# microsoft/Nova

Hardware: NVIDIA H100
Metric: MSM throughput (2^20 BN254 scalar*G1/s) (higher is better)
Workload: dtype u32 limbs (256-bit prime-field / curve integers)

## Files before the change

nova_b200/csrc/capi.cu:

```cuda
#include <cuda_runtime.h>

#include <atomic>
#include <cstdarg>
#include <cstdio>
#include <cstring>
#include <cstdlib>
#include <map>
#include <memory>
#include <mutex>
#include <vector>

#include "../../include/nova_b200.h"
#include "msm_kernels.cuh"
#include "field_kernels.cuh"
#include "ops.cuh"
#include "poly_kernels.cuh"
#include "transcript.cuh"
#include "transcript_batched.cuh"
#include "sumcheck_tail.cuh"

using namespace nova;

namespace {

thread_local char g_err[512] = "";

int fail(int code, const char* fmt, ...) {
  va_list ap;
  va_start(ap, fmt);
  vsnprintf(g_err, sizeof(g_err), fmt, ap);
  va_end(ap);
  return code;
}

#define CU(call)                                                                        \
  do {                                                                                  \
    cudaError_t e_ = (call);                                                            \
    if (e_ != cudaSuccess)                                                              \
      return fail(e_ == cudaErrorMemoryAllocation ? B200_E_NOMEM : B200_E_CUDA,         \
                  "%s failed: %s (%s:%d)", #call, cudaGetErrorString(e_), __FILE__, __LINE__); \
  } while (0)

struct curve_info {
  int base_fid, scalar_fid;
};
const curve_info CURVES[4] = {
    {B200_FIELD_BN254_FQ, B200_FIELD_BN254_FR},
    {B200_FIELD_BN254_FR, B200_FIELD_BN254_FQ},
    {B200_FIELD_PALLAS_FP, B200_FIELD_PALLAS_FQ},
    {B200_FIELD_PALLAS_FQ, B200_FIELD_PALLAS_FP},
};
const int FIELD_BITS[4] = {254, 254, 255, 255};

struct device_state {
  std::mutex mu;
  bool ready = false;
  int device = 0;
  cudaStream_t stream = nullptr;
  cudaStream_t aux = nullptr;
  bool pool = true;
} g_dev;

int ensure_init() {
  std::lock_guard<std::mutex> lk(g_dev.mu);
  if (g_dev.ready) {
    CU(cudaSetDevice(g_dev.device));
    return B200_OK;
  }
  int cnt = 0;
  cudaError_t e = cudaGetDeviceCount(&cnt);
  if (e != cudaSuccess || cnt == 0)
    return fail(B200_E_CUDA, "no usable CUDA device (%s); nova_b200 has no CPU fallback",
                e == cudaSuccess ? "count = 0" : cudaGetErrorString(e));
  CU(cudaSetDevice(g_dev.device));
  CU(cudaStreamCreateWithFlags(&g_dev.stream, cudaStreamNonBlocking));
  CU(cudaStreamCreateWithFlags(&g_dev.aux, cudaStreamNonBlocking));
  const char* pe = getenv("NOVA_B200_POOL");
  g_dev.pool = !(pe && pe[0] == '0');
  if (g_dev.pool) {
    cudaMemPool_t pool;
    if (cudaDeviceGetDefaultMemPool(&pool, g_dev.device) == cudaSuccess) {
      uint64_t keep = UINT64_MAX;
      cudaMemPoolSetAttribute(pool, cudaMemPoolAttrReleaseThreshold, &keep);
    } else {
      g_dev.pool = false;
      cudaGetLastError();
    }
  }
  g_dev.ready = true;
  return B200_OK;
}

cudaError_t pool_alloc(void** p, size_t bytes) {
  return g_dev.pool ? cudaMallocAsync(p, bytes ? bytes : 1, g_dev.stream) : cudaMalloc(p, bytes ? bytes : 1);
}
cudaError_t pool_free(void* p) { return g_dev.pool ? cudaFreeAsync(p, g_dev.stream) : cudaFree(p); }

struct workspace {
  size_t cap_n = 0;
  void* scalars = nullptr;
  int32_t* digits = nullptr;
  uint32_t *counts = nullptr, *start = nullptr, *cursor = nullptr, *blocksums = nullptr;
  uint64_t* entries = nullptr;
  void *buckets = nullptr, *parts = nullptr, *rparts = nullptr, *sumscratch = nullptr;
  uint32_t* pkeys = nullptr;
  uint32_t* heavy = nullptr;
  uint32_t heavy_cap = 0;
  void* hparts = nullptr;
  void* d_out = nullptr;
  void* h_out = nullptr;
  size_t out_slots = 0;
  uint32_t* idx32 = nullptr;
  size_t idx_cap = 0;
  cudaStream_t last_stream = nullptr;
  cudaEvent_t busy = nullptr;
  void release() {
    if (busy) cudaEventDestroy(busy);
    void* ptrs[] = {scalars, digits, counts, start, cursor, blocksums, entries, buckets,
                    parts, rparts, sumscratch, pkeys, heavy, hparts, d_out, idx32};
    for (void* p : ptrs)
      if (p) cudaFree(p);
    if (h_out) cudaFreeHost(h_out);
    *this = workspace();
  }
};

struct ck_ctx {
  std::mutex mu;
  int curve = 0;
  size_t n = 0;
  size_t stride = 0;
  bool has_h = false;
  int c = 0, W = 0, F = 0, G = 0;
  uint32_t B = 0;
  int m = 4;
  void* tables = nullptr;
  workspace ws;
  struct lane {
    workspace ws;
    cudaStream_t s = nullptr;
    cudaEvent_t done = nullptr;
  };
  static constexpr int NLANES = 4;
  lane lanes[NLANES];
  struct host_slot {
    std::mutex mu;
    workspace ws;
    cudaStream_t s = nullptr, side = nullptr;
  };
  static constexpr int NSLOTS = 4;
  host_slot slots[NSLOTS];
  unsigned next_slot = 0;
  std::shared_ptr<ck_ctx> small;
  ~ck_ctx() {
    if (tables) cudaFree(tables);
    ws.release();
    for (lane& l : lanes) {
      l.ws.release();
      if (l.done) cudaEventDestroy(l.done);
      if (l.s) cudaStreamDestroy(l.s);
    }
    for (host_slot& h : slots) {
      h.ws.release();
      if (h.s) cudaStreamDestroy(h.s);
      if (h.side) cudaStreamDestroy(h.side);
    }
  }
};

enum { ST_DIGITS = 0, ST_SORT, ST_ACCUMULATE, ST_FIXUP, ST_REDUCE, ST_COUNT };
const int STAGE_KERNELS[ST_COUNT] = {1, 4, 1, 3, 2};
struct profile_state {
  std::mutex mu;
  bool enabled = false;
  static constexpr int PROF_RING = 4;
  cudaEvent_t ev[PROF_RING][ST_COUNT + 1] = {};
  bool have_events = false;
  bool pending[PROF_RING] = {};
  int next = 0;
  double ms[ST_COUNT] = {};
  uint64_t msms = 0;
  uint64_t launches = 0;
} g_prof;

void prof_fold_set_locked(int k) {
  if (!g_prof.pending[k]) return;
  if (cudaEventSynchronize(g_prof.ev[k][ST_COUNT]) == cudaSuccess) {
    for (int i = 0; i < ST_COUNT; i++) {
      float t = 0;
      if (cudaEventElapsedTime(&t, g_prof.ev[k][i], g_prof.ev[k][i + 1]) == cudaSuccess) g_prof.ms[i] += t;
    }
    g_prof.msms++;
  }
  g_prof.pending[k] = false;
}
void prof_fold_locked() {
  for (int k = 0; k < profile_state::PROF_RING; k++) prof_fold_set_locked(k);
}

void count_launch(int k) {
  std::lock_guard<std::mutex> lk(g_prof.mu);
  g_prof.launches += k;
}

std::mutex g_handles_mu;
std::map<uint64_t, std::shared_ptr<ck_ctx>> g_handles;
uint64_t g_next_handle = 1;

std::shared_ptr<ck_ctx> get_ck(uint64_t h) {
  std::lock_guard<std::mutex> lk(g_handles_mu);
  auto it = g_handles.find(h);
  return it == g_handles.end() ? nullptr : it->second;
}

constexpr size_t XYZZ_BYTES = 144;
constexpr int SUM_THREADS = NUM_SMS * 128;
constexpr int L_MIN = 32;
constexpr int L_FLOOR_DEFAULT = 16;
constexpr size_t ACC_THREADS = (size_t)NUM_SMS * 16 * 32 * 3;
constexpr uint32_t HEAVY_PARTS = 96;

size_t acc_threads() {
  static const size_t threads = [] {
    const char* e = getenv("NOVA_B200_ACC_WAVES");
    double w = e ? atof(e) : 0.0;
    return w > 0.0 ? (size_t)((double)NUM_SMS * 16 * 32 * w) : ACC_THREADS;
  }();
  return threads;
}
size_t acc_lmin() {
  static const size_t lmin = [] {
    const char* e = getenv("NOVA_B200_ACC_LMIN");
    int v = e ? atoi(e) : L_FLOOR_DEFAULT;
    return (size_t)(v < 8 ? 8 : (v > L_MIN ? L_MIN : v));
  }();
  return lmin;
}
int segment_len(size_t entries) {
  size_t L = (entries + acc_threads() - 1) / acc_threads();
  return (int)(L < acc_lmin() ? acc_lmin() : L);
}
size_t max_segments(size_t entries) {
  size_t by_floor = (entries + acc_lmin() - 1) / acc_lmin();
  size_t cap = acc_threads() + 256;
  return by_floor < cap ? by_floor : cap;
}

int ws_acquire(workspace& w, cudaStream_t s) {
  if (w.busy && w.last_stream != s) CU(cudaStreamWaitEvent(s, w.busy, 0));
  return B200_OK;
}
int ws_release(workspace& w, cudaStream_t s) {
  if (!w.busy) CU(cudaEventCreateWithFlags(&w.busy, cudaEventDisableTiming));
  CU(cudaEventRecord(w.busy, s));
  w.last_stream = s;
  return B200_OK;
}

int ensure_workspace(ck_ctx& ck, workspace& w, size_t n, size_t out_slots) {
  if (out_slots > w.out_slots) {
    if (w.d_out) cudaFree(w.d_out);
    if (w.h_out) cudaFreeHost(w.h_out);
    w.d_out = w.h_out = nullptr;
    CU(cudaMalloc(&w.d_out, out_slots * 96));
    CU(cudaMallocHost(&w.h_out, out_slots * 96));
    w.out_slots = out_slots;
  }
  if (n <= w.cap_n) return B200_OK;
  CU(cudaDeviceSynchronize());
  void** szbufs[] = {&w.scalars, (void**)&w.digits, (void**)&w.entries, &w.parts, (void**)&w.pkeys,
                     (void**)&w.heavy, &w.hparts};
  for (void** p : szbufs)
    if (*p) {
      cudaFree(*p);
      *p = nullptr;
    }
  size_t K = (size_t)ck.G * ck.B;
  size_t entries = n * (size_t)ck.W;
  size_t nseg = max_segments(entries);
  w.heavy_cap = (uint32_t)(nseg / HEAVY_PARTS + 2);
  CU(cudaMalloc((void**)&w.heavy, ((size_t)w.heavy_cap + 1) * 4));
  CU(cudaMalloc(&w.hparts, (size_t)w.heavy_cap * HEAVY_SPLIT * XYZZ_BYTES));
  CU(cudaMalloc(&w.scalars, n * 32));
  CU(cudaMalloc((void**)&w.digits, entries * sizeof(int32_t)));
  CU(cudaMalloc((void**)&w.entries, entries * sizeof(uint64_t)));
  CU(cudaMalloc(&w.parts, 2 * nseg * XYZZ_BYTES));
  CU(cudaMalloc((void**)&w.pkeys, 2 * nseg * sizeof(uint32_t)));
  if (!w.counts) {
    CU(cudaMalloc((void**)&w.counts, K * 4));
    CU(cudaMalloc((void**)&w.start, (K + 1) * 4));
    CU(cudaMalloc((void**)&w.cursor, K * 4));
    CU(cudaMalloc((void**)&w.blocksums, 4096 * 4));
    CU(cudaMalloc(&w.buckets, K * XYZZ_BYTES));
    CU(cudaMalloc(&w.rparts, ((size_t)ck.G * (ck.B / ck.m + 4096)) * XYZZ_BYTES));
    CU(cudaMalloc(&w.sumscratch, (size_t)SUM_THREADS * XYZZ_BYTES));
  }
  w.cap_n = n;
  return B200_OK;
}

int ensure_workspace(ck_ctx& ck, size_t n, size_t out_slots) {
  return ensure_workspace(ck, ck.ws, n, out_slots);
}

msm_plan make_plan(ck_ctx& ck, workspace& ws, size_t base_offset, size_t n) {
  msm_plan p;
  p.n = n;
  p.n_ck = ck.stride;
  p.base_offset = base_offset;
  p.blind_i = SIZE_MAX;
  p.h_index = ck.n;
  p.c = ck.c;
  p.W = ck.W;
  p.G = ck.G;
  p.B = ck.B;
  p.L = segment_len(n * (size_t)ck.W);
  p.m = ck.m;
  p.heavy = ws.heavy;
  p.heavy_min = HEAVY_PARTS * (uint32_t)p.L;
  p.heavy_cap = ws.heavy_cap;
  p.hparts = ws.hparts;
  p.digits = ws.digits;
  p.counts = ws.counts;
  p.start = ws.start;
  p.cursor = ws.cursor;
  p.entries = ws.entries;
  p.buckets = ws.buckets;
  p.parts = ws.parts;
  p.pkeys = ws.pkeys;
  p.rparts = ws.rparts;
  p.blocksums = ws.blocksums;
  return p;
}

int enqueue_msm(ck_ctx& ck, workspace& ws, size_t base_offset, const void* d_scalars, size_t n,
                void* d_out, cudaStream_t s, int small_elem_bytes = 0, bool blinded = false,
                bool digits_done = false, const msm_peer* peer = nullptr, bool profile_ok = true) {
  const field_ops* sops = ops_for_field(CURVES[ck.curve].scalar_fid);
  const field_ops* bops = ops_for_field(CURVES[ck.curve].base_fid);
  {
    int arc = ws_acquire(ws, s);
    if (arc) return arc;
  }
  if (n == 0) {
    if (peer && peer->world > 1) {
      msm_plan p0 = make_plan(ck, ws, base_offset, 0);
      p0.peer = *peer;
      bops->exchange_identity(s, p0, d_out);
      count_launch(1);
      CU(cudaGetLastError());
      return B200_OK;
    }
    CU(cudaMemsetAsync(d_out, 0, 96, s));
    return B200_OK;
  }
  msm_plan p = make_plan(ck, ws, base_offset, n);
  if (peer) p.peer = *peer;
  if (blinded) p.blind_i = n - 1;
  size_t K = (size_t)ck.G * ck.B;
  if (!digits_done) CU(cudaMemsetAsync(p.counts, 0, K * 4, s));
  CU(cudaMemsetAsync(p.heavy, 0, 4, s));
  std::lock_guard<std::mutex> plk(g_prof.mu);
  const bool prof = g_prof.enabled && profile_ok;
  const int pset = g_prof.next;
  if (prof) {
    if (!g_prof.have_events) {
      for (auto& set : g_prof.ev)
        for (auto& e : set) CU(cudaEventCreate(&e));
      g_prof.have_events = true;
    }
    prof_fold_set_locked(pset);
    g_prof.next = (pset + 1) % profile_state::PROF_RING;
  }
#define STAGE_MARK(i) \
  if (prof) CU(cudaEventRecord(g_prof.ev[pset][i], s))
  STAGE_MARK(ST_DIGITS);
  if (digits_done)
    ;
  else if (small_elem_bytes)
    msm_digits_small(s, d_scalars, small_elem_bytes, p);
  else
    sops->digits(s, d_scalars, p);
  STAGE_MARK(ST_SORT);
  msm_scan(s, p);
  msm_scatter(s, p);
  STAGE_MARK(ST_ACCUMULATE);
  bops->accumulate(s, ck.tables, p);
  STAGE_MARK(ST_FIXUP);
  bops->fixup(s, p);
  STAGE_MARK(ST_REDUCE);
  bops->reduce(s, p, d_out);
  STAGE_MARK(ST_COUNT);
#undef STAGE_MARK
  if (prof) g_prof.pending[pset] = true;
  for (int i = 0; i < ST_COUNT; i++) g_prof.launches += STAGE_KERNELS[i];
  g_prof.launches += (ck.c - 1 + 3) / 4 - 1;
  CU(cudaGetLastError());
  return ws_release(ws, s);
}

int enqueue_msm(ck_ctx& ck, size_t base_offset, const void* d_scalars, size_t n, void* d_out,
                cudaStream_t s, int small_elem_bytes = 0, bool blinded = false) {
  return enqueue_msm(ck, ck.ws, base_offset, d_scalars, n, d_out, s, small_elem_bytes, blinded);
}

struct dev_flag {
  uint32_t* p = nullptr;
  ~dev_flag() {
    if (p) cudaFree(p);
  }
};

constexpr size_t SMALL_KEY_MAX = (size_t)1 << 21;
constexpr int SMALL_KEY_WINDOW = 17;

int choose_window(size_t n) {
  int lg = 0;
  while (((size_t)1 << lg) < n) lg++;
  int c = lg;
  if (c < 8) c = 8;
  if (c > 16) c = 16;
  if (lg >= 22) c = 20;
  else if (lg >= 19) c = 17;
  return c;
}

constexpr int CURVE_B_SMALL[4] = {3, -17, 5, 5};

int register_key(int curve_id, const void* bases, bool bases_on_device, size_t n, const void* h,
                 int window_bits, bool expand, std::shared_ptr<ck_ctx>& out, size_t* first_bad = nullptr,
                 cudaStream_t st = nullptr, size_t src_pitch_points = 0, size_t src_block_points = 0) {
  if (!st) st = g_dev.stream;
  if (curve_id < 0 || curve_id > 3) return fail(B200_E_ARG, "unknown curve id %d", curve_id);
  if (bases == nullptr || n == 0) return fail(B200_E_ARG, "empty commitment key");
  if (window_bits != 0 && (window_bits < 2 || window_bits > 24))
    return fail(B200_E_ARG, "window_bits %d out of range [2,24]", window_bits);
  auto ck = std::make_shared<ck_ctx>();
  ck->curve = curve_id;
  ck->n = n;
  ck->has_h = h != nullptr;
  ck->stride = n + (h ? 1 : 0);
  ck->c = window_bits ? window_bits : choose_window(n);
  int bits = FIELD_BITS[CURVES[curve_id].scalar_fid];
  ck->W = (bits + ck->c - 1) / ck->c;
  ck->F = expand ? ck->W : 1;
  ck->G = expand ? 1 : ck->W;
  ck->B = 1u << (ck->c - 1);
  ck->m = ck->B >= 4 ? 4 : 1;
  if ((size_t)ck->F * ck->stride >= ((size_t)1 << 31))
    return fail(B200_E_RANGE, "key too large for 31-bit table indices (%zu x %d)", n, ck->F);
  CU(cudaMalloc(&ck->tables, (size_t)ck->F * ck->stride * 64));
  const cudaMemcpyKind kind = bases_on_device ? cudaMemcpyDeviceToDevice : cudaMemcpyHostToDevice;
  if (src_block_points == 0) {
    CU(cudaMemcpyAsync(ck->tables, bases, n * 64, kind, st));
  } else {
    const size_t full = n / src_block_points, rest = n % src_block_points;
    if (full)
      CU(cudaMemcpy2DAsync(ck->tables, src_block_points * 64, bases, src_pitch_points * 64, src_block_points * 64, full,
                           kind, st));
    if (rest)
      CU(cudaMemcpyAsync((char*)ck->tables + full * src_block_points * 64,
                         (const char*)bases + full * src_pitch_points * 64, rest * 64, kind, st));
  }
  if (h)
    CU(cudaMemcpyAsync((char*)ck->tables + n * 64, h, 64, cudaMemcpyHostToDevice, st));
  if (first_bad) {
    *first_bad = SIZE_MAX;
    dev_flag flag;
    CU(cudaMalloc(&flag.p, 4));
    CU(cudaMemsetAsync(flag.p, 0xFF, 4, st));
    ops_for_field(CURVES[curve_id].base_fid)
        ->on_curve(st, ck->tables, ck->stride, CURVE_B_SMALL[curve_id], flag.p);
    count_launch(1);
    CU(cudaGetLastError());
    uint32_t bad = 0;
    CU(cudaMemcpyAsync(&bad, flag.p, 4, cudaMemcpyDeviceToHost, st));
    CU(cudaStreamSynchronize(st));
    if (bad != 0xFFFFFFFFu) {
      *first_bad = bad;
      return fail(B200_E_POINT, "key point %u%s has a non-canonical coordinate or is not on the curve", bad,
                  (h && bad == n) ? " (the blinding generator)" : "");
    }
  }
  {
    const field_ops* bops = ops_for_field(CURVES[curve_id].base_fid);
    bops->expand_key(st, ck->tables, ck->stride, ck->F, ck->c * ck->G);
    CU(cudaGetLastError());
  }
  CU(cudaStreamSynchronize(st));
  if (expand && window_bits == 0 && ck->c >= 20) {
    size_t ns = n < SMALL_KEY_MAX ? n : SMALL_KEY_MAX;
    if (src_block_points) return fail(B200_E_ARG, "strided keys carry one table set");
    int rc = register_key(curve_id, bases, bases_on_device, ns, h, SMALL_KEY_WINDOW, true, ck->small, nullptr, st);
    if (rc) return rc;
  }
  out = ck;
  return B200_OK;
}

ck_ctx& route(ck_ctx& ck, size_t base_offset, size_t n) {
  if (ck.small && base_offset + n <= ck.small->n) return *ck.small;
  return ck;
}

template <class Fn>
int with_field(int field_id, Fn fn) {
  int rc = ensure_init();
  if (rc) return rc;
  const field_ops* ops = ops_for_field(field_id);
  if (!ops) return fail(B200_E_ARG, "unknown field id %d", field_id);
  return fn(ops);
}

struct dev_buf {
  void* p = nullptr;
  ~dev_buf() {
    if (p) pool_free(p);
  }
  int alloc(size_t bytes) {
    CU(pool_alloc(&p, bytes));
    return B200_OK;
  }
};

}

extern "C" {

const char* b200_last_error(void) { return g_err; }
const char* b200_version(void) { return "nova_b200 0.1 (sm_90a)"; }

int b200_init(int device) {
  {
    std::lock_guard<std::mutex> lk(g_dev.mu);
    if (!g_dev.ready) g_dev.device = device;
  }
  return ensure_init();
}

int b200_device_count(int* count) {
  if (!count) return fail(B200_E_ARG, "null count");
  cudaError_t e = cudaGetDeviceCount(count);
  if (e != cudaSuccess) {
    *count = 0;
    return fail(B200_E_CUDA, "cudaGetDeviceCount: %s", cudaGetErrorString(e));
  }
  return B200_OK;
}

int b200_host_alloc(size_t bytes, void** ptr) {
  int rc = ensure_init();
  if (rc) return rc;
  CU(cudaMallocHost(ptr, bytes ? bytes : 1));
  return B200_OK;
}
int b200_host_free(void* ptr) {
  CU(cudaFreeHost(ptr));
  return B200_OK;
}
int b200_dev_alloc(size_t bytes, void** dptr) {
  int rc = ensure_init();
  if (rc) return rc;
  CU(pool_alloc(dptr, bytes));
  return B200_OK;
}
int b200_dev_free(void* dptr) {
  if (!dptr) return B200_OK;
  int rc = ensure_init();
  if (rc) return rc;
  CU(pool_free(dptr));
  return B200_OK;
}
int b200_memcpy_h2d(void* dptr, const void* hptr, size_t bytes) {
  int rc = ensure_init();
  if (rc) return rc;
  CU(cudaMemcpyAsync(dptr, hptr, bytes, cudaMemcpyHostToDevice, g_dev.stream));
  CU(cudaStreamSynchronize(g_dev.stream));
  return B200_OK;
}
int b200_memcpy_d2h(void* hptr, const void* dptr, size_t bytes) {
  int rc = ensure_init();
  if (rc) return rc;
  CU(cudaMemcpyAsync(hptr, dptr, bytes, cudaMemcpyDeviceToHost, g_dev.stream));
  CU(cudaStreamSynchronize(g_dev.stream));
  return B200_OK;
}
int b200_memcpy_d2d(void* dst, const void* src, size_t bytes, void* stream) {
  int rc = ensure_init();
  if (rc) return rc;
  if (bytes == 0) return B200_OK;
  if (!dst || !src) return fail(B200_E_ARG, "null pointer");
  CU(cudaMemcpyAsync(dst, src, bytes, cudaMemcpyDeviceToDevice,
                     stream ? (cudaStream_t)stream : g_dev.stream));
  return B200_OK;
}
int b200_memset_dev(void* dptr, int byte, size_t bytes, void* stream) {
  int rc = ensure_init();
  if (rc) return rc;
  if (bytes == 0) return B200_OK;
  if (!dptr) return fail(B200_E_ARG, "null pointer");
  CU(cudaMemsetAsync(dptr, byte, bytes, stream ? (cudaStream_t)stream : g_dev.stream));
  return B200_OK;
}
int b200_sync(void) {
  int rc = ensure_init();
  if (rc) return rc;
  CU(cudaDeviceSynchronize());
  return B200_OK;
}

int b200_profile_enable(int on) {
  std::lock_guard<std::mutex> lk(g_prof.mu);
  g_prof.enabled = on != 0;
  return B200_OK;
}
int b200_profile_reset(void) {
  std::lock_guard<std::mutex> lk(g_prof.mu);
  prof_fold_locked();
  for (double& m : g_prof.ms) m = 0;
  g_prof.msms = 0;
  g_prof.launches = 0;
  return B200_OK;
}
int b200_profile_read(double* stage_ms, int nstages, uint64_t* msms, uint64_t* launches) {
  std::lock_guard<std::mutex> lk(g_prof.mu);
  prof_fold_locked();
  for (int i = 0; i < nstages && i < ST_COUNT; i++)
    if (stage_ms) stage_ms[i] = g_prof.ms[i];
  if (msms) *msms = g_prof.msms;
  if (launches) *launches = g_prof.launches;
  return B200_OK;
}

int b200_jacobian_sum_dev(int curve_id, const void* d_points, size_t k, void* d_out, void* stream) {
  int rc = ensure_init();
  if (rc) return rc;
  if (curve_id < 0 || curve_id > 3) return fail(B200_E_ARG, "unknown curve id %d", curve_id);
  if (!d_out || (k && !d_points)) return fail(B200_E_ARG, "null pointer");
  const field_ops* bops = ops_for_field(CURVES[curve_id].base_fid);
  bops->jacobian_sum(stream ? (cudaStream_t)stream : g_dev.stream, d_points, (int)k, d_out);
  {
    std::lock_guard<std::mutex> lk(g_prof.mu);
    g_prof.launches += 1;
  }
  CU(cudaGetLastError());
  return B200_OK;
}

int b200_ck_register(int curve_id, const void* bases, size_t n, const void* h, int window_bits,
                     uint64_t* handle) {
  int rc = ensure_init();
  if (rc) return rc;
  if (!handle) return fail(B200_E_ARG, "null handle pointer");
  std::shared_ptr<ck_ctx> ck;
  rc = register_key(curve_id, bases, false, n, h, window_bits, true, ck);
  if (rc) return rc;
  std::lock_guard<std::mutex> lk(g_handles_mu);
  *handle = g_next_handle++;
  g_handles[*handle] = ck;
  return B200_OK;
}

int b200_ck_register_checked(int curve_id, const void* bases, size_t n, const void* h, int window_bits,
                             uint64_t* handle, size_t* first_bad) {
  int rc = ensure_init();
  if (rc) return rc;
  if (!handle || !first_bad) return fail(B200_E_ARG, "null pointer");
  *handle = 0;
  std::shared_ptr<ck_ctx> ck;
  rc = register_key(curve_id, bases, false, n, h, window_bits, true, ck, first_bad);
  if (rc) return rc;
  std::lock_guard<std::mutex> lk(g_handles_mu);
  *handle = g_next_handle++;
  g_handles[*handle] = ck;
  return B200_OK;
}

int b200_ck_setup_synthetic(int curve_id, const void* gen_affine, uint64_t k0, size_t n, int with_h,
                            int window_bits, uint64_t* handle) {
  int rc = ensure_init();
  if (rc) return rc;
  if (curve_id < 0 || curve_id > 3) return fail(B200_E_ARG, "unknown curve id %d", curve_id);
  if (!gen_affine || !handle || n == 0) return fail(B200_E_ARG, "bad argument");
  size_t total = n + (with_h ? 1 : 0);
  dev_buf bases, gen;
  if ((rc = bases.alloc(total * 64))) return rc;
  if ((rc = gen.alloc(64))) return rc;
  CU(cudaMemcpyAsync(gen.p, gen_affine, 64, cudaMemcpyHostToDevice, g_dev.stream));
  const field_ops* bops = ops_for_field(CURVES[curve_id].base_fid);
  bops->index_bases(g_dev.stream, bases.p, total, gen.p, k0);
  CU(cudaGetLastError());
  std::vector<char> h(64);
  if (with_h)
    CU(cudaMemcpyAsync(h.data(), (char*)bases.p + n * 64, 64, cudaMemcpyDeviceToHost, g_dev.stream));
  CU(cudaStreamSynchronize(g_dev.stream));
  std::shared_ptr<ck_ctx> ck;
  rc = register_key(curve_id, bases.p, true, n, with_h ? h.data() : nullptr, window_bits, true, ck);
  if (rc) return rc;
  std::lock_guard<std::mutex> lk(g_handles_mu);
  *handle = g_next_handle++;
  g_handles[*handle] = ck;
  return B200_OK;
}

int b200_ck_setup_tau(int curve_id, const void* gen_affine, const void* tau_mont, size_t n, int window_bits,
                      uint64_t* handle) {
  int rc = ensure_init();
  if (rc) return rc;
  if (curve_id < 0 || curve_id > 3) return fail(B200_E_ARG, "unknown curve id %d", curve_id);
  if (!gen_affine || !tau_mont || !handle || n == 0) return fail(B200_E_ARG, "bad argument");
  dev_buf bases, gen, tau, pw;
  if ((rc = bases.alloc(n * 64)) || (rc = gen.alloc(64)) || (rc = tau.alloc(32)) || (rc = pw.alloc(n * 32))) return rc;
  CU(cudaMemcpyAsync(gen.p, gen_affine, 64, cudaMemcpyHostToDevice, g_dev.stream));
  CU(cudaMemcpyAsync(tau.p, tau_mont, 32, cudaMemcpyHostToDevice, g_dev.stream));
  ops_for_field(CURVES[curve_id].scalar_fid)->powers_canonical(g_dev.stream, tau.p, n, pw.p);
  ops_for_field(CURVES[curve_id].base_fid)->scalar_bases(g_dev.stream, bases.p, n, gen.p, pw.p);
  count_launch(2);
  CU(cudaGetLastError());
  CU(cudaStreamSynchronize(g_dev.stream));
  std::shared_ptr<ck_ctx> ck;
  rc = register_key(curve_id, bases.p, true, n, nullptr, window_bits, true, ck);
  if (rc) return rc;
  std::lock_guard<std::mutex> lk(g_handles_mu);
  *handle = g_next_handle++;
  g_handles[*handle] = ck;
  return B200_OK;
}

int b200_ck_export_bases(uint64_t handle, size_t offset, size_t n, void* out_host) {
  int rc = ensure_init();
  if (rc) return rc;
  auto ck = get_ck(handle);
  if (!ck) return fail(B200_E_HANDLE, "unknown key handle %llu", (unsigned long long)handle);
  if (offset + n > ck->n) return fail(B200_E_RANGE, "export [%zu, %zu) exceeds key length %zu", offset, offset + n, ck->n);
  if (n == 0) return B200_OK;
  if (!out_host) return fail(B200_E_ARG, "null pointer");
#if defined(NOVA_MSM_ARITH29)
  return fail(B200_E_ARG, "b200_ck_export_bases: table 0 is not in the boundary format in this build");
#else
  std::lock_guard<std::mutex> lk(ck->mu);
  CU(cudaMemcpyAsync(out_host, (const char*)ck->tables + offset * 64, n * 64, cudaMemcpyDeviceToHost, g_dev.stream));
  CU(cudaStreamSynchronize(g_dev.stream));
  return B200_OK;
#endif
}

int b200_ck_release(uint64_t handle) {
  std::shared_ptr<ck_ctx> ck;
  {
    std::lock_guard<std::mutex> lk(g_handles_mu);
    auto it = g_handles.find(handle);
    if (it == g_handles.end()) return fail(B200_E_HANDLE, "unknown key handle %llu",
                                           (unsigned long long)handle);
    ck = it->second;
    g_handles.erase(it);
  }
  std::lock_guard<std::mutex> lk(ck->mu);
  for (ck_ctx* t : {ck.get(), ck->small.get()})
    if (t)
      for (ck_ctx::host_slot& h : t->slots) std::lock_guard<std::mutex> wait(h.mu);
  cudaSetDevice(g_dev.device);
  return B200_OK;
}

int b200_ck_len(uint64_t handle, size_t* n, int* window_bits, int* num_tables) {
  auto ck = get_ck(handle);
  if (!ck) return fail(B200_E_HANDLE, "unknown key handle %llu", (unsigned long long)handle);
  if (n) *n = ck->n;
  if (window_bits) *window_bits = ck->c;
  if (num_tables) *num_tables = ck->F;
  return B200_OK;
}

static int lane_stream(ck_ctx::lane& ln, int index) {
  if (ln.s) return B200_OK;
  int least = 0, greatest = 0;
  CU(cudaDeviceGetStreamPriorityRange(&least, &greatest));
  int prio = greatest + index;
  if (prio > least) prio = least;
  CU(cudaStreamCreateWithPriority(&ln.s, cudaStreamNonBlocking, prio));
  CU(cudaEventCreateWithFlags(&ln.done, cudaEventDisableTiming));
  return B200_OK;
}

static int msm_host(ck_ctx& ck, size_t base_offset, const void* scalars, size_t n, void* out,
                    const void* blind = nullptr) {
  int rc = B200_OK;
  static const int h2d_chunks = [] {
    const char* e = getenv("NOVA_B200_H2D_CHUNKS");
    int k = e ? atoi(e) : 4;
    return k < 1 ? 1 : (k > 64 ? 64 : k);
  }();
  static const int e2e_slices = [] {
    const char* e = getenv("NOVA_B200_E2E_SLICES");
    int k = e ? atoi(e) : 4;
    return k < 1 ? 1 : (k > ck_ctx::NLANES ? ck_ctx::NLANES : k);
  }();
  if (e2e_slices > 1 && n >= ((size_t)1 << 23)) {
    std::lock_guard<std::mutex> lk(ck.mu);
    cudaStream_t s = g_dev.stream;
    const int k = e2e_slices;
    rc = ensure_workspace(ck, 1, (size_t)k + 1);
    if (rc) return rc;
    if ((rc = ws_acquire(ck.ws, s))) return rc;
    cudaEvent_t ev = nullptr;
    CU(cudaEventCreateWithFlags(&ev, cudaEventDisableTiming));
    CU(cudaEventRecord(ev, s));
    const size_t per = (n + k - 1) / k;
    int used = 0;
    for (int j = 0; j < k && rc == B200_OK; j++) {
      const size_t lo = (size_t)j * per, hi = lo + per < n ? lo + per : n;
      if (lo >= hi) break;
      const bool last = hi == n;
      ck_ctx::lane& ln = ck.lanes[j];
      if ((rc = lane_stream(ln, j))) break;
      CU(cudaStreamWaitEvent(ln.s, ev, 0));
      rc = ensure_workspace(ck, ln.ws, hi - lo + 1, 1);
      if (rc) break;
      if ((rc = ws_acquire(ln.ws, ln.s))) break;
      CU(cudaMemcpyAsync(ln.ws.scalars, (const char*)scalars + 32 * lo, 32 * (hi - lo), cudaMemcpyHostToDevice, ln.s));
      const bool with_blind = last && blind != nullptr;
      if (with_blind)
        CU(cudaMemcpyAsync((char*)ln.ws.scalars + 32 * (hi - lo), blind, 32, cudaMemcpyHostToDevice, ln.s));
      rc = enqueue_msm(ck, ln.ws, base_offset + lo, ln.ws.scalars, hi - lo + (with_blind ? 1 : 0),
                       (char*)ck.ws.d_out + 96 * (j + 1), ln.s, 0, with_blind);
      used = j + 1;
    }
    for (int j = 0; j < used; j++) {
      cudaEventRecord(ck.lanes[j].done, ck.lanes[j].s);
      cudaStreamWaitEvent(s, ck.lanes[j].done, 0);
    }
    cudaEventDestroy(ev);
    if (rc) return rc;
    ops_for_field(CURVES[ck.curve].base_fid)->jacobian_sum(s, (char*)ck.ws.d_out + 96, used, ck.ws.d_out);
    count_launch(1);
    CU(cudaGetLastError());
    CU(cudaMemcpyAsync(ck.ws.h_out, ck.ws.d_out, 96, cudaMemcpyDeviceToHost, s));
    CU(cudaStreamSynchronize(s));
    memcpy(out, ck.ws.h_out, 96);
    return B200_OK;
  }
  ck_ctx::host_slot* slot = nullptr;
  for (ck_ctx::host_slot& h : ck.slots)
    if (h.mu.try_lock()) {
      slot = &h;
      break;
    }
  if (!slot) {
    unsigned turn;
    {
      std::lock_guard<std::mutex> lk(ck.mu);
      turn = ck.next_slot++ % ck_ctx::NSLOTS;
    }
    slot = &ck.slots[turn];
    slot->mu.lock();
  }
  std::lock_guard<std::mutex> slk(slot->mu, std::adopt_lock);
  if (!slot->s) {
    CU(cudaStreamCreateWithFlags(&slot->s, cudaStreamNonBlocking));
    CU(cudaStreamCreateWithFlags(&slot->side, cudaStreamNonBlocking));
  }
  workspace& W = slot->ws;
  cudaStream_t s = slot->s;
  if ((rc = ensure_workspace(ck, W, n + 1, 1))) return rc;
  if (h2d_chunks > 1 && n >= ((size_t)1 << 16)) {
    cudaStream_t side = slot->side;
    const size_t total = n + (blind ? 1 : 0);
    const field_ops* sops = ops_for_field(CURVES[ck.curve].scalar_fid);
    msm_plan p = make_plan(ck, W, base_offset, total);
    cudaEvent_t ev = nullptr;
    CU(cudaEventCreateWithFlags(&ev, cudaEventDisableTiming));
    CU(cudaEventRecord(ev, s));
    CU(cudaStreamWaitEvent(side, ev, 0));
    CU(cudaMemsetAsync(p.counts, 0, (size_t)ck.G * ck.B * 4, side));
    const size_t per = (n + h2d_chunks - 1) / h2d_chunks;
    auto piece = [&](const void* src, size_t lo, size_t hi) -> int {
      CU(cudaMemcpyAsync((char*)W.scalars + 32 * lo, src, 32 * (hi - lo), cudaMemcpyHostToDevice, s));
      CU(cudaEventRecord(ev, s));
      CU(cudaStreamWaitEvent(side, ev, 0));
      sops->digits_range(side, W.scalars, lo, hi, p);
      count_launch(1);
      return B200_OK;
    };
    for (size_t lo = 0; lo < n && rc == B200_OK; lo += per)
      rc = piece((const char*)scalars + 32 * lo, lo, lo + per < n ? lo + per : n);
    if (blind && rc == B200_OK) rc = piece(blind, n, n + 1);
    if (rc) {
      cudaEventDestroy(ev);
      return rc;
    }
    CU(cudaEventRecord(ev, side));
    CU(cudaStreamWaitEvent(s, ev, 0));
    cudaEventDestroy(ev);
    rc = enqueue_msm(ck, W, base_offset, W.scalars, total, W.d_out, s, 0, blind != nullptr, true);
  } else {
    if (n) CU(cudaMemcpyAsync(W.scalars, scalars, n * 32, cudaMemcpyHostToDevice, s));
    if (blind) CU(cudaMemcpyAsync((char*)W.scalars + n * 32, blind, 32, cudaMemcpyHostToDevice, s));
    rc = enqueue_msm(ck, W, base_offset, W.scalars, n + (blind ? 1 : 0), W.d_out, s, 0, blind != nullptr);
  }
  if (rc) return rc;
  CU(cudaMemcpyAsync(W.h_out, W.d_out, 96, cudaMemcpyDeviceToHost, s));
  CU(cudaStreamSynchronize(s));
  memcpy(out, W.h_out, 96);
  return B200_OK;
}

int b200_msm(uint64_t handle, size_t base_offset, const void* scalars, size_t n, void* out) {
  int rc = ensure_init();
  if (rc) return rc;
  auto ck = get_ck(handle);
  if (!ck) return fail(B200_E_HANDLE, "unknown key handle %llu", (unsigned long long)handle);
  if (!out || (n && !scalars)) return fail(B200_E_ARG, "null pointer");
  if (base_offset + n > ck->n)
    return fail(B200_E_RANGE, "msm slice [%zu, %zu) exceeds key length %zu", base_offset,
                base_offset + n, ck->n);
  return msm_host(route(*ck, base_offset, n), base_offset, scalars, n, out);
}

int b200_commit(uint64_t handle, const void* scalars, size_t n, const void* r, void* out) {
  int rc = ensure_init();
  if (rc) return rc;
  auto ck = get_ck(handle);
  if (!ck) return fail(B200_E_HANDLE, "unknown key handle %llu", (unsigned long long)handle);
  if (!out || (n && !scalars)) return fail(B200_E_ARG, "null pointer");
  if (n > ck->n)
    return fail(B200_E_RANGE, "commit of %zu scalars exceeds key length %zu", n, ck->n);
  if (r && !ck->has_h) return fail(B200_E_ARG, "key was registered without a blinding generator");
  return msm_host(route(*ck, 0, n), 0, scalars, n, out, r);
}

int b200_msm_dev(uint64_t handle, size_t base_offset, const void* d_scalars, size_t n, void* d_out,
                 void* stream) {
  int rc = ensure_init();
  if (rc) return rc;
  auto ck = get_ck(handle);
  if (!ck) return fail(B200_E_HANDLE, "unknown key handle %llu", (unsigned long long)handle);
  if (!d_out || (n && !d_scalars)) return fail(B200_E_ARG, "null pointer");
  if (base_offset + n > ck->n)
    return fail(B200_E_RANGE, "msm slice [%zu, %zu) exceeds key length %zu", base_offset,
                base_offset + n, ck->n);
  ck_ctx& t = route(*ck, base_offset, n);
  std::lock_guard<std::mutex> lk(t.mu);
  rc = ensure_workspace(t, n ? n : 1, 1);
  if (rc) return rc;
  return enqueue_msm(t, base_offset, d_scalars, n, d_out,
                     stream ? (cudaStream_t)stream : g_dev.stream);
}

int b200_commit_dev(uint64_t handle, const void* d_scalars, size_t n, const void* d_blind_or_null,
                    void* d_out, void* stream) {
  int rc = ensure_init();
  if (rc) return rc;
  auto ck = get_ck(handle);
  if (!ck) return fail(B200_E_HANDLE, "unknown key handle %llu", (unsigned long long)handle);
  if (!d_out || (n && !d_scalars)) return fail(B200_E_ARG, "null pointer");
  if (n > ck->n) return fail(B200_E_RANGE, "commit of %zu scalars exceeds key length %zu", n, ck->n);
  if (d_blind_or_null && !ck->has_h)
    return fail(B200_E_ARG, "key was registered without a blinding generator");
  ck_ctx& t = route(*ck, 0, n);
  std::lock_guard<std::mutex> lk(t.mu);
  rc = ensure_workspace(t, n + 1, 1);
  if (rc) return rc;
  cudaStream_t s = stream ? (cudaStream_t)stream : g_dev.stream;
  if (!d_blind_or_null) return enqueue_msm(t, 0, d_scalars, n, d_out, s);
  if ((rc = ws_acquire(t.ws, s))) return rc;
  if (n) CU(cudaMemcpyAsync(t.ws.scalars, d_scalars, n * 32, cudaMemcpyDeviceToDevice, s));
  CU(cudaMemcpyAsync((char*)t.ws.scalars + n * 32, d_blind_or_null, 32, cudaMemcpyDeviceToDevice, s));
  return enqueue_msm(t, 0, t.ws.scalars, n + 1, d_out, s, 0, true);
}

static int enqueue_many(ck_ctx& ck, const void* const* vecs, const size_t* lens, size_t k,
                        bool from_host, void* d_out, cudaStream_t s, const size_t* offsets = nullptr) {
  std::unique_lock<std::mutex> lsmall;
  if (ck.small) lsmall = std::unique_lock<std::mutex>(ck.small->mu);
  cudaEvent_t start_ev = nullptr;
  CU(cudaEventCreateWithFlags(&start_ev, cudaEventDisableTiming));
  CU(cudaEventRecord(start_ev, s));
  bool used[2][ck_ctx::NLANES] = {};
  size_t next[2] = {0, 0};
  int rc = B200_OK;
  for (size_t j = 0; j < k && rc == B200_OK; j++) {
    const size_t off = offsets ? offsets[j] : 0;
    ck_ctx& t = route(ck, off, lens[j]);
    int which = &t == &ck ? 0 : 1;
    int li = (int)(next[which]++ % ck_ctx::NLANES);
    ck_ctx::lane& ln = t.lanes[li];
    if ((rc = lane_stream(ln, li))) break;
    if (!used[which][li]) {
      CU(cudaStreamWaitEvent(ln.s, start_ev, 0));
      used[which][li] = true;
    }
    rc = ensure_workspace(t, ln.ws, lens[j] ? lens[j] : 1, 1);
    if (rc) break;
    const void* src = vecs[j];
    if ((rc = ws_acquire(ln.ws, ln.s))) break;
    if (from_host && lens[j]) {
      CU(cudaMemcpyAsync(ln.ws.scalars, vecs[j], lens[j] * 32, cudaMemcpyHostToDevice, ln.s));
      src = ln.ws.scalars;
    }
    rc = enqueue_msm(t, ln.ws, off, src, lens[j], (char*)d_out + 96 * j, ln.s);
  }
  for (int which = 0; which < 2; which++) {
    ck_ctx* t = which == 0 ? &ck : ck.small.get();
    for (int li = 0; t && li < ck_ctx::NLANES; li++)
      if (used[which][li]) {
        cudaEventRecord(t->lanes[li].done, t->lanes[li].s);
        cudaStreamWaitEvent(s, t->lanes[li].done, 0);
      }
  }
  cudaEventDestroy(start_ev);
  return rc;
}

static int check_many(ck_ctx& ck, const void* const* vecs, const size_t* lens, size_t k) {
  if (!vecs || !lens) return fail(B200_E_ARG, "null pointer");
  for (size_t j = 0; j < k; j++) {
    if (lens[j] > ck.n)
      return fail(B200_E_RANGE, "batch vector %zu has %zu scalars, key has %zu", j, lens[j], ck.n);
    if (lens[j] && !vecs[j]) return fail(B200_E_ARG, "null scalar vector %zu", j);
  }
  return B200_OK;
}

int b200_msm_batch(uint64_t handle, const void* const* scalars, const size_t* lens, size_t k,
                   void* out) {
  int rc = ensure_init();
  if (rc) return rc;
  auto ck = get_ck(handle);
  if (!ck) return fail(B200_E_HANDLE, "unknown key handle %llu", (unsigned long long)handle);
  if (k == 0) return B200_OK;
  if (!out) return fail(B200_E_ARG, "null pointer");
  if ((rc = check_many(*ck, scalars, lens, k))) return rc;
  std::lock_guard<std::mutex> lk(ck->mu);
  rc = ensure_workspace(*ck, 1, k);
  if (rc) return rc;
  cudaStream_t s = g_dev.stream;
  rc = enqueue_many(*ck, scalars, lens, k, true, ck->ws.d_out, s);
  if (rc) return rc;
  CU(cudaMemcpyAsync(ck->ws.h_out, ck->ws.d_out, 96 * k, cudaMemcpyDeviceToHost, s));
  CU(cudaStreamSynchronize(s));
  memcpy(out, ck->ws.h_out, 96 * k);
  return B200_OK;
}

int b200_commit_many_dev(uint64_t handle, const void* const* d_scalars, const size_t* lens, size_t k,
                         void* d_out, void* stream) {
  int rc = ensure_init();
  if (rc) return rc;
  auto ck = get_ck(handle);
  if (!ck) return fail(B200_E_HANDLE, "unknown key handle %llu", (unsigned long long)handle);
  if (k == 0) return B200_OK;
  if (!d_out) return fail(B200_E_ARG, "null pointer");
  if ((rc = check_many(*ck, d_scalars, lens, k))) return rc;
  std::lock_guard<std::mutex> lk(ck->mu);
  return enqueue_many(*ck, d_scalars, lens, k, false, d_out,
                      stream ? (cudaStream_t)stream : g_dev.stream);
}

int b200_msm_many_dev(uint64_t handle, const size_t* base_offsets, const void* const* d_scalars, const size_t* lens,
                      size_t k, void* d_out, void* stream) {
  int rc = ensure_init();
  if (rc) return rc;
  auto ck = get_ck(handle);
  if (!ck) return fail(B200_E_HANDLE, "unknown key handle %llu", (unsigned long long)handle);
  if (k == 0) return B200_OK;
  if (!d_out || !base_offsets || !d_scalars || !lens) return fail(B200_E_ARG, "null pointer");
  for (size_t j = 0; j < k; j++) {
    if (base_offsets[j] + lens[j] > ck->n)
      return fail(B200_E_RANGE, "msm %zu: slice [%zu, %zu) exceeds key length %zu", j, base_offsets[j],
                  base_offsets[j] + lens[j], ck->n);
    if (lens[j] && !d_scalars[j]) return fail(B200_E_ARG, "null scalar vector %zu", j);
  }
  std::lock_guard<std::mutex> lk(ck->mu);
  return enqueue_many(*ck, d_scalars, lens, k, false, d_out,
                      stream ? (cudaStream_t)stream : g_dev.stream, base_offsets);
}

int b200_msm_small(uint64_t handle, size_t base_offset, const void* scalars, int elem_bytes, size_t n,
                   int max_bits, void* out) {
  int rc = ensure_init();
  if (rc) return rc;
  auto ck = get_ck(handle);
  if (!ck) return fail(B200_E_HANDLE, "unknown key handle %llu", (unsigned long long)handle);
  if (!out || (n && !scalars)) return fail(B200_E_ARG, "null pointer");
  if (elem_bytes != 1 && elem_bytes != 2 && elem_bytes != 4 && elem_bytes != 8)
    return fail(B200_E_ARG, "elem_bytes must be 1, 2, 4 or 8 (got %d)", elem_bytes);
  if (max_bits < 0 || max_bits > 64) return fail(B200_E_ARG, "max_bits %d out of range", max_bits);
  if (base_offset + n > ck->n)
    return fail(B200_E_RANGE, "msm slice [%zu, %zu) exceeds key length %zu", base_offset,
                base_offset + n, ck->n);
  ck_ctx& t = route(*ck, base_offset, n);
  std::lock_guard<std::mutex> lk(t.mu);
  rc = ensure_workspace(t, n ? n : 1, 1);
  if (rc) return rc;
  cudaStream_t s = g_dev.stream;
  if ((rc = ws_acquire(t.ws, s))) return rc;
  if (n) CU(cudaMemcpyAsync(t.ws.scalars, scalars, n * elem_bytes, cudaMemcpyHostToDevice, s));
  rc = enqueue_msm(t, base_offset, t.ws.scalars, n, t.ws.d_out, s, elem_bytes);
  if (rc) return rc;
  CU(cudaMemcpyAsync(t.ws.h_out, t.ws.d_out, 96, cudaMemcpyDeviceToHost, s));
  CU(cudaStreamSynchronize(s));
  memcpy(out, t.ws.h_out, 96);
  return B200_OK;
}

int b200_msm_indices(uint64_t handle, const uint64_t* idx, size_t m, void* out) {
  int rc = ensure_init();
  if (rc) return rc;
  auto ck = get_ck(handle);
  if (!ck) return fail(B200_E_HANDLE, "unknown key handle %llu", (unsigned long long)handle);
  if (!out || (m && !idx)) return fail(B200_E_ARG, "null pointer");
  std::vector<uint32_t> idx32(m);
  for (size_t j = 0; j < m; j++) {
    if (idx[j] >= ck->n) return fail(B200_E_RANGE, "index %llu outside key of %zu",
                                     (unsigned long long)idx[j], ck->n);
    idx32[j] = (uint32_t)idx[j];
  }
  std::lock_guard<std::mutex> lk(ck->mu);
  rc = ensure_workspace(*ck, 1, 1);
  if (rc) return rc;
  workspace& w = ck->ws;
  if (m > w.idx_cap) {
    if (w.idx32) cudaFree(w.idx32);
    w.idx32 = nullptr;
    CU(cudaMalloc((void**)&w.idx32, m * 4));
    w.idx_cap = m;
  }
  cudaStream_t s = g_dev.stream;
  if (m) CU(cudaMemcpyAsync(w.idx32, idx32.data(), m * 4, cudaMemcpyHostToDevice, s));
  const field_ops* bops = ops_for_field(CURVES[ck->curve].base_fid);
  bops->sum_points(s, ck->tables, w.idx32, m, w.sumscratch, w.d_out);
  count_launch(2);
  CU(cudaGetLastError());
  CU(cudaMemcpyAsync(w.h_out, w.d_out, 96, cudaMemcpyDeviceToHost, s));
  CU(cudaStreamSynchronize(s));
  memcpy(out, w.h_out, 96);
  return B200_OK;
}

int b200_msm_adhoc(int curve_id, const void* bases, const void* scalars, size_t n, void* out) {
  int rc = ensure_init();
  if (rc) return rc;
  if (!out) return fail(B200_E_ARG, "null out");
  if (n == 0) {
    memset(out, 0, 96);
    return B200_OK;
  }
  if (!bases || !scalars) return fail(B200_E_ARG, "null pointer");
  std::shared_ptr<ck_ctx> ck;
  rc = register_key(curve_id, bases, false, n, nullptr, 0, false, ck);
  if (rc) return rc;
  return msm_host(route(*ck, 0, n), 0, scalars, n, out);
}

int b200_keccak256(const void* data, size_t len, void* out32) {
  if (!out32 || (len && !data)) return fail(B200_E_ARG, "null pointer");
  const size_t rate = 136;
  uint64_t st[25] = {};
  const uint8_t* p = (const uint8_t*)data;
  auto absorb_block = [&](const uint8_t* blk) {
    for (size_t i = 0; i < rate / 8; i++) {
      uint64_t w;
      memcpy(&w, blk + 8 * i, 8);
      st[i] ^= w;
    }
    nova::keccak_f1600(st);
  };
  while (len >= rate) {
    absorb_block(p);
    p += rate;
    len -= rate;
  }
  uint8_t last[136] = {};
  if (len) memcpy(last, p, len);
  last[len] ^= 0x01;
  last[rate - 1] ^= 0x80;
  absorb_block(last);
  memcpy(out32, st, 32);
  return B200_OK;
}

namespace {
struct peer_group {
  std::mutex mu;
  msm_peer desc;
};
std::mutex g_groups_mu;
std::map<uint64_t, std::shared_ptr<peer_group>> g_groups;
uint64_t g_next_group = 1;
}

int b200_peer_buffer_alloc(void** dptr) {
  int rc = ensure_init();
  if (rc) return rc;
  if (!dptr) return fail(B200_E_ARG, "null pointer");
  CU(cudaMalloc(dptr, MSM_PEER_BUF_BYTES));
  CU(cudaMemset(*dptr, 0, MSM_PEER_BUF_BYTES));
  return B200_OK;
}
int b200_peer_buffer_free(void* dptr) {
  if (dptr) CU(cudaFree(dptr));
  return B200_OK;
}
int b200_ipc_export(const void* dptr, void* handle64_out) {
  int rc = ensure_init();
  if (rc) return rc;
  if (!dptr || !handle64_out) return fail(B200_E_ARG, "null pointer");
  static_assert(sizeof(cudaIpcMemHandle_t) == 64, "the ABI carries IPC handles as 64 bytes");
  cudaIpcMemHandle_t h;
  CU(cudaIpcGetMemHandle(&h, const_cast<void*>(dptr)));
  memcpy(handle64_out, &h, 64);
  return B200_OK;
}
int b200_ipc_open(const void* handle64, void** dptr) {
  int rc = ensure_init();
  if (rc) return rc;
  if (!handle64 || !dptr) return fail(B200_E_ARG, "null pointer");
  cudaIpcMemHandle_t h;
  memcpy(&h, handle64, 64);
  CU(cudaIpcOpenMemHandle(dptr, h, cudaIpcMemLazyEnablePeerAccess));
  return B200_OK;
}
int b200_ipc_close(void* dptr) {
  if (!dptr) return B200_OK;
  CU(cudaIpcCloseMemHandle(dptr));
  return B200_OK;
}
int b200_peer_group_create(int rank, int world, void* const* bufs, uint64_t* group) {
  int rc = ensure_init();
  if (rc) return rc;
  if (!bufs || !group) return fail(B200_E_ARG, "null pointer");
  if (world < 1 || world > MSM_PEER_MAX || rank < 0 || rank >= world)
    return fail(B200_E_ARG, "peer group of %d ranks (rank %d): world must be 1..%d", world, rank, MSM_PEER_MAX);
  auto g = std::make_shared<peer_group>();
  g->desc.world = world;
  g->desc.rank = rank;
  for (int r = 0; r < world; r++) {
    if (!bufs[r]) return fail(B200_E_ARG, "null exchange buffer for rank %d", r);
    g->desc.buf[r] = bufs[r];
  }
  std::lock_guard<std::mutex> lk(g_groups_mu);
  *group = g_next_group++;
  g_groups[*group] = g;
  return B200_OK;
}
int b200_peer_group_release(uint64_t group) {
  std::lock_guard<std::mutex> lk(g_groups_mu);
  if (!g_groups.erase(group)) return fail(B200_E_HANDLE, "unknown peer group %llu", (unsigned long long)group);
  return B200_OK;
}
static std::shared_ptr<peer_group> get_group(uint64_t h) {
  std::lock_guard<std::mutex> lk(g_groups_mu);
  auto it = g_groups.find(h);
  return it == g_groups.end() ? nullptr : it->second;
}
int b200_peer_group_status(uint64_t group) {
  int rc = ensure_init();
  if (rc) return rc;
  auto g = get_group(group);
  if (!g) return fail(B200_E_HANDLE, "unknown peer group %llu", (unsigned long long)group);
  unsigned long long err = 0;
  CU(cudaMemcpy(&err, (const char*)g->desc.buf[g->desc.rank] + MSM_PEER_ERR_OFF, 8, cudaMemcpyDeviceToHost));
  if (err) return fail(B200_E_PEER, "a peer never delivered its partial sum (epoch %llu): exchange timed out", err);
  return B200_OK;
}

int b200_msm_sharded_dev(uint64_t handle, size_t base_offset, const void* d_scalars, size_t n, uint64_t group,
                         void* d_out, void* stream) {
  int rc = ensure_init();
  if (rc) return rc;
  auto ck = get_ck(handle);
  if (!ck) return fail(B200_E_HANDLE, "unknown key handle %llu", (unsigned long long)handle);
  auto g = get_group(group);
  if (!g) return fail(B200_E_HANDLE, "unknown peer group %llu", (unsigned long long)group);
  if (!d_out || (n && !d_scalars)) return fail(B200_E_ARG, "null pointer");
  if (base_offset + n > ck->n)
    return fail(B200_E_RANGE, "msm slice [%zu, %zu) exceeds key length %zu", base_offset, base_offset + n, ck->n);
#if defined(NOVA_MSM_ARITH29)
  return fail(B200_E_ARG, "the fused exchange needs the default (8x32-bit) arithmetic build");
#else
  ck_ctx& t = route(*ck, base_offset, n);
  std::lock_guard<std::mutex> glk(g->mu);
  std::lock_guard<std::mutex> lk(t.mu);
  rc = ensure_workspace(t, n ? n : 1, 1);
  if (rc) return rc;
  msm_peer peer = g->desc;
  peer.epoch = ++g->desc.epoch;
  return enqueue_msm(t, t.ws, base_offset, d_scalars, n, d_out, stream ? (cudaStream_t)stream : g_dev.stream, 0,
                     false, false, &peer);
#endif
}

namespace {
struct poseidon_ctx {
  int fid = 0, t = 0, r_f = 0, r_p = 0;
  void *rc = nullptr, *mds = nullptr;
  ~poseidon_ctx() {
    if (rc) cudaFree(rc);
    if (mds) cudaFree(mds);
  }
};
std::mutex g_pos_mu;
std::map<uint64_t, std::shared_ptr<poseidon_ctx>> g_pos;
uint64_t g_next_pos = 1;

void poseidon_tag(uint32_t n, unsigned char out32[32]) {
  typedef unsigned __int128 u128;
  const u128 base = (u128)0 - 159;
  u128 x_i = 1, state = 0;
  auto update = [&](uint32_t a) {
    x_i *= base;
    state += x_i * (u128)a;
  };
  if (n) update(n + (1u << 31));
  update(1);
  update(0);
  memset(out32, 0, 32);
  memcpy(out32, &state, 16);
}
}

int b200_poseidon_register(int fid, int arity, int r_f, int r_p, const void* rc_mont, const void* mds_mont, uint64_t* handle) {
  int rc = ensure_init();
  if (rc) return rc;
  if (!ops_for_field(fid)) return fail(B200_E_ARG, "unknown field id %d", fid);
  if (arity < 1 || arity + 1 > 25 || r_f < 2 || (r_f & 1) || r_p < 0 || !rc_mont || !mds_mont || !handle)
    return fail(B200_E_ARG, "bad Poseidon parameters (arity %d, R_F %d, R_P %d)", arity, r_f, r_p);
  auto c = std::make_shared<poseidon_ctx>();
  c->fid = fid;
  c->t = arity + 1;
  c->r_f = r_f;
  c->r_p = r_p;
  const size_t nrc = (size_t)(r_f + r_p) * c->t, nm = (size_t)c->t * c->t;
  CU(cudaMalloc(&c->rc, nrc * 32));
  CU(cudaMalloc(&c->mds, nm * 32));
  CU(cudaMemcpyAsync(c->rc, rc_mont, nrc * 32, cudaMemcpyHostToDevice, g_dev.stream));
  CU(cudaMemcpyAsync(c->mds, mds_mont, nm * 32, cudaMemcpyHostToDevice, g_dev.stream));
  CU(cudaStreamSynchronize(g_dev.stream));
  std::lock_guard<std::mutex> lk(g_pos_mu);
  *handle = g_next_pos++;
  g_pos[*handle] = c;
  return B200_OK;
}
int b200_poseidon_release(uint64_t handle) {
  std::lock_guard<std::mutex> lk(g_pos_mu);
  if (!g_pos.erase(handle)) return fail(B200_E_HANDLE, "unknown Poseidon handle %llu", (unsigned long long)handle);
  return B200_OK;
}
int b200_poseidon_ro_dev(uint64_t handle, const void* d_elems, size_t n, int num_bits, int start_with_one, void* d_out96,
                         void* stream) {
  int rc = ensure_init();
  if (rc) return rc;
  std::shared_ptr<poseidon_ctx> c;
  {
    std::lock_guard<std::mutex> lk(g_pos_mu);
    auto it = g_pos.find(handle);
    if (it == g_pos.end()) return fail(B200_E_HANDLE, "unknown Poseidon handle %llu", (unsigned long long)handle);
    c = it->second;
  }
  if (!d_out96 || (n && !d_elems)) return fail(B200_E_ARG, "null pointer");
  if (num_bits < 1 || num_bits > 250) return fail(B200_E_ARG, "num_bits %d outside 1..250", num_bits);
  if (n >= (1u << 31)) return fail(B200_E_ARG, "too many elements");
  cudaStream_t s = stream ? (cudaStream_t)stream : g_dev.stream;
  unsigned char tag[32];
  poseidon_tag((uint32_t)n, tag);
  void* d_tag = nullptr;
  CU(cudaMallocAsync(&d_tag, 32, s));
  CU(cudaMemcpyAsync(d_tag, tag, 32, cudaMemcpyHostToDevice, s));
  ops_for_field(c->fid)->poseidon_ro(s, c->t, c->r_f, c->r_p, c->rc, c->mds, d_elems, (uint32_t)n, d_tag, num_bits,
                                     start_with_one, d_out96);
  count_launch(1);
  CU(cudaGetLastError());
  CU(cudaFreeAsync(d_tag, s));
  return B200_OK;
}
int b200_poseidon_ro(uint64_t handle, const void* elems_mont, size_t n, int num_bits, int start_with_one, void* out96) {
  int rc = ensure_init();
  if (rc) return rc;
  if (!out96 || (n && !elems_mont)) return fail(B200_E_ARG, "null pointer");
  dev_buf in, out;
  if ((rc = in.alloc(n * 32 + 32)) || (rc = out.alloc(96))) return rc;
  if (n) CU(cudaMemcpyAsync(in.p, elems_mont, n * 32, cudaMemcpyHostToDevice, g_dev.stream));
  rc = b200_poseidon_ro_dev(handle, in.p, n, num_bits, start_with_one, out.p, g_dev.stream);
  if (rc) return rc;
  CU(cudaMemcpyAsync(out96, out.p, 96, cudaMemcpyDeviceToHost, g_dev.stream));
  CU(cudaStreamSynchronize(g_dev.stream));
  return B200_OK;
}
int b200_to_mont_dev(int fid, const void* d_canonical, size_t n, void* d_out, void* stream) {
  return with_field(fid, [&](const field_ops* ops) {
    if (n && (!d_canonical || !d_out)) return fail(B200_E_ARG, "null pointer");
    ops->to_mont(stream ? (cudaStream_t)stream : g_dev.stream, d_canonical, n, d_out);
    count_launch(1);
    CU(cudaGetLastError());
    return (int)B200_OK;
  });
}

namespace {
constexpr size_t MGPU_BLOCK = 4096;
struct mgpu_state {
  std::mutex mu;
  bool ready = false;
  int ndev = 0;
  int dev[MSM_PEER_MAX] = {};
  cudaStream_t stream[MSM_PEER_MAX] = {};
  void* xbuf[MSM_PEER_MAX] = {};
  void* out_dev[MSM_PEER_MAX] = {};
  void* out_host = nullptr;
  unsigned long long epoch = 0;
} g_mgpu;
struct mgpu_key {
  int curve = 0;
  size_t n = 0;
  bool has_h = false;
  std::shared_ptr<ck_ctx> part[MSM_PEER_MAX];
};
std::mutex g_mkeys_mu;
std::map<uint64_t, std::shared_ptr<mgpu_key>> g_mkeys;
uint64_t g_next_mkey = 1;

size_t mgpu_count(size_t n, int d, int D) {
  const size_t round = MGPU_BLOCK * (size_t)D;
  const size_t rem = n % round;
  size_t extra = rem > (size_t)d * MGPU_BLOCK ? rem - (size_t)d * MGPU_BLOCK : 0;
  if (extra > MGPU_BLOCK) extra = MGPU_BLOCK;
  return (n / round) * MGPU_BLOCK + extra;
}
struct device_guard {
  ~device_guard() { cudaSetDevice(g_dev.device); }
};
}

int b200_mgpu_init(int ndev, const int* devices_or_null) {
  int rc = ensure_init();
  if (rc) return rc;
  if (ndev < 1 || ndev > MSM_PEER_MAX) return fail(B200_E_ARG, "ndev %d outside 1..%d", ndev, MSM_PEER_MAX);
  std::lock_guard<std::mutex> lk(g_mgpu.mu);
  if (g_mgpu.ready) {
    if (g_mgpu.ndev != ndev) return fail(B200_E_ARG, "already initialised with %d devices", g_mgpu.ndev);
    return B200_OK;
  }
  int have = 0;
  CU(cudaGetDeviceCount(&have));
  device_guard guard;
  for (int d = 0; d < ndev; d++) {
    int id = devices_or_null ? devices_or_null[d] : d;
    if (id < 0 || id >= have) return fail(B200_E_ARG, "device %d not present (%d visible)", id, have);
    g_mgpu.dev[d] = id;
  }
  for (int d = 0; d < ndev; d++) {
    CU(cudaSetDevice(g_mgpu.dev[d]));
    CU(cudaStreamCreateWithFlags(&g_mgpu.stream[d], cudaStreamNonBlocking));
    CU(cudaMalloc(&g_mgpu.xbuf[d], MSM_PEER_BUF_BYTES));
    CU(cudaMemset(g_mgpu.xbuf[d], 0, MSM_PEER_BUF_BYTES));
    CU(cudaMalloc(&g_mgpu.out_dev[d], 96));
    for (int e = 0; e < ndev; e++) {
      if (g_mgpu.dev[e] == g_mgpu.dev[d]) continue;
      int can = 0;
      CU(cudaDeviceCanAccessPeer(&can, g_mgpu.dev[d], g_mgpu.dev[e]));
      if (!can) return fail(B200_E_CUDA, "device %d cannot access device %d (no NVLink / P2P path)", g_mgpu.dev[d], g_mgpu.dev[e]);
      cudaError_t pe = cudaDeviceEnablePeerAccess(g_mgpu.dev[e], 0);
      if (pe != cudaSuccess && pe != cudaErrorPeerAccessAlreadyEnabled)
        return fail(B200_E_CUDA, "cudaDeviceEnablePeerAccess(%d -> %d): %s", g_mgpu.dev[d], g_mgpu.dev[e], cudaGetErrorString(pe));
      cudaGetLastError();
    }
  }
  CU(cudaMallocHost(&g_mgpu.out_host, 96));
  g_mgpu.ndev = ndev;
  g_mgpu.ready = true;
  return B200_OK;
}

int b200_mgpu_ck_register(int curve_id, const void* bases, size_t n, const void* h, int window_bits, uint64_t* key) {
  int rc = ensure_init();
  if (rc) return rc;
  if (!g_mgpu.ready) return fail(B200_E_ARG, "b200_mgpu_init has not been called");
  if (curve_id < 0 || curve_id > 3) return fail(B200_E_ARG, "unknown curve id %d", curve_id);
  if (!bases || !key || n == 0) return fail(B200_E_ARG, "bad argument");
  std::lock_guard<std::mutex> lk(g_mgpu.mu);
  device_guard guard;
  auto mk = std::make_shared<mgpu_key>();
  mk->curve = curve_id;
  mk->n = n;
  mk->has_h = h != nullptr;
  const int D = g_mgpu.ndev;
  for (int d = 0; d < D; d++) {
    size_t nd = mgpu_count(n, d, D);
    if (nd == 0 && !(d == 0 && h)) continue;
    CU(cudaSetDevice(g_mgpu.dev[d]));
    if (nd == 0) return fail(B200_E_ARG, "key of %zu points is too small to carry a blinding generator on %d devices", n, D);
    rc = register_key(curve_id, (const char*)bases + (size_t)d * MGPU_BLOCK * 64, false, nd, d == 0 ? h : nullptr,
                      window_bits, true, mk->part[d], nullptr, g_mgpu.stream[d], MGPU_BLOCK * (size_t)D, MGPU_BLOCK);
    if (rc) return rc;
  }
  std::lock_guard<std::mutex> lk2(g_mkeys_mu);
  *key = g_next_mkey++;
  g_mkeys[*key] = mk;
  return B200_OK;
}

int b200_mgpu_ck_release(uint64_t key) {
  std::shared_ptr<mgpu_key> mk;
  {
    std::lock_guard<std::mutex> lk(g_mkeys_mu);
    auto it = g_mkeys.find(key);
    if (it == g_mkeys.end()) return fail(B200_E_HANDLE, "unknown multi-GPU key %llu", (unsigned long long)key);
    mk = it->second;
    g_mkeys.erase(it);
  }
  std::lock_guard<std::mutex> lk(g_mgpu.mu);
  device_guard guard;
  for (int d = 0; d < g_mgpu.ndev; d++) {
    cudaSetDevice(g_mgpu.dev[d]);
    cudaStreamSynchronize(g_mgpu.stream[d]);
  }
  return B200_OK;
}

int b200_mgpu_commit(uint64_t key, const void* scalars, size_t n, const void* r, void* out) {
  int rc = ensure_init();
  if (rc) return rc;
  if (!g_mgpu.ready) return fail(B200_E_ARG, "b200_mgpu_init has not been called");
  std::shared_ptr<mgpu_key> mk;
  {
    std::lock_guard<std::mutex> lk(g_mkeys_mu);
    auto it = g_mkeys.find(key);
    if (it == g_mkeys.end()) return fail(B200_E_HANDLE, "unknown multi-GPU key %llu", (unsigned long long)key);
    mk = it->second;
  }
  if (!out || (n && !scalars)) return fail(B200_E_ARG, "null pointer");
  if (n > mk->n) return fail(B200_E_RANGE, "commit of %zu scalars exceeds key length %zu", n, mk->n);
  if (r && !mk->has_h) return fail(B200_E_ARG, "key was registered without a blinding generator");
#if defined(NOVA_MSM_ARITH29)
  return fail(B200_E_ARG, "the fused exchange needs the default (8x32-bit) arithmetic build");
#else
  std::lock_guard<std::mutex> lk(g_mgpu.mu);
  device_guard guard;
  const int D = g_mgpu.ndev;
  msm_peer peer;
  peer.world = D;
  peer.epoch = ++g_mgpu.epoch;
  for (int d = 0; d < D; d++) peer.buf[d] = g_mgpu.xbuf[d];
  const field_ops* bops = ops_for_field(CURVES[mk->curve].base_fid);
  for (int d = 0; d < D; d++) {
    ck_ctx* part = mk->part[d].get();
    const size_t nd = mgpu_count(n, d, D);
    if (!part || (nd == 0 && !(d == 0 && r))) continue;
    CU(cudaSetDevice(g_mgpu.dev[d]));
    std::lock_guard<std::mutex> plk(part->mu);
    if ((rc = ensure_workspace(*part, part->ws, nd + 1, 1))) return rc;
  }
  for (int d = 0; d < D; d++) {
    CU(cudaSetDevice(g_mgpu.dev[d]));
    cudaStream_t s = g_mgpu.stream[d];
    peer.rank = d;
    const size_t nd = mgpu_count(n, d, D);
    const bool blind = d == 0 && r != nullptr;
    ck_ctx* part = mk->part[d].get();
    if ((nd == 0 && !blind) || !part) {
      msm_plan p0{};
      p0.peer = peer;
      bops->exchange_identity(s, p0, g_mgpu.out_dev[d]);
      count_launch(1);
      CU(cudaGetLastError());
      continue;
    }
    std::lock_guard<std::mutex> plk(part->mu);
    rc = ensure_workspace(*part, part->ws, nd + 1, 1);
    if (rc) return rc;
    if ((rc = ws_acquire(part->ws, s))) return rc;
    const size_t full = nd / MGPU_BLOCK, rest = nd % MGPU_BLOCK;
    const char* src = (const char*)scalars + (size_t)d * MGPU_BLOCK * 32;
    if (full)
      CU(cudaMemcpy2DAsync(part->ws.scalars, MGPU_BLOCK * 32, src, MGPU_BLOCK * (size_t)D * 32, MGPU_BLOCK * 32, full,
                           cudaMemcpyHostToDevice, s));
    if (rest)
      CU(cudaMemcpyAsync((char*)part->ws.scalars + full * MGPU_BLOCK * 32, src + full * MGPU_BLOCK * (size_t)D * 32,
                         rest * 32, cudaMemcpyHostToDevice, s));
    if (blind) CU(cudaMemcpyAsync((char*)part->ws.scalars + nd * 32, r, 32, cudaMemcpyHostToDevice, s));
    rc = enqueue_msm(*part, part->ws, 0, part->ws.scalars, nd + (blind ? 1 : 0), g_mgpu.out_dev[d], s, 0, blind, false,
                     &peer, false);
    if (rc) return rc;
  }
  CU(cudaSetDevice(g_mgpu.dev[0]));
  CU(cudaMemcpyAsync(g_mgpu.out_host, g_mgpu.out_dev[0], 96, cudaMemcpyDeviceToHost, g_mgpu.stream[0]));
  for (int d = 0; d < D; d++) {
    CU(cudaSetDevice(g_mgpu.dev[d]));
    CU(cudaStreamSynchronize(g_mgpu.stream[d]));
  }
  unsigned long long err = 0;
  CU(cudaSetDevice(g_mgpu.dev[0]));
  CU(cudaMemcpy(&err, (const char*)g_mgpu.xbuf[0] + MSM_PEER_ERR_OFF, 8, cudaMemcpyDeviceToHost));
  if (err) return fail(B200_E_PEER, "a device never delivered its partial sum (epoch %llu)", err);
  memcpy(out, g_mgpu.out_host, 96);
  return B200_OK;
#endif
}

int b200_cross_term_dev(int fid, const void* az, const void* bz, const void* cz, const void* e1,
                        const void* e2, const void* u, size_t n, void* t, void* stream) {
  return with_field(fid, [&](const field_ops* ops) {
    if (n == 0) return (int)B200_OK;
    if (!az || !bz || !cz || !e1 || !u || !t) return fail(B200_E_ARG, "null pointer");
    ops->cross_term(stream ? (cudaStream_t)stream : g_dev.stream, az, bz, cz, e1, e2, u, n, t);
    count_launch(1);
    CU(cudaGetLastError());
    return (int)B200_OK;
  });
}
int b200_axpy_dev(int fid, const void* a, const void* b, const void* r, size_t n, void* out,
                  void* stream) {
  return with_field(fid, [&](const field_ops* ops) {
    if (n == 0) return (int)B200_OK;
    if (!a || !b || !r || !out) return fail(B200_E_ARG, "null pointer");
    ops->axpy(stream ? (cudaStream_t)stream : g_dev.stream, a, b, r, n, out);
    count_launch(1);
    CU(cudaGetLastError());
    return (int)B200_OK;
  });
}
int b200_vec_mul_dev(int fid, const void* a, const void* b, size_t n, void* out, void* stream) {
  return with_field(fid, [&](const field_ops* ops) {
    if (n == 0) return (int)B200_OK;
    if (!a || !b || !out) return fail(B200_E_ARG, "null pointer");
    ops->vec_mul(stream ? (cudaStream_t)stream : g_dev.stream, a, b, n, out);
    count_launch(1);
    CU(cudaGetLastError());
    return (int)B200_OK;
  });
}
int b200_logup_hash_dev(int fid, const void* val, const void* addr_or_null, const void* gamma,
                        const void* r, size_t n, void* out, void* stream) {
  return with_field(fid, [&](const field_ops* ops) {
    if (n == 0) return (int)B200_OK;
    if (!val || !gamma || !r || !out) return fail(B200_E_ARG, "null pointer");
    ops->logup_hash(stream ? (cudaStream_t)stream : g_dev.stream, val, addr_or_null, gamma, r, n, out);
    count_launch(1);
    CU(cudaGetLastError());
    return (int)B200_OK;
  });
}
int b200_vec_add_dev(int fid, const void* a, const void* b, size_t n, void* out, void* stream) {
  return with_field(fid, [&](const field_ops* ops) {
    if (n == 0) return (int)B200_OK;
    if (!a || !b || !out) return fail(B200_E_ARG, "null pointer");
    ops->vec_add(stream ? (cudaStream_t)stream : g_dev.stream, a, b, n, out);
    count_launch(1);
    CU(cudaGetLastError());
    return (int)B200_OK;
  });
}
int b200_bind_top_dev(int fid, void* z, size_t n, const void* r, void* stream) {
  return with_field(fid, [&](const field_ops* ops) {
    if (n < 2) return (int)B200_OK;
    if (n & 1) return fail(B200_E_ARG, "bind_top needs an even length, got %zu", n);
    if (!z || !r) return fail(B200_E_ARG, "null pointer");
    ops->bind_top(stream ? (cudaStream_t)stream : g_dev.stream, z, n, r);
    count_launch(1);
    CU(cudaGetLastError());
    return (int)B200_OK;
  });
}

int b200_bind_top_multi_dev(int fid, void* const* zs, size_t k, size_t n, const void* r, void* stream) {
  return with_field(fid, [&](const field_ops* ops) {
    if (k == 0 || n < 2) return (int)B200_OK;
    if (n & 1) return fail(B200_E_ARG, "bind_top needs an even length, got %zu", n);
    if (!zs || !r) return fail(B200_E_ARG, "null pointer");
    cudaStream_t s = stream ? (cudaStream_t)stream : g_dev.stream;
    for (size_t j = 0; j < k; j += BIND_MULTI_MAX) {
      const int cnt = (int)(k - j < (size_t)BIND_MULTI_MAX ? k - j : (size_t)BIND_MULTI_MAX);
      for (int i = 0; i < cnt; i++)
        if (!zs[j + i]) return fail(B200_E_ARG, "null table %zu", j + i);
      ops->bind_top_multi(s, zs + j, cnt, n, r);
      count_launch(1);
    }
    CU(cudaGetLastError());
    return (int)B200_OK;
  });
}

int b200_cross_term(int fid, const void* az, const void* bz, const void* cz, const void* e1,
                    const void* e2, const void* u, size_t n, void* t) {
  int rc = ensure_init();
  if (rc) return rc;
  if (n == 0) return B200_OK;
  if (!az || !bz || !cz || !e1 || !u || !t) return fail(B200_E_ARG, "null pointer");
  dev_buf buf;
  size_t vec = n * 32;
  int nvec = e2 ? 6 : 5;
  rc = buf.alloc(vec * nvec + 32);
  if (rc) return rc;
  char* d = (char*)buf.p;
  cudaStream_t s = g_dev.stream;
  const void* src[5] = {az, bz, cz, e1, e2};
  for (int k = 0; k < (e2 ? 5 : 4); k++)
    CU(cudaMemcpyAsync(d + vec * k, src[k], vec, cudaMemcpyHostToDevice, s));
  char* du = d + vec * nvec;
  CU(cudaMemcpyAsync(du, u, 32, cudaMemcpyHostToDevice, s));
  char* dt = d + vec * (nvec - 1);
  rc = b200_cross_term_dev(fid, d, d + vec, d + 2 * vec, d + 3 * vec, e2 ? d + 4 * vec : nullptr, du,
                           n, dt, s);
  if (rc) return rc;
  CU(cudaMemcpyAsync(t, dt, vec, cudaMemcpyDeviceToHost, s));
  CU(cudaStreamSynchronize(s));
  return B200_OK;
}

int b200_axpy(int fid, const void* a, const void* b, const void* r, size_t n, void* out) {
  int rc = ensure_init();
  if (rc) return rc;
  if (n == 0) return B200_OK;
  if (!a || !b || !r || !out) return fail(B200_E_ARG, "null pointer");
  dev_buf buf;
  size_t vec = n * 32;
  rc = buf.alloc(vec * 3 + 32);
  if (rc) return rc;
  char* d = (char*)buf.p;
  cudaStream_t s = g_dev.stream;
  CU(cudaMemcpyAsync(d, a, vec, cudaMemcpyHostToDevice, s));
  CU(cudaMemcpyAsync(d + vec, b, vec, cudaMemcpyHostToDevice, s));
  CU(cudaMemcpyAsync(d + 3 * vec, r, 32, cudaMemcpyHostToDevice, s));
  rc = b200_axpy_dev(fid, d, d + vec, d + 3 * vec, n, d + 2 * vec, s);
  if (rc) return rc;
  CU(cudaMemcpyAsync(out, d + 2 * vec, vec, cudaMemcpyDeviceToHost, s));
  CU(cudaStreamSynchronize(s));
  return B200_OK;
}

int b200_vec_add(int fid, const void* a, const void* b, size_t n, void* out) {
  int rc = ensure_init();
  if (rc) return rc;
  if (n == 0) return B200_OK;
  if (!a || !b || !out) return fail(B200_E_ARG, "null pointer");
  dev_buf buf;
  size_t vec = n * 32;
  rc = buf.alloc(vec * 3);
  if (rc) return rc;
  char* d = (char*)buf.p;
  cudaStream_t s = g_dev.stream;
  CU(cudaMemcpyAsync(d, a, vec, cudaMemcpyHostToDevice, s));
  CU(cudaMemcpyAsync(d + vec, b, vec, cudaMemcpyHostToDevice, s));
  rc = b200_vec_add_dev(fid, d, d + vec, n, d + 2 * vec, s);
  if (rc) return rc;
  CU(cudaMemcpyAsync(out, d + 2 * vec, vec, cudaMemcpyDeviceToHost, s));
  CU(cudaStreamSynchronize(s));
  return B200_OK;
}

int b200_bind_top(int fid, void* z, size_t n, const void* r) {
  int rc = ensure_init();
  if (rc) return rc;
  if (n < 2) return B200_OK;
  if (n & 1) return fail(B200_E_ARG, "bind_top needs an even length, got %zu", n);
  if (!z || !r) return fail(B200_E_ARG, "null pointer");
  dev_buf buf;
  size_t vec = n * 32;
  rc = buf.alloc(vec + 32);
  if (rc) return rc;
  char* d = (char*)buf.p;
  cudaStream_t s = g_dev.stream;
  CU(cudaMemcpyAsync(d, z, vec, cudaMemcpyHostToDevice, s));
  CU(cudaMemcpyAsync(d + vec, r, 32, cudaMemcpyHostToDevice, s));
  rc = b200_bind_top_dev(fid, d, n, d + vec, s);
  if (rc) return rc;
  CU(cudaMemcpyAsync(z, d, vec / 2, cudaMemcpyDeviceToHost, s));
  CU(cudaStreamSynchronize(s));
  return B200_OK;
}

}

#include "capi_poly.inc"
#include "capi_sumcheck.inc"
#include "capi_stream.inc"
```

nova_b200/csrc/capi_stream.inc:

```

namespace {

struct witness_stream {
  std::mutex mu;
  std::shared_ptr<ck_ctx> key;
  ck_ctx* target = nullptr;
  size_t n = 0, filled = 0;
  workspace ws;
  cudaStream_t side = nullptr;
  cudaEvent_t ready = nullptr;
  bool finished = false;
  ~witness_stream() {
    ws.release();
    if (ready) cudaEventDestroy(ready);
    if (side) cudaStreamDestroy(side);
  }
};
std::mutex g_wstreams_mu;
std::map<uint64_t, std::shared_ptr<witness_stream>> g_wstreams;
uint64_t g_next_wstream = 1;

std::shared_ptr<witness_stream> get_wstream(uint64_t h) {
  std::lock_guard<std::mutex> lk(g_wstreams_mu);
  auto it = g_wstreams.find(h);
  return it == g_wstreams.end() ? nullptr : it->second;
}

}

extern "C" {

int b200_ck_validate(int curve_id, const void* bases, size_t n, size_t* first_bad) {
  int rc = ensure_init();
  if (rc) return rc;
  if (curve_id < 0 || curve_id > 3) return fail(B200_E_ARG, "unknown curve id %d", curve_id);
  if (!first_bad || (n && !bases)) return fail(B200_E_ARG, "null pointer");
  if (n >= 0xFFFFFFFFull) return fail(B200_E_RANGE, "key too large for 32-bit indices");
  *first_bad = SIZE_MAX;
  if (n == 0) return B200_OK;
  cudaStream_t s = g_dev.stream;
  scratch_buf pts(s), flag(s);
  if ((rc = pts.alloc(n * 64))) return rc;
  if ((rc = flag.alloc(4))) return rc;
  CU(cudaMemcpyAsync(pts.p, bases, n * 64, cudaMemcpyHostToDevice, s));
  CU(cudaMemsetAsync(flag.p, 0xFF, 4, s));
  ops_for_field(CURVES[curve_id].base_fid)->on_curve(s, pts.p, n, CURVE_B_SMALL[curve_id], (uint32_t*)flag.p);
  count_launch(1);
  CU(cudaGetLastError());
  uint32_t bad = 0;
  CU(cudaMemcpyAsync(&bad, flag.p, 4, cudaMemcpyDeviceToHost, s));
  CU(cudaStreamSynchronize(s));
  if (bad != 0xFFFFFFFFu) *first_bad = bad;
  return B200_OK;
}

int b200_witness_begin(uint64_t ck_handle, size_t n, uint64_t* stream_handle) {
  int rc = ensure_init();
  if (rc) return rc;
  if (!stream_handle) return fail(B200_E_ARG, "null handle pointer");
  auto ck = get_ck(ck_handle);
  if (!ck) return fail(B200_E_HANDLE, "unknown key handle %llu", (unsigned long long)ck_handle);
  if (n > ck->n)
    return fail(B200_E_RANGE, "witness of %zu scalars exceeds key length %zu", n, ck->n);
  auto w = std::make_shared<witness_stream>();
  w->key = ck;
  w->target = &route(*ck, 0, n);
  w->n = n;
  rc = ensure_workspace(*w->target, w->ws, n + 1, 1);
  if (rc) return rc;
  CU(cudaStreamCreateWithFlags(&w->side, cudaStreamNonBlocking));
  CU(cudaEventCreateWithFlags(&w->ready, cudaEventDisableTiming));
  size_t K = (size_t)w->target->G * w->target->B;
  CU(cudaMemsetAsync(w->ws.counts, 0, K * 4, w->side));
  CU(cudaMemsetAsync((char*)w->ws.scalars + n * 32, 0, 32, w->side));
  std::lock_guard<std::mutex> lk(g_wstreams_mu);
  *stream_handle = g_next_wstream++;
  g_wstreams[*stream_handle] = w;
  return B200_OK;
}

int b200_witness_append(uint64_t stream_handle, const void* scalars, size_t count) {
  int rc = ensure_init();
  if (rc) return rc;
  auto w = get_wstream(stream_handle);
  if (!w) return fail(B200_E_HANDLE, "unknown witness stream %llu", (unsigned long long)stream_handle);
  if (count == 0) return B200_OK;
  if (!scalars) return fail(B200_E_ARG, "null pointer");
  std::lock_guard<std::mutex> lk(w->mu);
  if (w->finished) return fail(B200_E_ARG, "witness stream already finished");
  if (w->filled + count > w->n)
    return fail(B200_E_RANGE, "append of %zu scalars overflows the witness (%zu of %zu filled)", count,
                w->filled, w->n);
  CU(cudaMemcpyAsync((char*)w->ws.scalars + w->filled * 32, scalars, count * 32, cudaMemcpyHostToDevice,
                     w->side));
  const field_ops* sops = ops_for_field(CURVES[w->target->curve].scalar_fid);
  msm_plan p = make_plan(*w->target, w->ws, 0, w->n + 1);
  sops->digits_range(w->side, w->ws.scalars, w->filled, w->filled + count, p);
  count_launch(1);
  CU(cudaGetLastError());
  w->filled += count;
  return B200_OK;
}

int b200_witness_finish(uint64_t stream_handle, const void* r_or_null, void* out, void** d_witness_or_null) {
  int rc = ensure_init();
  if (rc) return rc;
  auto w = get_wstream(stream_handle);
  if (!w) return fail(B200_E_HANDLE, "unknown witness stream %llu", (unsigned long long)stream_handle);
  if (!out) return fail(B200_E_ARG, "null pointer");
  std::lock_guard<std::mutex> lk(w->mu);
  if (w->finished) return fail(B200_E_ARG, "witness stream already finished");
  ck_ctx& t = *w->target;
  if (r_or_null && !t.has_h) return fail(B200_E_ARG, "key was registered without a blinding generator");
  if (r_or_null)
    CU(cudaMemcpyAsync((char*)w->ws.scalars + w->n * 32, r_or_null, 32, cudaMemcpyHostToDevice, w->side));
  if (w->filled < w->n)
    CU(cudaMemsetAsync((char*)w->ws.scalars + w->filled * 32, 0, (w->n - w->filled) * 32, w->side));
  const field_ops* sops = ops_for_field(CURVES[t.curve].scalar_fid);
  msm_plan p = make_plan(t, w->ws, 0, w->n + 1);
  sops->digits_range(w->side, w->ws.scalars, w->filled, w->n + 1, p);
  w->filled = w->n;
  count_launch(1);
  CU(cudaEventRecord(w->ready, w->side));
  cudaStream_t s = g_dev.stream;
  CU(cudaStreamWaitEvent(s, w->ready, 0));
  rc = enqueue_msm(t, w->ws, 0, w->ws.scalars, w->n + 1, w->ws.d_out, s, 0, t.has_h,
                   true);
  if (rc) return rc;
  CU(cudaMemcpyAsync(w->ws.h_out, w->ws.d_out, 96, cudaMemcpyDeviceToHost, s));
  CU(cudaStreamSynchronize(s));
  memcpy(out, w->ws.h_out, 96);
  if (d_witness_or_null) *d_witness_or_null = w->ws.scalars;
  w->finished = true;
  return B200_OK;
}

int b200_witness_reset(uint64_t stream_handle) {
  int rc = ensure_init();
  if (rc) return rc;
  auto w = get_wstream(stream_handle);
  if (!w) return fail(B200_E_HANDLE, "unknown witness stream %llu", (unsigned long long)stream_handle);
  std::lock_guard<std::mutex> lk(w->mu);
  CU(cudaEventRecord(w->ready, g_dev.stream));
  CU(cudaStreamWaitEvent(w->side, w->ready, 0));
  size_t K = (size_t)w->target->G * w->target->B;
  CU(cudaMemsetAsync(w->ws.counts, 0, K * 4, w->side));
  CU(cudaMemsetAsync((char*)w->ws.scalars + w->n * 32, 0, 32, w->side));
  w->filled = 0;
  w->finished = false;
  return B200_OK;
}

int b200_witness_release(uint64_t stream_handle) {
  std::shared_ptr<witness_stream> w;
  {
    std::lock_guard<std::mutex> lk(g_wstreams_mu);
    auto it = g_wstreams.find(stream_handle);
    if (it == g_wstreams.end())
      return fail(B200_E_HANDLE, "unknown witness stream %llu", (unsigned long long)stream_handle);
    w = it->second;
    g_wstreams.erase(it);
  }
  std::lock_guard<std::mutex> lk(w->mu);
  cudaSetDevice(g_dev.device);
  if (w->side) cudaStreamSynchronize(w->side);
  return B200_OK;
}

}
```

nova_b200/csrc/msm_common.cu:

```cuda
#include "ops.cuh"
#include "msm_kernels.cuh"

namespace nova {

constexpr int SCAN_BLOCK = 1024;
constexpr int SCAN_ITEMS = 4;

__global__ void __launch_bounds__(SCAN_BLOCK) k_scan_block(const uint32_t* __restrict__ in,
                                                           uint32_t* __restrict__ out,
                                                           uint32_t* __restrict__ blocksums,
                                                           uint32_t K) {
  __shared__ uint32_t warp_tot[32];
  uint32_t base = blockIdx.x * (SCAN_BLOCK * SCAN_ITEMS) + threadIdx.x * SCAN_ITEMS;
  uint32_t v[SCAN_ITEMS], tot = 0;
#pragma unroll
  for (int k = 0; k < SCAN_ITEMS; k++) {
    v[k] = (base + k < K) ? in[base + k] : 0;
    tot += v[k];
  }
  uint32_t inc = tot;
  int lane = threadIdx.x & 31, wid = threadIdx.x >> 5;
#pragma unroll
  for (int d = 1; d < 32; d <<= 1) {
    uint32_t o = __shfl_up_sync(0xffffffffu, inc, d);
    if (lane >= d) inc += o;
  }
  if (lane == 31) warp_tot[wid] = inc;
  __syncthreads();
  if (wid == 0) {
    uint32_t w = warp_tot[lane];
    uint32_t winc = w;
#pragma unroll
    for (int d = 1; d < 32; d <<= 1) {
      uint32_t o = __shfl_up_sync(0xffffffffu, winc, d);
      if (lane >= d) winc += o;
    }
    warp_tot[lane] = winc - w;
    if (lane == 31) blocksums[blockIdx.x] = winc;
  }
  __syncthreads();
  uint32_t excl = inc - tot + warp_tot[wid];
#pragma unroll
  for (int k = 0; k < SCAN_ITEMS; k++) {
    if (base + k < K) out[base + k] = excl;
    excl += v[k];
  }
}

__global__ void __launch_bounds__(SCAN_BLOCK) k_scan_sums(uint32_t* blocksums, uint32_t nblocks) {
  __shared__ uint32_t warp_tot[32];
  uint32_t base = threadIdx.x * SCAN_ITEMS;
  uint32_t v[SCAN_ITEMS], tot = 0;
#pragma unroll
  for (int k = 0; k < SCAN_ITEMS; k++) {
    v[k] = (base + k < nblocks) ? blocksums[base + k] : 0;
    tot += v[k];
  }
  uint32_t inc = tot;
  int lane = threadIdx.x & 31, wid = threadIdx.x >> 5;
#pragma unroll
  for (int d = 1; d < 32; d <<= 1) {
    uint32_t o = __shfl_up_sync(0xffffffffu, inc, d);
    if (lane >= d) inc += o;
  }
  if (lane == 31) warp_tot[wid] = inc;
  __syncthreads();
  if (wid == 0) {
    uint32_t w = warp_tot[lane], winc = w;
#pragma unroll
    for (int d = 1; d < 32; d <<= 1) {
      uint32_t o = __shfl_up_sync(0xffffffffu, winc, d);
      if (lane >= d) winc += o;
    }
    warp_tot[lane] = winc - w;
  }
  __syncthreads();
  uint32_t excl = inc - tot + warp_tot[wid];
#pragma unroll
  for (int k = 0; k < SCAN_ITEMS; k++) {
    if (base + k < nblocks) blocksums[base + k] = excl;
    excl += v[k];
  }
}

__global__ void __launch_bounds__(256) k_scan_add(uint32_t* __restrict__ start,
                                                  uint32_t* __restrict__ cursor,
                                                  const uint32_t* __restrict__ counts,
                                                  const uint32_t* __restrict__ blocksums,
                                                  uint32_t K, uint32_t* __restrict__ heavy,
                                                  uint32_t heavy_min, uint32_t heavy_cap) {
  uint32_t i = blockIdx.x * blockDim.x + threadIdx.x;
  if (i >= K) return;
  uint32_t s = start[i] + blocksums[i / (SCAN_BLOCK * SCAN_ITEMS)];
  start[i] = s;
  cursor[i] = s;
  uint32_t cnt = counts[i];
  if (i == K - 1) start[K] = s + cnt;
  if (cnt > heavy_min) {
    uint32_t slot = atomicAdd(&heavy[0], 1u);
    if (slot < heavy_cap) heavy[1 + slot] = i;
  }
}

__global__ void __launch_bounds__(256) k_digits_small(const void* __restrict__ scalars,
                                                      int elem_bytes, size_t n, int c, int W, int G,
                                                      uint32_t B, int32_t* __restrict__ digits,
                                                      uint32_t* __restrict__ counts) {
  size_t i = (size_t)blockIdx.x * blockDim.x + threadIdx.x;
  const bool live = i < n;
  uint64_t v64 = 0;
  if (live) switch (elem_bytes) {
    case 1: v64 = ((const uint8_t*)scalars)[i]; break;
    case 2: v64 = ((const uint16_t*)scalars)[i]; break;
    case 4: v64 = ((const uint32_t*)scalars)[i]; break;
    default: v64 = ((const uint64_t*)scalars)[i]; break;
  }
  const uint32_t half = 1u << (c - 1);
  const uint64_t mask = (1ull << c) - 1;
  uint32_t carry = 0;
  for (int w = 0; w < W; w++) {
    int bit = w * c;
    uint32_t v = bit < 64 ? (uint32_t)((v64 >> bit) & mask) : 0u;
    v += carry;
    int32_t dgt;
    if (v > half) {
      dgt = (int32_t)v - (int32_t)(1u << c);
      carry = 1;
    } else {
      dgt = (int32_t)v;
      carry = 0;
    }
    if (live) digits[(size_t)w * n + i] = dgt;
    uint32_t key = NO_KEY;
    if (dgt != 0) {
      uint32_t mag = dgt < 0 ? (uint32_t)(-dgt) : (uint32_t)dgt;
      key = (uint32_t)(w % G) * B + (mag - 1);
    }
    count_key(counts, key);
  }
}

__global__ void __launch_bounds__(256) k_scatter(const int32_t* __restrict__ digits, size_t n,
                                                 int W, int G, uint32_t B, size_t n_ck,
                                                 size_t base_offset, size_t blind_i, size_t h_index,
                                                 uint32_t* __restrict__ cursor,
                                                 uint64_t* __restrict__ entries) {
  size_t i = (size_t)blockIdx.x * blockDim.x + threadIdx.x;
  int w = blockIdx.y;
  int32_t dgt = i < n ? digits[(size_t)w * n + i] : 0;
  uint32_t sign = dgt < 0 ? 1u : 0u;
  uint32_t mag = sign ? (uint32_t)(-dgt) : (uint32_t)dgt;
  uint32_t key = dgt != 0 ? (uint32_t)(w % G) * B + (mag - 1) : NO_KEY;
  uint32_t pos;
  if (!warp_has_repeats(key)) {
    if (key == NO_KEY) return;
    pos = atomicAdd(&cursor[key], 1u);
  } else {
    unsigned peers = __match_any_sync(0xFFFFFFFFu, key);
    if (key == NO_KEY) return;
    unsigned lane = threadIdx.x & 31u, leader = (unsigned)(__ffs(peers) - 1);
    uint32_t base = 0;
    if (lane == leader) base = atomicAdd(&cursor[key], (uint32_t)__popc(peers));
    base = __shfl_sync(peers, base, leader);
    pos = base + (uint32_t)__popc(peers & ((1u << lane) - 1u));
  }
  size_t bi = (i == blind_i) ? h_index : base_offset + i;
  uint32_t idx = (uint32_t)((size_t)(w / G) * n_ck + bi);
  entries[pos] = ((uint64_t)key << 32) | ((uint64_t)sign << 31) | idx;
}

void msm_scan(cudaStream_t s, const msm_plan& p) {
  uint32_t K = (uint32_t)p.G * p.B;
  uint32_t per_block = SCAN_BLOCK * SCAN_ITEMS;
  uint32_t nblocks = (K + per_block - 1) / per_block;
  k_scan_block<<<nblocks, SCAN_BLOCK, 0, s>>>(p.counts, p.start, p.blocksums, K);
  k_scan_sums<<<1, SCAN_BLOCK, 0, s>>>(p.blocksums, nblocks);
  k_scan_add<<<(K + 255) / 256, 256, 0, s>>>(p.start, p.cursor, p.counts, p.blocksums, K, p.heavy,
                                             p.heavy_min, p.heavy_cap);
}

void msm_digits_small(cudaStream_t s, const void* scalars, int elem_bytes, const msm_plan& p) {
  k_digits_small<<<(unsigned)((p.n + 255) / 256), 256, 0, s>>>(scalars, elem_bytes, p.n, p.c, p.W,
                                                               p.G, p.B, p.digits, p.counts);
}

void msm_scatter(cudaStream_t s, const msm_plan& p) {
  dim3 grid((unsigned)((p.n + 255) / 256), (unsigned)p.W);
  k_scatter<<<grid, 256, 0, s>>>(p.digits, p.n, p.W, p.G, p.B, p.n_ck, p.base_offset, p.blind_i,
                                 p.h_index, p.cursor,
                                 p.entries);
}

}
```

nova_b200/csrc/msm_kernels.cuh:

```cuda
#pragma once
#include <cuda_runtime.h>
#include "curve29.cuh"
#include "coop.cuh"

namespace nova {

constexpr uint32_t KEY_INVALID = 0xffffffffu;

constexpr int MSM_PEER_MAX = 8;
constexpr size_t MSM_PEER_FLAGS_OFF = (size_t)2 * MSM_PEER_MAX * 128;
constexpr size_t MSM_PEER_ERR_OFF = MSM_PEER_FLAGS_OFF + (size_t)MSM_PEER_MAX * 8;
constexpr size_t MSM_PEER_BUF_BYTES = MSM_PEER_ERR_OFF + 8;
struct msm_peer {
  int world = 1, rank = 0;
  unsigned long long epoch = 0;
  void* buf[MSM_PEER_MAX] = {};
};

struct msm_plan {
  size_t n;
  size_t n_ck;
  size_t base_offset;
  size_t blind_i;
  size_t h_index;
  int c;
  int W;
  int G;
  uint32_t B;
  int L;
  int m;
  int32_t* digits;
  uint32_t* counts;
  uint32_t* start;
  uint32_t* cursor;
  uint64_t* entries;
  void* buckets;
  void* parts;
  uint32_t* pkeys;
  void* rparts;
  uint32_t* blocksums;
  uint32_t* heavy;
  uint32_t heavy_min;
  uint32_t heavy_cap;
  void* hparts;
  msm_peer peer;
};

constexpr uint32_t NO_KEY = 0xFFFFFFFFu;
__device__ __forceinline__ bool warp_has_repeats(uint32_t key) {
  uint32_t next = __shfl_down_sync(0xFFFFFFFFu, key, 1);
  return __any_sync(0xFFFFFFFFu, key != NO_KEY && key == next && (threadIdx.x & 31u) != 31u);
}
__device__ __forceinline__ void count_key(uint32_t* counts, uint32_t key) {
  if (!warp_has_repeats(key)) {
    if (key != NO_KEY) atomicAdd(&counts[key], 1u);
    return;
  }
  unsigned peers = __match_any_sync(0xFFFFFFFFu, key);
  if (key != NO_KEY && (threadIdx.x & 31u) == (unsigned)(__ffs(peers) - 1))
    atomicAdd(&counts[key], (uint32_t)__popc(peers));
}

template <class S>
__global__ void __launch_bounds__(256) k_digits(const void* __restrict__ scalars, size_t i0, size_t i1,
                                                size_t n, int c, int W, int G, uint32_t B,
                                                int32_t* __restrict__ digits,
                                                uint32_t* __restrict__ counts) {
  size_t i = i0 + (size_t)blockIdx.x * blockDim.x + threadIdx.x;
  const bool live = i < i1;
  fe_t s = live ? fe_from_mont<S>(fe_load(scalars, i)) : fe_zero<S>();
  uint32_t p[8], t[8];
  load_p<S>(p);
  bool neg = false;
  if (!fe_is_zero(s)) {
    sub8(t, p, s.l);
    uint32_t d[8];
    uint32_t lt = sub8(d, t, s.l);
    if (lt) {
      neg = true;
#pragma unroll
      for (int k = 0; k < 8; k++) s.l[k] = t[k];
    }
  }
  const uint32_t half = 1u << (c - 1);
  const uint32_t mask = (1u << c) - 1;
  uint32_t carry = 0;
  for (int w = 0; w < W; w++) {
    int bit = w * c;
    int limb = bit >> 5, sh = bit & 31;
    uint32_t v = 0;
    if (limb < 8) {
      uint64_t two = s.l[limb];
      if (limb + 1 < 8) two |= (uint64_t)s.l[limb + 1] << 32;
      v = (uint32_t)(two >> sh) & mask;
    }
    v += carry;
    int32_t dgt;
    if (v > half) {
      dgt = (int32_t)v - (int32_t)(1u << c);
      carry = 1;
    } else {
      dgt = (int32_t)v;
      carry = 0;
    }
    if (neg) dgt = -dgt;
    if (live) digits[(size_t)w * n + i] = dgt;
    uint32_t key = NO_KEY;
    if (dgt != 0) {
      uint32_t mag = dgt < 0 ? (uint32_t)(-dgt) : (uint32_t)dgt;
      key = (uint32_t)(w % G) * B + (mag - 1);
    }
    count_key(counts, key);
  }
}

template <class F>
__global__ void __launch_bounds__(128) k_accumulate(const uint64_t* __restrict__ entries,
                                                    const uint32_t* __restrict__ start, uint32_t K,
                                                    const void* __restrict__ tables, int L,
                                                    void* __restrict__ buckets,
                                                    void* __restrict__ parts,
                                                    uint32_t* __restrict__ pkeys) {
  using PA = msm_arith<F>;
  const uint32_t M = start[K];
  size_t t = (size_t)blockIdx.x * blockDim.x + threadIdx.x;
  size_t seg_start = t * (size_t)L;
  if (seg_start >= M) return;
  size_t seg_end = seg_start + L < M ? seg_start + L : M;

  typename PA::pt acc = PA::identity();
  uint64_t ent = entries[seg_start];
  uint32_t cur_key = (uint32_t)(ent >> 32);
  bool first = true;
  typename PA::aff pt = PA::load_table(tables, (uint32_t)ent & 0x7fffffffu);
  for (size_t e = seg_start; e < seg_end; e++) {
    uint32_t key = (uint32_t)(ent >> 32);
    bool sign = (ent >> 31) & 1;
    typename PA::aff cur = pt;
    if (e + 1 < seg_end) {
      ent = entries[e + 1];
      pt = PA::load_table(tables, (uint32_t)ent & 0x7fffffffu);
    }
    if (key != cur_key) {
      if (first) {
        PA::store(parts, 2 * t, acc);
        pkeys[2 * t] = cur_key;
        first = false;
      } else {
        PA::store(buckets, cur_key, acc);
      }
      acc = PA::identity();
      cur_key = key;
    }
    if (!PA::aff_is_identity(cur)) {
      if (sign) PA::neg_aff(cur);
      PA::madd(acc, cur);
    }
  }
  if (first) {
    PA::store(parts, 2 * t, acc);
    pkeys[2 * t] = cur_key;
    pkeys[2 * t + 1] = KEY_INVALID;
  } else {
    PA::store(parts, 2 * t + 1, acc);
    pkeys[2 * t + 1] = cur_key;
  }
}

constexpr int ACC_TMA_DEPTH = 3;
#if defined(__CUDACC__) && !defined(NOVA_MSM_ARITH29)
NOVA_D uint32_t smem_addr_u32(const void* p) { return (uint32_t)__cvta_generic_to_shared(p); }
NOVA_D void mbar_init(uint64_t* bar, uint32_t arrivals) {
  asm volatile("mbarrier.init.shared::cta.b64 [%0], %1;" ::"r"(smem_addr_u32(bar)), "r"(arrivals) : "memory");
}
NOVA_D void mbar_arrive_expect_tx(uint64_t* bar, uint32_t bytes) {
  asm volatile("mbarrier.arrive.expect_tx.shared::cta.b64 _, [%0], %1;" ::"r"(smem_addr_u32(bar)), "r"(bytes)
               : "memory");
}
NOVA_D void mbar_wait_parity(uint64_t* bar, uint32_t parity) {
  asm volatile(
      "{\n"
      ".reg .pred p;\n"
      "MBAR_WAIT:\n"
      "mbarrier.try_wait.parity.shared::cta.b64 p, [%0], %1;\n"
      "@p bra MBAR_DONE;\n"
      "bra MBAR_WAIT;\n"
      "MBAR_DONE:\n"
      "}\n" ::"r"(smem_addr_u32(bar)),
      "r"(parity)
      : "memory");
}
NOVA_D void tma_load_1d(void* smem_dst, const void* gmem_src, uint32_t bytes, uint64_t* bar) {
  asm volatile("cp.async.bulk.shared::cluster.global.mbarrier::complete_tx::bytes [%0], [%1], %2, [%3];" ::"r"(
                   smem_addr_u32(smem_dst)),
               "l"(gmem_src), "r"(bytes), "r"(smem_addr_u32(bar))
               : "memory");
}

template <class F>
__global__ void __launch_bounds__(128) k_accumulate_tma(const uint64_t* __restrict__ entries,
                                                        const uint32_t* __restrict__ start, uint32_t K,
                                                        const void* __restrict__ tables, int L,
                                                        void* __restrict__ buckets, void* __restrict__ parts,
                                                        uint32_t* __restrict__ pkeys) {
  using PA = msm_arith<F>;
  static_assert(sizeof(typename PA::aff) == 64, "one table point = one 64-byte bulk copy");
  __shared__ __align__(128) uint4 slots[ACC_TMA_DEPTH][128][4];
  __shared__ __align__(8) uint64_t bars[4][ACC_TMA_DEPTH];
  const uint32_t M = start[K];
  const int warp = threadIdx.x >> 5, lane = threadIdx.x & 31;
  if (lane == 0)
    for (int st = 0; st < ACC_TMA_DEPTH; st++) mbar_init(&bars[warp][st], 1);
  asm volatile("fence.mbarrier_init.release.cluster;" ::: "memory");
  __syncwarp();
  size_t t = (size_t)blockIdx.x * blockDim.x + threadIdx.x;
  size_t seg_start = t * (size_t)L;
  const bool active = seg_start < M;
  size_t seg_end = seg_start + L < M ? seg_start + L : M;
  const int len = active ? (int)(seg_end - seg_start) : 0;
  int wlen = len;
#pragma unroll
  for (int d = 16; d > 0; d >>= 1) {
    int o = __shfl_xor_sync(0xffffffffu, wlen, d);
    wlen = o > wlen ? o : wlen;
  }
  if (wlen == 0) return;

  auto issue = [&](int j) -> uint64_t {
    const bool mine = j < len;
    uint64_t ent = mine ? entries[seg_start + j] : 0;
    const int st = j % ACC_TMA_DEPTH;
    unsigned who = __ballot_sync(0xffffffffu, mine);
    if (who) {
      if (lane == (int)(__ffs(who) - 1)) mbar_arrive_expect_tx(&bars[warp][st], 64u * (uint32_t)__popc(who));
      __syncwarp();
      if (mine)
        tma_load_1d(&slots[st][threadIdx.x][0],
                    (const char*)tables + (size_t)((uint32_t)ent & 0x7fffffffu) * 64, 64, &bars[warp][st]);
    }
    return ent;
  };

  static_assert(ACC_TMA_DEPTH == 3, "the rotation below is written for three stages");
  uint64_t e0 = issue(0), e1 = issue(1);

  typename PA::pt acc = PA::identity();
  uint32_t cur_key = active ? (uint32_t)(e0 >> 32) : 0;
  bool first = true;
  int st = 0;
  uint32_t phase = 0;
#pragma unroll 1
  for (int k = 0; k < wlen; k++) {
    const uint64_t e2 = issue(k + 2);
    if (__ballot_sync(0xffffffffu, k < len)) mbar_wait_parity(&bars[warp][st], phase);
    if (k < len) {
      const uint64_t ent = e0;
      const uint32_t key = (uint32_t)(ent >> 32);
      const bool sign = (ent >> 31) & 1;
      typename PA::aff cur;
      {
        const uint4* sp = &slots[st][threadIdx.x][0];
        uint4 a = sp[0], b = sp[1], c = sp[2], d = sp[3];
        cur.x.l[0] = a.x; cur.x.l[1] = a.y; cur.x.l[2] = a.z; cur.x.l[3] = a.w;
        cur.x.l[4] = b.x; cur.x.l[5] = b.y; cur.x.l[6] = b.z; cur.x.l[7] = b.w;
        cur.y.l[0] = c.x; cur.y.l[1] = c.y; cur.y.l[2] = c.z; cur.y.l[3] = c.w;
        cur.y.l[4] = d.x; cur.y.l[5] = d.y; cur.y.l[6] = d.z; cur.y.l[7] = d.w;
      }
      if (key != cur_key) {
        if (first) {
          PA::store(parts, 2 * t, acc);
          pkeys[2 * t] = cur_key;
          first = false;
        } else {
          PA::store(buckets, cur_key, acc);
        }
        acc = PA::identity();
        cur_key = key;
      }
      if (!PA::aff_is_identity(cur)) {
        if (sign) PA::neg_aff(cur);
        PA::madd(acc, cur);
      }
    }
    e0 = e1;
    e1 = e2;
    if (++st == ACC_TMA_DEPTH) {
      st = 0;
      phase ^= 1u;
    }
  }
  if (!active) return;
  if (first) {
    PA::store(parts, 2 * t, acc);
    pkeys[2 * t] = cur_key;
    pkeys[2 * t + 1] = KEY_INVALID;
  } else {
    PA::store(parts, 2 * t + 1, acc);
    pkeys[2 * t + 1] = cur_key;
  }
}
#endif

template <class F>
__global__ void __launch_bounds__(128) k_fixup(const uint32_t* __restrict__ start, uint32_t K,
                                               int L, uint32_t heavy_min, int G,
                                               const void* __restrict__ parts,
                                               const uint32_t* __restrict__ pkeys,
                                               void* __restrict__ buckets) {
  using PA = msm_arith<F>;
  uint32_t gtid = blockIdx.x * blockDim.x + threadIdx.x;
  uint32_t key = gtid / G, sub = gtid % G;
  bool live = key < K;
  uint32_t s0 = 0, s1 = 0;
  if (live) {
    s0 = start[key];
    s1 = start[key + 1];
    live = s1 != s0 && s1 - s0 <= heavy_min;
  }
  typename PA::pt acc = PA::identity();
  bool found = false;
  if (live) {
    size_t j0 = 2 * ((size_t)s0 / L), j1 = 2 * (((size_t)s1 - 1) / L) + 1;
    for (size_t j = j0 + sub; j <= j1; j += G) {
      if (pkeys[j] == key) {
        typename PA::pt o = PA::load(parts, j);
        PA::add(acc, o);
        found = true;
      }
    }
  }
  for (int d = G / 2; d > 0; d >>= 1) {
    typename PA::pt o = PA::shfl_down(acc, d, G);
    bool of = __shfl_down_sync(0xffffffffu, (int)found, d, G) != 0;
    if (sub + d < (uint32_t)G && of) {
      PA::add(acc, o);
      found = true;
    }
  }
  if (live && sub == 0 && found) PA::store(buckets, key, acc);
}

constexpr int HEAVY_SPLIT = 16;
template <class F>
__global__ void __launch_bounds__(256) k_fixup_heavy1(const uint32_t* __restrict__ start, int L,
                                                      const uint32_t* __restrict__ heavy,
                                                      const void* __restrict__ parts,
                                                      const uint32_t* __restrict__ pkeys,
                                                      void* __restrict__ hparts) {
  using PA = msm_arith<F>;
  __shared__ typename msm_arith<F>::pt sm[256];
  const uint32_t nitems = heavy[0] * HEAVY_SPLIT;
  for (uint32_t it = blockIdx.x; it < nitems; it += gridDim.x) {
    uint32_t h = it / HEAVY_SPLIT, sl = it % HEAVY_SPLIT;
    uint32_t key = heavy[1 + h];
    size_t s0 = 2 * ((size_t)start[key] / L);
    size_t s1 = 2 * (((size_t)start[key + 1] - 1) / L) + 2;
    size_t per = (s1 - s0 + HEAVY_SPLIT - 1) / HEAVY_SPLIT;
    size_t lo = s0 + sl * per, hi = lo + per < s1 ? lo + per : s1;
    typename PA::pt acc = PA::identity();
    for (size_t k = lo + threadIdx.x; k < hi; k += blockDim.x) {
      if (pkeys[k] == key) {
        typename PA::pt o = PA::load(parts, k);
        PA::add(acc, o);
      }
    }
    sm[threadIdx.x] = acc;
    __syncthreads();
    for (int s = blockDim.x / 2; s > 0; s >>= 1) {
      if ((int)threadIdx.x < s) {
        typename PA::pt a = sm[threadIdx.x];
        PA::add(a, sm[threadIdx.x + s]);
        sm[threadIdx.x] = a;
      }
      __syncthreads();
    }
    if (threadIdx.x == 0) PA::store(hparts, it, sm[0]);
    __syncthreads();
  }
}

template <class F>
__global__ void __launch_bounds__(32) k_fixup_heavy2(const uint32_t* __restrict__ heavy,
                                                     const void* __restrict__ hparts,
                                                     void* __restrict__ buckets) {
  using PA = msm_arith<F>;
  static_assert(HEAVY_SPLIT <= 32 && (HEAVY_SPLIT & (HEAVY_SPLIT - 1)) == 0, "one warp joins the slices");
  const uint32_t nheavy = heavy[0];
  for (uint32_t h = blockIdx.x; h < nheavy; h += gridDim.x) {
    typename PA::pt acc = PA::identity();
    if (threadIdx.x < HEAVY_SPLIT) acc = PA::load(hparts, (size_t)h * HEAVY_SPLIT + threadIdx.x);
    for (int d = HEAVY_SPLIT / 2; d > 0; d >>= 1) {
      typename PA::pt o = PA::shfl_down(acc, d, 32);
      if ((int)threadIdx.x < d) PA::add(acc, o);
    }
    if (threadIdx.x == 0) PA::store(buckets, heavy[1 + h], acc);
  }
}

template <class F>
__global__ void __launch_bounds__(128) k_reduce1(const uint32_t* __restrict__ start, uint32_t B,
                                                 int G, int m, const void* __restrict__ buckets,
                                                 void* __restrict__ rparts) {
  using PA = msm_arith<F>;
  uint32_t T = B / m;
  uint32_t tid = blockIdx.x * blockDim.x + threadIdx.x;
  if (tid >= T * (uint32_t)G) return;
  uint32_t g = tid / T, k = tid % T;
  uint32_t lo = k * m;
  typename PA::pt run = PA::identity(), tot = PA::identity();
  for (int b = m - 1; b >= 0; b--) {
    uint32_t key = g * B + lo + b;
    if (start[key + 1] > start[key]) {
      typename PA::pt bk = PA::load(buckets, key);
      PA::add(run, bk);
    }
    PA::add(tot, run);
  }
  if (lo != 0) {
    typename PA::pt sc = PA::mul_small(run, lo);
    PA::add(tot, sc);
  }
  PA::store(rparts, tid, tot);
}

template <class F>
__global__ void __launch_bounds__(256) k_reduce2(const void* __restrict__ rparts, uint32_t T, int G,
                                                 int c, void* __restrict__ out_jac) {
  using PA = msm_arith<F>;
  __shared__ typename msm_arith<F>::pt sm[256];
  typename PA::pt total = PA::identity();
  for (int g = G - 1; g >= 0; g--) {
    typename PA::pt acc = PA::identity();
    for (uint32_t k = threadIdx.x; k < T; k += blockDim.x) {
      typename PA::pt o = PA::load(rparts, (size_t)g * T + k);
      PA::add(acc, o);
    }
    sm[threadIdx.x] = acc;
    __syncthreads();
    for (int s = blockDim.x / 2; s > 0; s >>= 1) {
      if ((int)threadIdx.x < s) {
        typename PA::pt a = sm[threadIdx.x];
        PA::add(a, sm[threadIdx.x + s]);
        sm[threadIdx.x] = a;
      }
      __syncthreads();
    }
    if (threadIdx.x == 0) {
      if (g != G - 1)
        for (int d = 0; d < c; d++) PA::dbl(total);
      PA::add(total, sm[0]);
    }
    __syncthreads();
  }
  if (threadIdx.x == 0) {
    fe_t X, Y, Z;
    PA::to_jacobian_std(total, X, Y, Z);
    fe_store(out_jac, 0, X);
    fe_store(out_jac, 1, Y);
    fe_store(out_jac, 2, Z);
  }
}

constexpr int RED_NSPLIT = 4;
template <class F>
__global__ void __launch_bounds__(128) k_red_digits(const uint32_t* __restrict__ start, uint32_t B,
                                                    int bits, const void* __restrict__ buckets,
                                                    void* __restrict__ parts ) {
  using PA = msm_arith<F>;
  __shared__ typename PA::pt sm[128];
  const int nd = (bits + 3) / 4;
  const int x = blockIdx.x, d = blockIdx.y / 16, v = blockIdx.y % 16, g = blockIdx.z;
  const int width = bits - 4 * d < 4 ? bits - 4 * d : 4;
  typename PA::pt acc = PA::identity();
  if (v < (1 << width)) {
    const uint32_t count = B >> width;
    const uint32_t per = (count + RED_NSPLIT - 1) / RED_NSPLIT;
    const uint32_t lo = x * per, hi = lo + per < count ? lo + per : count;
    const uint32_t lowmask = (1u << (4 * d)) - 1;
    for (uint32_t i = lo + threadIdx.x; i < hi; i += blockDim.x) {
      uint32_t b = ((i >> (4 * d)) << (4 * d + width)) | ((uint32_t)v << (4 * d)) | (i & lowmask);
      uint32_t key = g * B + b;
      if (start[key + 1] > start[key]) {
        typename PA::pt o = PA::load(buckets, key);
        PA::add(acc, o);
      }
    }
  }
  sm[threadIdx.x] = acc;
  __syncthreads();
  for (int s = blockDim.x / 2; s > 0; s >>= 1) {
    if ((int)threadIdx.x < s) {
      typename PA::pt a = sm[threadIdx.x];
      PA::add(a, sm[threadIdx.x + s]);
      sm[threadIdx.x] = a;
    }
    __syncthreads();
  }
  if (threadIdx.x == 0) PA::store(parts, (((size_t)g * nd + d) * 16 + v) * RED_NSPLIT + x, sm[0]);
}

template <class F>
__global__ void __launch_bounds__(256) k_red_final(const void* __restrict__ parts, int G, int bits, int c,
                                                   void* __restrict__ out_jac) {
  using PA = msm_arith<F>;
  __shared__ typename PA::pt sm[8];
  const int nd = (bits + 3) / 4;
  const int w = threadIdx.x >> 5, lane = threadIdx.x & 31;
  typename PA::pt total = PA::identity();
  for (int g = G - 1; g >= 0; g--) {
    typename PA::pt S = PA::identity();
    if (w < nd && lane < 16)
      for (int x = 0; x < RED_NSPLIT; x++) {
        typename PA::pt o = PA::load(parts, (((size_t)g * nd + w) * 16 + lane) * RED_NSPLIT + x);
        PA::add(S, o);
      }
    for (int d = 1; d < 16; d <<= 1) {
      typename PA::pt o = PA::shfl_down(S, d, 16);
      if (lane < 16 && lane + d < 16) PA::add(S, o);
    }
    typename PA::pt T0 = S;
    typename PA::pt X = (lane >= 1 && lane < 16) ? S : PA::identity();
    for (int d = 8; d > 0; d >>= 1) {
      typename PA::pt o = PA::shfl_down(X, d, 16);
      if (lane < 16 && lane + d < 16) PA::add(X, o);
    }
    if (lane == 0 && w < nd) {
      for (int k = 0; k < 4 * w; k++) PA::dbl(X);
      if (w == 0) PA::add(X, T0);
      sm[w] = X;
    }
    __syncthreads();
    if (threadIdx.x == 0) {
      if (g != G - 1)
        for (int k = 0; k < c; k++) PA::dbl(total);
      for (int k = 0; k < nd; k++) PA::add(total, sm[k]);
    }
    __syncthreads();
  }
  if (threadIdx.x == 0) {
    fe_t X, Y, Z;
    PA::to_jacobian_std(total, X, Y, Z);
    fe_store(out_jac, 0, X);
    fe_store(out_jac, 1, Y);
    fe_store(out_jac, 2, Z);
  }
}

#if !defined(NOVA_MSM_ARITH29)
NOVA_D xyzz_t xyzz_load_q(const void* base, size_t idx) { return xyzz_load(base, idx); }

template <class F>
__global__ void __launch_bounds__(128) k_fixup_q(const uint32_t* __restrict__ start, uint32_t K, int L,
                                                 uint32_t heavy_min, const void* __restrict__ parts,
                                                 const uint32_t* __restrict__ pkeys,
                                                 void* __restrict__ buckets) {
  quad_comm_dev cm;
  uint32_t key = (blockIdx.x * blockDim.x + threadIdx.x) >> 2;
  bool live = key < K;
  uint32_t s0 = 0, s1 = 0;
  if (live) {
    s0 = start[key];
    s1 = start[key + 1];
    live = s1 != s0 && s1 - s0 <= heavy_min;
  }
  size_t j0 = live ? 2 * ((size_t)s0 / L) : 1, j1 = live ? 2 * (((size_t)s1 - 1) / L) + 1 : 0;
  xyzz_t acc = xyzz_identity<F>();
  bool found = false;
  for (size_t j = j0; j <= j1; j++) {
    if (pkeys[j] == key) {
      xyzz_t o = xyzz_load(parts, j);
      coop_add<F>(acc, o, cm);
      found = true;
    }
  }
  if (live && found && cm.lane() == 0) xyzz_store(buckets, key, acc);
}

template <class F>
__global__ void __launch_bounds__(256) k_red_digits_q(const uint32_t* __restrict__ start, uint32_t B,
                                                      int bits, const void* __restrict__ buckets,
                                                      void* __restrict__ parts ) {
  __shared__ xyzz_t sm[64];
  quad_comm_dev cm;
  const int nd = (bits + 3) / 4;
  const int nsplit = gridDim.x;
  const int x = blockIdx.x, d = blockIdx.y / 16, v = blockIdx.y % 16, g = blockIdx.z;
  const int width = bits - 4 * d < 4 ? bits - 4 * d : 4;
  const int quad = threadIdx.x >> 2;
  xyzz_t acc = xyzz_identity<F>();
  if (v < (1 << width)) {
    const uint32_t count = B >> width;
    const uint32_t per = (count + nsplit - 1) / nsplit;
    const uint32_t lo = x * per, hi = lo + per < count ? lo + per : count;
    const uint32_t lowmask = (1u << (4 * d)) - 1;
    for (uint32_t i = lo + quad; i < hi; i += 64) {
      uint32_t b = ((i >> (4 * d)) << (4 * d + width)) | ((uint32_t)v << (4 * d)) | (i & lowmask);
      uint32_t key = g * B + b;
      if (start[key + 1] > start[key]) {
        xyzz_t o = xyzz_load(buckets, key);
        coop_add<F>(acc, o, cm);
      }
    }
  }
  if (cm.lane() == 0) sm[quad] = acc;
  __syncthreads();
  for (int s = 32; s > 0; s >>= 1) {
    if (quad < s) {
      xyzz_t o = sm[quad + s];
      coop_add<F>(acc, o, cm);
    }
    __syncthreads();
    if (quad < s && cm.lane() == 0) sm[quad] = acc;
    __syncthreads();
  }
  if (threadIdx.x == 0) xyzz_store(parts, (((size_t)g * nd + d) * 16 + v) * nsplit + x, acc);
}

template <class F>
__global__ void __launch_bounds__(256) k_red_merge_q(const void* __restrict__ parts, int nd, int nsplit,
                                                     void* __restrict__ merged) {
  __shared__ xyzz_t sm[64];
  quad_comm_dev cm;
  const int dv = blockIdx.x, g = blockIdx.y;
  const int quad = threadIdx.x >> 2;
  const size_t base = ((size_t)g * nd * 16 + dv) * nsplit;
  xyzz_t acc = xyzz_identity<F>();
  for (int x = quad; x < nsplit; x += 64) {
    xyzz_t o = xyzz_load(parts, base + x);
    coop_add<F>(acc, o, cm);
  }
  if (cm.lane() == 0) sm[quad] = acc;
  __syncthreads();
  for (int s = 32; s > 0; s >>= 1) {
    if (quad < s && s < nsplit) {
      xyzz_t o = sm[quad + s];
      coop_add<F>(acc, o, cm);
    }
    __syncthreads();
    if (quad < s && cm.lane() == 0) sm[quad] = acc;
    __syncthreads();
  }
  if (threadIdx.x == 0) xyzz_store(merged, (size_t)g * nd * 16 + dv, acc);
}

template <class F>
__global__ void __launch_bounds__(256) k_red_level_q(const uint32_t* __restrict__ start_or_null, uint32_t key_base_stride,
                                                     const void* __restrict__ X, uint32_t N, int nsplit,
                                                     void* __restrict__ parts ,
                                                     void* __restrict__ next ) {
  __shared__ xyzz_t sm[64];
  quad_comm_dev cm;
  const int quad = threadIdx.x >> 2;
  const uint32_t g = blockIdx.z;
  const uint32_t groups = N >> 4;
  const size_t xbase = (size_t)g * N;
  auto load = [&](uint32_t i) -> xyzz_t {
    if (start_or_null) {
      const uint32_t key = g * key_base_stride + i;
      if (start_or_null[key + 1] == start_or_null[key]) return xyzz_identity<F>();
    }
    return xyzz_load(X, xbase + i);
  };
  if (blockIdx.y == 16) {
    const uint32_t j = blockIdx.x * 16 + (quad >> 2);
    const int sub = quad & 3;
    const bool live = j < groups;
    xyzz_t acc = xyzz_identity<F>();
    if (live) {
      acc = load(16 * j + 4 * sub);
      for (int k = 1; k < 4; k++) {
        xyzz_t o = load(16 * j + 4 * sub + k);
        coop_add<F>(acc, o, cm);
      }
    }
    if (cm.lane() == 0) sm[quad] = acc;
    __syncthreads();
    if (live && sub < 2) {
      xyzz_t o = sm[quad + 2];
      coop_add<F>(acc, o, cm);
    }
    __syncthreads();
    if (sub < 2 && cm.lane() == 0) sm[quad] = acc;
    __syncthreads();
    if (live && sub == 0) {
      xyzz_t o = sm[quad + 1];
      coop_add<F>(acc, o, cm);
      if (cm.lane() == 0) xyzz_store(next, (size_t)g * groups + j, acc);
    }
    return;
  }
  if ((int)blockIdx.x >= nsplit) return;
  const uint32_t v = blockIdx.y;
  const uint32_t per = (groups + nsplit - 1) / nsplit;
  const uint32_t lo = blockIdx.x * per, hi = lo + per < groups ? lo + per : groups;
  xyzz_t acc = xyzz_identity<F>();
  for (uint32_t j = lo + quad; j < hi; j += 64) {
    xyzz_t o = load(16 * j + v);
    coop_add<F>(acc, o, cm);
  }
  if (cm.lane() == 0) sm[quad] = acc;
  __syncthreads();
  for (int s = 32; s > 0; s >>= 1) {
    if (quad < s) {
      xyzz_t o = sm[quad + s];
      coop_add<F>(acc, o, cm);
    }
    __syncthreads();
    if (quad < s && cm.lane() == 0) sm[quad] = acc;
    __syncthreads();
  }
  if (threadIdx.x == 0) xyzz_store(parts, ((size_t)g * 16 + v) * nsplit + blockIdx.x, acc);
}

struct red_levels {
  int nd;
  int nsplit[8];
  unsigned parts_off[8];
  unsigned top_off;
  unsigned top_n;
};
template <class F>
__global__ void __launch_bounds__(256) k_red_merge_levels_q(const void* __restrict__ scratch, const red_levels lv,
                                                            const uint32_t* __restrict__ start, uint32_t B,
                                                            const void* __restrict__ buckets, int G,
                                                            void* __restrict__ merged) {
  __shared__ xyzz_t sm[64];
  quad_comm_dev cm;
  const int d = blockIdx.x >> 4, v = blockIdx.x & 15, g = blockIdx.y;
  const int quad = threadIdx.x >> 2;
  xyzz_t acc = xyzz_identity<F>();
  if (d == lv.nd - 1) {
    if (threadIdx.x == 0) {
      if ((unsigned)v < lv.top_n) {
        if (lv.top_off == 0xFFFFFFFFu) {
          uint32_t key = (uint32_t)g * B + v;
          if (start[key + 1] > start[key]) acc = xyzz_load(buckets, key);
        } else {
          acc = xyzz_load(scratch, (size_t)lv.top_off + (size_t)g * lv.top_n + v);
        }
      }
      xyzz_store(merged, ((size_t)g * lv.nd + d) * 16 + v, acc);
    }
    return;
  }
  const int nsplit = lv.nsplit[d];
  const size_t base = (size_t)lv.parts_off[d] + ((size_t)g * 16 + v) * nsplit;
  for (int x = quad; x < nsplit; x += 64) {
    xyzz_t o = xyzz_load(scratch, base + x);
    coop_add<F>(acc, o, cm);
  }
  if (cm.lane() == 0) sm[quad] = acc;
  __syncthreads();
  for (int s = 32; s > 0; s >>= 1) {
    if (quad < s && s < nsplit) {
      xyzz_t o = sm[quad + s];
      coop_add<F>(acc, o, cm);
    }
    __syncthreads();
    if (quad < s && cm.lane() == 0) sm[quad] = acc;
    __syncthreads();
  }
  if (threadIdx.x == 0) xyzz_store(merged, ((size_t)g * lv.nd + d) * 16 + v, acc);
}

template <class F>
NOVA_D xyzz_t peer_exchange_sum(const xyzz_t& mine, const msm_peer& peer, xyzz_t* sm ,
                                const quad_comm_dev& cm) {
  const int tid = threadIdx.x, quad = tid >> 2;
  const int set = (int)(peer.epoch & 1ull);
  if (tid == 0) sm[0] = mine;
  __syncthreads();
  if (tid < peer.world) {
    char* dst = (char*)peer.buf[tid];
    xyzz_store(dst, (size_t)set * MSM_PEER_MAX + peer.rank, sm[0]);
    __threadfence_system();
    volatile unsigned long long* flag = (volatile unsigned long long*)(dst + MSM_PEER_FLAGS_OFF) + peer.rank;
    *flag = peer.epoch;
    char* loc = (char*)peer.buf[peer.rank];
    const unsigned long long* lflag = (const unsigned long long*)(loc + MSM_PEER_FLAGS_OFF) + tid;
    unsigned long long seen = 0;
    long long t0 = clock64();
    for (;;) {
      asm volatile("ld.acquire.sys.global.u64 %0, [%1];" : "=l"(seen) : "l"(lflag) : "memory");
      if (seen >= peer.epoch) break;
      if (clock64() - t0 > (1ll << 32)) {
        *(volatile unsigned long long*)(loc + MSM_PEER_ERR_OFF) = peer.epoch;
        break;
      }
    }
  }
  __syncthreads();
  xyzz_t acc = xyzz_identity<F>();
  if (quad < peer.world) acc = xyzz_load((const char*)peer.buf[peer.rank], (size_t)set * MSM_PEER_MAX + quad);
  for (int s = MSM_PEER_MAX / 2; s > 0; s >>= 1) {
    if (quad < 2 * s && cm.lane() == 0) sm[quad] = acc;
    __syncthreads();
    if (quad < s && quad + s < peer.world) {
      xyzz_t o = sm[quad + s];
      coop_add<F>(acc, o, cm);
    }
    __syncthreads();
  }
  return acc;
}

template <class F>
__global__ void __launch_bounds__(384) k_red_final_q(const void* __restrict__ merged, int G, int bits, int c,
                                                     void* __restrict__ out_jac, const msm_peer peer) {
  __shared__ xyzz_t sm[96];
  quad_comm_dev cm;
  const int nd = (bits + 3) / 4;
  const int quad = threadIdx.x >> 2;
  const int d = quad >> 4, v = quad & 15;
  xyzz_t total = xyzz_identity<F>();
  for (int g = G - 1; g >= 0; g--) {
    xyzz_t acc = xyzz_identity<F>();
    if (d < nd) acc = xyzz_load(merged, ((size_t)g * nd + d) * 16 + v);
    if (cm.lane() == 0) sm[quad] = acc;
    __syncthreads();
    for (int dd = 1; dd < 16; dd <<= 1) {
      bool have = v + dd < 16;
      xyzz_t o = xyzz_identity<F>();
      if (have) o = sm[quad + dd];
      __syncthreads();
      if (have) coop_add<F>(acc, o, cm);
      if (cm.lane() == 0) sm[quad] = acc;
      __syncthreads();
    }
    xyzz_t t0 = acc;
    if (v == 0) acc = xyzz_identity<F>();
    if (cm.lane() == 0) sm[quad] = acc;
    __syncthreads();
    for (int s = 8; s > 0; s >>= 1) {
      bool have = v < s;
      xyzz_t o = xyzz_identity<F>();
      if (have) o = sm[quad + s];
      __syncthreads();
      if (have) coop_add<F>(acc, o, cm);
      if (cm.lane() == 0) sm[quad] = acc;
      __syncthreads();
    }
    if (v == 0 && d < nd) {
      for (int i = 0; i < 4 * d; i++) coop_dbl<F>(acc, cm);
      if (d == 0) coop_add<F>(acc, t0, cm);
      if (cm.lane() == 0) sm[quad] = acc;
    }
    __syncthreads();
    if (quad == 0) {
      if (g != G - 1)
        for (int i = 0; i < c; i++) coop_dbl<F>(total, cm);
      for (int dd = 0; dd < nd; dd++) {
        xyzz_t o = sm[dd * 16];
        coop_add<F>(total, o, cm);
      }
    }
    __syncthreads();
  }
  if (peer.world > 1) total = peer_exchange_sum<F>(total, peer, sm, cm);
  if (threadIdx.x == 0) {
    fe_t X, Y, Z;
    xyzz_to_jacobian<F>(total, X, Y, Z);
    fe_store(out_jac, 0, X);
    fe_store(out_jac, 1, Y);
    fe_store(out_jac, 2, Z);
  }
}
#endif

template <class F>
__global__ void k_jacobian_sum(const void* __restrict__ pts, int k, void* __restrict__ out_jac) {
  using PA = msm_arith<F>;
  if (blockIdx.x != 0 || threadIdx.x != 0) return;
  typename PA::pt acc = PA::identity();
  for (int i = 0; i < k; i++) {
    fe_t X = fe_load(pts, 3 * (size_t)i), Y = fe_load(pts, 3 * (size_t)i + 1),
         Z = fe_load(pts, 3 * (size_t)i + 2);
    typename PA::pt p = PA::from_jacobian_std(X, Y, Z);
    PA::add(acc, p);
  }
  fe_t X, Y, Z;
  PA::to_jacobian_std(acc, X, Y, Z);
  fe_store(out_jac, 0, X);
  fe_store(out_jac, 1, Y);
  fe_store(out_jac, 2, Z);
}

#if !defined(NOVA_MSM_ARITH29)
template <class F>
__global__ void __launch_bounds__(32) k_jacobian_sum_q(const void* __restrict__ pts, int k, void* __restrict__ out_jac) {
  __shared__ xyzz_t sm[8];
  quad_comm_dev cm;
  const int quad = threadIdx.x >> 2;
  xyzz_t acc = xyzz_identity<F>();
  for (int i = quad; i < k; i += 8) {
    fe_t X = fe_load(pts, 3 * (size_t)i), Y = fe_load(pts, 3 * (size_t)i + 1), Z = fe_load(pts, 3 * (size_t)i + 2);
    xyzz_t p = xyzz_identity<F>();
    if (!fe_is_zero(Z)) {
      p.x = X;
      p.y = Y;
      p.zz = fe_sqr<F>(Z);
      p.zzz = fe_mul<F>(p.zz, Z);
    }
    coop_add<F>(acc, p, cm);
  }
  for (int s = 4; s > 0; s >>= 1) {
    if (quad < 2 * s && cm.lane() == 0) sm[quad] = acc;
    __syncwarp();
    if (quad < s) {
      xyzz_t o = sm[quad + s];
      coop_add<F>(acc, o, cm);
    }
    __syncwarp();
  }
  if (threadIdx.x == 0) {
    fe_t X, Y, Z;
    xyzz_to_jacobian<F>(acc, X, Y, Z);
    fe_store(out_jac, 0, X);
    fe_store(out_jac, 1, Y);
    fe_store(out_jac, 2, Z);
  }
}
#endif

template <class F>
__global__ void __launch_bounds__(128) k_index_bases(void* __restrict__ bases, size_t n,
                                                     const void* __restrict__ gen, uint64_t k0) {
  size_t i = (size_t)blockIdx.x * blockDim.x + threadIdx.x;
  if (i >= n) return;
  fe_t gx = fe_load(gen, 0), gy = fe_load(gen, 1);
  uint64_t k = k0 + i;
  xyzz_t acc = xyzz_identity<F>();
  for (int b = 63; b >= 0; b--) {
    xyzz_dbl<F>(acc);
    if ((k >> b) & 1) xyzz_madd<F>(acc, gx, gy);
  }
  fe_t x = fe_zero<F>(), y = fe_zero<F>();
  if (!xyzz_is_identity(acc)) {
    fe_t iz3 = fe_inv<F>(acc.zzz);
    fe_t iz2 = fe_mul<F>(fe_sqr<F>(acc.zz), fe_sqr<F>(iz3));
    x = fe_mul<F>(acc.x, iz2);
    y = fe_mul<F>(acc.y, iz3);
  }
  fe_store(bases, 2 * i, x);
  fe_store(bases, 2 * i + 1, y);
}

template <class F>
__global__ void __launch_bounds__(128) k_scalar_bases(void* __restrict__ bases, size_t n,
                                                      const void* __restrict__ gen,
                                                      const void* __restrict__ scalars) {
  size_t i = (size_t)blockIdx.x * blockDim.x + threadIdx.x;
  if (i >= n) return;
  fe_t gx = fe_load(gen, 0), gy = fe_load(gen, 1);
  fe_t k = fe_load(scalars, i);
  xyzz_t acc = xyzz_identity<F>();
  for (int b = 255; b >= 0; b--) {
    xyzz_dbl<F>(acc);
    if ((k.l[b >> 5] >> (b & 31)) & 1u) xyzz_madd<F>(acc, gx, gy);
  }
  fe_t x = fe_zero<F>(), y = fe_zero<F>();
  if (!xyzz_is_identity(acc)) {
    fe_t iz3 = fe_inv<F>(acc.zzz);
    fe_t iz2 = fe_mul<F>(fe_sqr<F>(acc.zz), fe_sqr<F>(iz3));
    x = fe_mul<F>(acc.x, iz2);
    y = fe_mul<F>(acc.y, iz3);
  }
  fe_store(bases, 2 * i, x);
  fe_store(bases, 2 * i + 1, y);
}

template <class F>
__global__ void __launch_bounds__(128) k_expand_key(void* __restrict__ tables, size_t n_ck,
                                                    int ntables, int shift) {
  using PA = msm_arith<F>;
  size_t i = (size_t)blockIdx.x * blockDim.x + threadIdx.x;
  if (i >= n_ck) return;
  fe_t bx = fe_load_rw(tables, 2 * i), by = fe_load_rw(tables, 2 * i + 1);
  if (fe_is_zero(bx) && fe_is_zero(by)) {
    for (int t = 1; t < ntables; t++) PA::store_table_identity(tables, (size_t)t * n_ck + i);
    return;
  }
  typename PA::aff p = PA::from_std_affine(bx, by);
  PA::store_table(tables, i, p);
  for (int t = 1; t < ntables; t++) {
    typename PA::pt q = PA::identity();
    PA::madd(q, p);
    for (int d = 0; d < shift; d++) PA::dbl(q);
    p = PA::to_affine(q);
    PA::store_table(tables, (size_t)t * n_ck + i, p);
  }
}

template <class F>
__global__ void __launch_bounds__(256) k_on_curve(const void* __restrict__ pts, size_t n, int b_small,
                                                  uint32_t* __restrict__ first_bad) {
  const fe_t b = fe_from_small_int<F>(b_small);
  for (size_t i = (size_t)blockIdx.x * blockDim.x + threadIdx.x; i < n; i += (size_t)gridDim.x * blockDim.x) {
    affine_t p;
    p.x = fe_load(pts, 2 * i);
    p.y = fe_load(pts, 2 * i + 1);
    if (!affine_valid_raw<F>(p, b)) atomicMin(first_bad, (uint32_t)i);
  }
}

}
```

nova_b200/csrc/ops.cuh:

```cuda
#pragma once
#include <cstdlib>
#include <cuda_runtime.h>
#include <cstddef>
#include <cstdint>

namespace nova {

struct msm_plan;
struct multi_args;
struct poly_multi_args;
struct scb_tail_args;

struct field_ops {
  int field_id;
  void (*digits)(cudaStream_t, const void* scalars, const msm_plan&);
  void (*expand_key)(cudaStream_t, void* tables, size_t n_ck, int ntables, int shift);
  void (*accumulate)(cudaStream_t, const void* tables, const msm_plan&);
  void (*fixup)(cudaStream_t, const msm_plan&);
  void (*reduce)(cudaStream_t, const msm_plan&, void* out_jac);
  void (*sum_points)(cudaStream_t, const void* tables, const uint32_t* idx_or_null, size_t n,
                     void* scratch_xyzz, void* out_jac);
  void (*jacobian_sum)(cudaStream_t, const void* pts, int k, void* out_jac);
  void (*index_bases)(cudaStream_t, void* bases, size_t n, const void* gen_affine, uint64_t k0);
  void (*cross_term)(cudaStream_t, const void* az, const void* bz, const void* cz, const void* e1,
                     const void* e2_or_null, const void* u, size_t n, void* t);
  void (*axpy)(cudaStream_t, const void* a, const void* b, const void* r, size_t n, void* out);
  void (*vec_add)(cudaStream_t, const void* a, const void* b, size_t n, void* out);
  void (*bind_top)(cudaStream_t, void* z, size_t n, const void* r);
  void (*bind_top_multi)(cudaStream_t, void* const* zs, int k, size_t n, const void* r);
  void (*vec_mul)(cudaStream_t, const void* a, const void* b, size_t n, void* out);
  void (*logup_hash)(cudaStream_t, const void* val, const void* addr_or_null, const void* gamma,
                     const void* r, size_t n, void* out);
  void (*fold_halves)(cudaStream_t, const void* v, size_t half, const void* x_lo, const void* x_hi, void* out);
  void (*ipa_scalars)(cudaStream_t, const void* a, const void* w, size_t n, size_t nk, void* sL, void* sR);
  void (*ipa_weights)(cudaStream_t, void* w, size_t n, size_t nk, const void* r, const void* r_inv);
  void (*fill_one)(cudaStream_t, void* w, size_t n);
  void (*sc_reduce)(cudaStream_t, int form, const void* A, const void* B, const void* C, size_t count,
                    size_t half, const void* eq_left, const void* eq_right, int shift, size_t id_mul,
                    size_t id_add, void* scratch, void* out);
  void (*eq_small)(cudaStream_t, const void* r, int ell, void* out);
  void (*eq_outer)(cudaStream_t, const void* left, const void* right, int right_bits, size_t n,
                   void* out);
  void (*batch_invert)(cudaStream_t, const void* in, size_t n, void* out, int* zero_flag);
  void (*rlc)(cudaStream_t, const void* const* polys, const size_t* lens, int k, const void* coeffs,
              size_t n, void* out);
  void (*kzg_fold)(cudaStream_t, const void* p, const void* x, size_t half, void* out);
  void (*poly_eval)(cudaStream_t, const void* f, size_t n, const void* us, int nu, void* scratch,
                    void* evals);
  void (*poly_div)(cudaStream_t, const void* f, size_t n, const void* u, void* scratch, void* out);
  void (*spmv_classify)(cudaStream_t, const void* vals, size_t nnz, int8_t* codes);
  void (*spmv)(cudaStream_t, const uint32_t* indptr, const uint32_t* cols, const int8_t* codes,
               const void* vals, size_t rows, const void* z1, const void* z2_or_null, void* o1,
               void* o2_or_null);
  void (*spmv_t)(cudaStream_t, const uint32_t* tptr, const uint32_t* trow, const uint32_t* tperm,
                 const int8_t* codes, const void* vals, size_t cols, size_t out_len, const void* rx,
                 void* out);
  void (*sc_round)(cudaStream_t, int kind, void* state, const void* res, const void* tau,
                   const void* tau_inv, const void* pending, uint32_t pending_len, int absorb_label,
                   int squeeze_label, void* out_poly, void* out_r);
  void (*fe_inv_each)(cudaStream_t, const void* in, size_t n, void* out);
  void (*digits_range)(cudaStream_t, const void* scalars, size_t i0, size_t i1, const msm_plan&);
  void (*sc_round_batched)(cudaStream_t, const void* desc, void* state, const void* sums, const void* pending,
                           uint32_t pending_len, int absorb_label, int squeeze_label, void* out_poly, void* out_r);
  void (*on_curve)(cudaStream_t, const void* pts, size_t n, int b_small, uint32_t* first_bad);
  void (*powers_canonical)(cudaStream_t, const void* u_mont, size_t n, void* out);
  void (*scalar_bases)(cudaStream_t, void* bases, size_t n, const void* gen_affine, const void* scalars_canonical);
  void (*poseidon_ro)(cudaStream_t, int t, int r_f, int r_p, const void* rc, const void* mds, const void* elems, uint32_t n,
                      const void* tag_canonical, int num_bits, int start_with_one, void* out);
  void (*to_mont)(cudaStream_t, const void* in_canonical, size_t n, void* out);
  void (*exchange_identity)(cudaStream_t, const msm_plan&, void* out_jac);
  void (*sc_round_batched_fused)(cudaStream_t, const void* desc, void* state, const void* partials, int nblocks,
                                 int nsums, const void* pending, uint32_t pending_len, int absorb_label,
                                 int squeeze_label, void* out_poly, void* out_r);
  int (*sc_reduce_multi_partials)(cudaStream_t, const multi_args&, void* scratch);
  void (*gather_heads)(cudaStream_t, void* const* zs, int k, void* out);
  void (*poly_eval_small_multi)(cudaStream_t, const poly_multi_args&, const void* us, int nu, void* evals);
  void (*eq_prefix_tables)(cudaStream_t, const void* taus, int hi, int K, void* out);
  void (*sc_reduce_multi)(cudaStream_t, const multi_args&, void* scratch, void* out);
  void (*scb_tail)(cudaStream_t, const scb_tail_args&, void* state, void* sums, const void* pending,
                   uint32_t pending_len, int absorb_label, int squeeze_label, void* polys, void* rs);
};
constexpr int NUM_SMS = 132;
constexpr int SC_MAX_BLOCKS = NUM_SMS * 4;
constexpr int EQ_PREFIX_MAX_K = 12;
constexpr int SC_MULTI_BLOCKS = NUM_SMS * 2;
inline size_t sc_multi_scratch_elems(int nsums) { return (size_t)nsums * SC_MULTI_BLOCKS * 3; }
inline bool sc_segmented_enabled() {
  static const bool on = [] {
    const char* e = getenv("NOVA_B200_SC_SEG");
    return e != nullptr && e[0] == '1';
  }();
  return on;
}
constexpr size_t POLY_EVAL_SCRATCH_ELEMS = (size_t)3 * (1 + SC_MAX_BLOCKS + 256) + (size_t)3 * SC_MAX_BLOCKS;
constexpr int POLY_CHUNK_HOST = 64;
inline size_t poly_div_scratch_elems(size_t n) {
  size_t t1 = (n + POLY_CHUNK_HOST - 1) / POLY_CHUNK_HOST, t2 = (t1 + POLY_CHUNK_HOST - 1) / POLY_CHUNK_HOST;
  return 2 * t1 + 2 * t2 + 8;
}

extern const field_ops OPS_BN254_FR, OPS_BN254_FQ, OPS_PALLAS_FP, OPS_PALLAS_FQ;

inline const field_ops* ops_for_field(int fid) {
  switch (fid) {
    case 0: return &OPS_BN254_FR;
    case 1: return &OPS_BN254_FQ;
    case 2: return &OPS_PALLAS_FP;
    case 3: return &OPS_PALLAS_FQ;
    default: return nullptr;
  }
}

void msm_scan(cudaStream_t, const msm_plan&);
void msm_scatter(cudaStream_t, const msm_plan&);
void msm_digits_small(cudaStream_t, const void* scalars, int elem_bytes, const msm_plan&);

}
```

nova_b200/csrc/ops_impl.cuh:

```cuda
#pragma once
#include "ops.cuh"
#include "msm_kernels.cuh"
#include "field_kernels.cuh"
#include "poly_kernels.cuh"
#include "transcript.cuh"
#include "transcript_batched.cuh"
#include "poseidon.cuh"
#include "sumcheck_tail.cuh"

namespace nova {

inline int stream_grid(size_t n, int block, int waves = 8) {
  size_t need = (n + block - 1) / block;
  size_t cap = (size_t)NUM_SMS * waves;
  size_t g = need < cap ? need : cap;
  return (int)(g == 0 ? 1 : g);
}

template <class F>
__global__ void __launch_bounds__(128) k_sum_points1(const void* __restrict__ tables,
                                                     const uint32_t* __restrict__ idx, size_t n,
                                                     void* __restrict__ partial) {
  size_t tid = (size_t)blockIdx.x * blockDim.x + threadIdx.x;
  size_t nthreads = (size_t)gridDim.x * blockDim.x;
  using PA = msm_arith<F>;
  typename PA::pt acc = PA::identity();
  for (size_t i = tid; i < n; i += nthreads) {
    typename PA::aff p = PA::load_table(tables, idx ? idx[i] : i);
    if (!PA::aff_is_identity(p)) PA::madd(acc, p);
  }
  PA::store(partial, tid, acc);
}

template <class F>
struct ops_impl {
  static void digits(cudaStream_t s, const void* scalars, const msm_plan& p) {
    digits_range(s, scalars, 0, p.n, p);
  }
  static void digits_range(cudaStream_t s, const void* scalars, size_t i0, size_t i1, const msm_plan& p) {
    if (i1 <= i0) return;
    int block = 256;
    int grid = (int)((i1 - i0 + block - 1) / block);
    k_digits<F><<<grid, block, 0, s>>>(scalars, i0, i1, p.n, p.c, p.W, p.G, p.B, p.digits, p.counts);
  }
  static void expand_key(cudaStream_t s, void* tables, size_t n_ck, int ntables, int shift) {
    int block = 128;
    int grid = (int)((n_ck + block - 1) / block);
    k_expand_key<F><<<grid, block, 0, s>>>(tables, n_ck, ntables, shift);
  }
  static void accumulate(cudaStream_t s, const void* tables, const msm_plan& p) {
    uint32_t K = (uint32_t)p.G * p.B;
    size_t max_entries = p.n * (size_t)p.W;
    size_t nseg = (max_entries + p.L - 1) / p.L;
    int block = 128;
    int grid = (int)((nseg + block - 1) / block);
#if !defined(NOVA_MSM_ARITH29)
    static const bool use_tma = [] {
      const char* e = getenv("NOVA_B200_ACC_TMA");
      return e != nullptr && e[0] == '1';
    }();
    if (use_tma) {
      k_accumulate_tma<F><<<grid, block, 0, s>>>(p.entries, p.start, K, tables, p.L, p.buckets, p.parts, p.pkeys);
      return;
    }
#endif
    k_accumulate<F><<<grid, block, 0, s>>>(p.entries, p.start, K, tables, p.L, p.buckets, p.parts,
                                           p.pkeys);
  }
  static void fixup(cudaStream_t s, const msm_plan& p) {
    uint32_t K = (uint32_t)p.G * p.B;
    size_t entries = p.n * (size_t)p.W;
    size_t ppk = entries / ((size_t)K * p.L) + 1;
    int G = 1;
    while (G < 32 && (size_t)G * 8 < ppk) G <<= 1;
    if (ppk <= 16) G = 1;
    size_t threads = (size_t)K * G;
#if !defined(NOVA_MSM_ARITH29)
    if (G == 1) {
      threads = (size_t)K * 4;
      k_fixup_q<F><<<(unsigned)((threads + 127) / 128), 128, 0, s>>>(p.start, K, p.L, p.heavy_min, p.parts,
                                                                     p.pkeys, p.buckets);
    } else
#endif
      k_fixup<F><<<(unsigned)((threads + 127) / 128), 128, 0, s>>>(p.start, K, p.L, p.heavy_min, G, p.parts,
                                                                   p.pkeys, p.buckets);
    k_fixup_heavy1<F><<<NUM_SMS * 4, 256, 0, s>>>(p.start, p.L, p.heavy, p.parts, p.pkeys, p.hparts);
    k_fixup_heavy2<F><<<NUM_SMS, 32, 0, s>>>(p.heavy, p.hparts, p.buckets);
  }
  static void index_bases(cudaStream_t s, void* bases, size_t n, const void* gen, uint64_t k0) {
    k_index_bases<F><<<(unsigned)((n + 127) / 128), 128, 0, s>>>(bases, n, gen, k0);
  }
  static void jacobian_sum(cudaStream_t s, const void* pts, int k, void* out_jac) {
#if !defined(NOVA_MSM_ARITH29)
    k_jacobian_sum_q<F><<<1, 32, 0, s>>>(pts, k, out_jac);
#else
    k_jacobian_sum<F><<<1, 32, 0, s>>>(pts, k, out_jac);
#endif
  }
  static void reduce(cudaStream_t s, const msm_plan& p, void* out_jac) {
    int bits = p.c - 1;
#if !defined(NOVA_MSM_ARITH29)
    static const int flat_mode = [] {
      const char* e = getenv("NOVA_B200_RED_FLAT");
      return e == nullptr ? -1 : (e[0] == '1' ? 1 : 0);
    }();
    static const int hier_bits = [] {
      const char* e = getenv("NOVA_B200_RED_HIER_BITS");
      return e ? atoi(e) : 18;
    }();
    const bool flat = flat_mode == 1 || (flat_mode == -1 && bits < hier_bits);
    if (bits >= 1 && bits <= 24 && !flat) {
      red_levels lv{};
      lv.nd = (bits + 3) / 4;
      size_t off = 0;
      uint32_t N = p.B;
      const void* X = p.buckets;
      for (int l = 0; l < lv.nd - 1; l++) {
        const uint32_t groups = N >> 4;
        int nsplit = (int)((groups + 511) / 512);
        if (nsplit < 1) nsplit = 1;
        lv.nsplit[l] = nsplit;
        lv.parts_off[l] = (unsigned)off;
        char* parts = (char*)p.rparts + off * 128;
        off += (size_t)p.G * 16 * nsplit;
        char* next = (char*)p.rparts + off * 128;
        const unsigned next_off = (unsigned)off;
        off += (size_t)p.G * groups;
        unsigned gx = (unsigned)nsplit, gb = (groups + 15) / 16;
        dim3 grid(gx > gb ? gx : gb, 17u, (unsigned)p.G);
        k_red_level_q<F><<<grid, 256, 0, s>>>(l == 0 ? p.start : nullptr, p.B, X, N, nsplit, parts, next);
        X = next;
        N = groups;
        lv.top_off = next_off;
      }
      if (lv.nd == 1) lv.top_off = 0xFFFFFFFFu;
      lv.top_n = N;
      char* merged = (char*)p.rparts + off * 128;
      dim3 g2((unsigned)(lv.nd * 16), (unsigned)p.G);
      k_red_merge_levels_q<F><<<g2, 256, 0, s>>>(p.rparts, lv, p.start, p.B, p.buckets, p.G, merged);
      k_red_final_q<F><<<1, 384, 0, s>>>(merged, p.G, bits, p.c, out_jac, p.peer);
      return;
    }
    if (bits >= 1 && bits <= 24) {
      int nd = (bits + 3) / 4;
      uint32_t count = p.B >> (bits < 4 ? bits : 4);
      int nsplit = (int)((count + 255) / 256);
      if (nsplit < 1) nsplit = 1;
      if (nsplit > 4096) nsplit = 4096;
      char* merged = (char*)p.rparts + (size_t)p.G * nd * 16 * nsplit * 128;
      dim3 g1((unsigned)nsplit, (unsigned)(nd * 16), (unsigned)p.G);
      k_red_digits_q<F><<<g1, 256, 0, s>>>(p.start, p.B, bits, p.buckets, p.rparts);
      dim3 g2((unsigned)(nd * 16), (unsigned)p.G);
      k_red_merge_q<F><<<g2, 256, 0, s>>>(p.rparts, nd, nsplit, merged);
      k_red_final_q<F><<<1, 384, 0, s>>>(merged, p.G, bits, p.c, out_jac, p.peer);
      return;
    }
#endif
    if (bits >= 1 && bits <= 24) {
      int nd = (bits + 3) / 4;
      dim3 g1(RED_NSPLIT, (unsigned)(nd * 16), (unsigned)p.G);
      k_red_digits<F><<<g1, 128, 0, s>>>(p.start, p.B, bits, p.buckets, p.rparts);
      k_red_final<F><<<1, 256, 0, s>>>(p.rparts, p.G, bits, p.c, out_jac);
      return;
    }
    uint32_t T = p.B / p.m;
    int block = 128;
    int grid = (int)(((size_t)T * p.G + block - 1) / block);
    k_reduce1<F><<<grid, block, 0, s>>>(p.start, p.B, p.G, p.m, p.buckets, p.rparts);
    k_reduce2<F><<<1, 256, 0, s>>>(p.rparts, T, p.G, p.c, out_jac);
  }
  static void sum_points(cudaStream_t s, const void* tables, const uint32_t* idx, size_t n,
                         void* scratch, void* out_jac) {
    int block = 128, grid = NUM_SMS;
    k_sum_points1<F><<<grid, block, 0, s>>>(tables, idx, n, scratch);
    k_reduce2<F><<<1, 256, 0, s>>>(scratch, (uint32_t)(grid * block), 1, 0, out_jac);
  }
  static void cross_term(cudaStream_t s, const void* az, const void* bz, const void* cz,
                         const void* e1, const void* e2, const void* u, size_t n, void* t) {
    k_cross_term<F><<<stream_grid(n, 256), 256, 0, s>>>(az, bz, cz, e1, e2, u, n, t);
  }
  static void axpy(cudaStream_t s, const void* a, const void* b, const void* r, size_t n,
                   void* out) {
    k_axpy<F><<<stream_grid(n, 256), 256, 0, s>>>(a, b, r, n, out);
  }
  static void vec_add(cudaStream_t s, const void* a, const void* b, size_t n, void* out) {
    k_vec_add<F><<<stream_grid(n, 256), 256, 0, s>>>(a, b, n, out);
  }
  static void vec_mul(cudaStream_t s, const void* a, const void* b, size_t n, void* out) {
    k_vec_mul<F><<<stream_grid(n, 256), 256, 0, s>>>(a, b, n, out);
  }
  static void logup_hash(cudaStream_t s, const void* val, const void* addr, const void* gamma,
                         const void* r, size_t n, void* out) {
    k_logup_hash<F><<<stream_grid(n, 256), 256, 0, s>>>(val, addr, gamma, r, n, out);
  }
  static void bind_top(cudaStream_t s, void* z, size_t n, const void* r) {
    k_bind_top<F><<<stream_grid(n / 2, 256), 256, 0, s>>>(z, n / 2, r);
  }
  static void bind_top_multi(cudaStream_t s, void* const* zs, int k, size_t n, const void* r) {
    bind_multi_args a{};
    for (int i = 0; i < k; i++) a.z[i] = zs[i];
    int gx = stream_grid(n / 2, 256, 8);
    int per = (NUM_SMS * 8 + k - 1) / k;
    if (gx > per) gx = per < 1 ? 1 : per;
    k_bind_top_multi<F><<<dim3((unsigned)gx, (unsigned)k), 256, 0, s>>>(a, n / 2, r);
  }
  static void fold_halves(cudaStream_t s, const void* v, size_t half, const void* x_lo, const void* x_hi,
                          void* out) {
    k_fold_halves<F><<<stream_grid(half, 256), 256, 0, s>>>(v, half, x_lo, x_hi, out);
  }
  static void ipa_scalars(cudaStream_t s, const void* a, const void* w, size_t n, size_t nk, void* sL,
                          void* sR) {
    k_ipa_scalars<F><<<stream_grid(n, 256), 256, 0, s>>>(a, w, n, nk, sL, sR);
  }
  static void ipa_weights(cudaStream_t s, void* w, size_t n, size_t nk, const void* r, const void* r_inv) {
    k_ipa_weights<F><<<stream_grid(n, 256), 256, 0, s>>>(w, n, nk, r, r_inv);
  }
  static void fill_one(cudaStream_t s, void* w, size_t n) {
    k_fill_one<F><<<stream_grid(n, 256), 256, 0, s>>>(w, n);
  }
  template <int FORM>
  static void sc_launch(cudaStream_t s, const void* A, const void* B, const void* C, size_t count,
                        size_t half, const void* eq_left, const void* eq_right, int shift,
                        size_t id_mul, size_t id_add, void* scratch, void* out) {
    constexpr int NOUT = sc_form_nout(FORM);
    sc_form<F, FORM> f;
    f.A = A;
    f.B = B;
    f.C = C;
    f.h = half;
    f.eq.left = eq_left;
    f.eq.right = eq_right;
    f.eq.shift = shift;
    f.eq.mask = ((size_t)1 << shift) - 1;
    f.eq.id_mul = id_mul;
    f.eq.id_add = id_add;
    size_t need = (count + 255) / 256;
    int grid = (int)(need < (size_t)SC_MAX_BLOCKS ? (need ? need : 1) : SC_MAX_BLOCKS);
    if constexpr (sc_form<F, FORM>::eq_weighted) {
      if (sc_segmented_enabled() && eq_left != nullptr && id_mul == 1 && shift >= 10) {
        size_t nseg = (count + ((size_t)1 << shift) - 1) >> shift;
        grid = (int)(nseg < (size_t)SC_MAX_BLOCKS ? nseg : SC_MAX_BLOCKS);
        k_form_reduce_eqseg<F, NOUT, sc_form<F, FORM>><<<grid, 256, 0, s>>>(f, count, scratch);
        k_form_final<F, NOUT><<<1, 256, 0, s>>>(scratch, grid, out);
        return;
      }
    }
    k_form_reduce<F, NOUT, sc_form<F, FORM>><<<grid, 256, 0, s>>>(f, count, scratch);
    k_form_final<F, NOUT><<<1, 256, 0, s>>>(scratch, grid, out);
  }
  static void sc_reduce(cudaStream_t s, int form, const void* A, const void* B, const void* C,
                        size_t count, size_t half, const void* eq_left, const void* eq_right,
                        int shift, size_t id_mul, size_t id_add, void* scratch, void* out) {
#define SC_CASE(X) \
  case X: sc_launch<X>(s, A, B, C, count, half, eq_left, eq_right, shift, id_mul, id_add, scratch, out); break
    switch (form) {
      SC_CASE(SC_QUAD_PROD);
      SC_CASE(SC_LINEAR);
      SC_CASE(SC_QUADRATIC);
      SC_CASE(SC_CUBIC);
      SC_CASE(SC_EQ_CUBIC3);
      SC_CASE(SC_EQ_CUBIC2);
      SC_CASE(SC_EQ_QUAD1);
      SC_CASE(SC_EQ_CUBIC3_M1);
      SC_CASE(SC_EQ_CUBIC2_M1);
      SC_CASE(SC_EQ_QUAD1_M1);
      SC_CASE(SC_DOT_EQ);
      SC_CASE(SC_DOT);
      default: break;
    }
#undef SC_CASE
  }
  static void eq_small(cudaStream_t s, const void* r, int ell, void* out) {
    size_t n = (size_t)1 << ell;
    k_eq_small<F><<<(unsigned)((n + 255) / 256), 256, 0, s>>>(r, ell, out);
  }
  static void eq_outer(cudaStream_t s, const void* left, const void* right, int right_bits, size_t n,
                       void* out) {
    k_eq_outer<F><<<stream_grid(n, 256), 256, 0, s>>>(left, right, right_bits, n, out);
  }
  static void batch_invert(cudaStream_t s, const void* in, size_t n, void* out, int* zero_flag) {
    static const int forced = [] {
      const char* e = getenv("NOVA_B200_BINV_CHUNK");
      int v = e ? atoi(e) : 0;
      return v >= 1 && v <= 4096 ? v : 0;
    }();
    int chunk = (int)(n / BINV_MIN_THREADS);
    chunk = chunk < BINV_CHUNK ? BINV_CHUNK : (chunk > BINV_CHUNK_MAX ? BINV_CHUNK_MAX : chunk);
    if (forced) chunk = forced;
    size_t threads = (n + chunk - 1) / chunk;
    k_batch_invert<F><<<(unsigned)((threads + 127) / 128), 128, 0, s>>>(in, n, out, zero_flag, chunk);
  }
  static void rlc(cudaStream_t s, const void* const* polys, const size_t* lens, int k,
                  const void* coeffs, size_t n, void* out) {
    rlc_args a;
    a.k = k;
    for (int i = 0; i < k; i++) {
      a.p[i] = polys[i];
      a.len[i] = lens[i];
    }
    k_rlc<F><<<stream_grid(n, 256), 256, 0, s>>>(a, coeffs, n, out);
  }
  static void kzg_fold(cudaStream_t s, const void* p, const void* x, size_t half, void* out) {
    k_kzg_fold<F><<<stream_grid(half, 256), 256, 0, s>>>(p, x, half, out);
  }
  template <int NU>
  static void poly_eval_n(cudaStream_t s, const void* f, size_t n, const void* us, void* scratch,
                          void* evals) {
    size_t need = (n + 255) / 256;
    int grid = (int)(need < (size_t)SC_MAX_BLOCKS ? (need ? need : 1) : SC_MAX_BLOCKS);
    void* pw = scratch;
    void* partials = (char*)scratch + (size_t)3 * (1 + SC_MAX_BLOCKS + 256) * 32;
    int np = NU * (1 + grid + 256);
    k_poly_eval_powers<F><<<(np + 127) / 128, 128, 0, s>>>(us, NU, grid, (uint64_t)grid * 256, pw);
    k_poly_eval_strided<F, NU><<<grid, 256, 0, s>>>(f, n, pw, partials);
    k_form_final<F, NU><<<1, 256, 0, s>>>(partials, grid, evals);
  }
  static void poly_eval(cudaStream_t s, const void* f, size_t n, const void* us, int nu, void* scratch,
                        void* evals) {
    if (nu == 1) poly_eval_n<1>(s, f, n, us, scratch, evals);
    else if (nu == 2) poly_eval_n<2>(s, f, n, us, scratch, evals);
    else poly_eval_n<3>(s, f, n, us, scratch, evals);
  }
  static void poly_div(cudaStream_t s, const void* f, size_t n, const void* u, void* scratch, void* out) {
    static_assert(POLY_CHUNK == POLY_CHUNK_HOST, "chunk constants out of sync");
    size_t T1 = (n + POLY_CHUNK - 1) / POLY_CHUNK, T2 = (T1 + POLY_CHUNK - 1) / POLY_CHUNK;
    char* base = (char*)scratch;
    void* v1 = base;
    void* s1 = base + T1 * 32;
    void* v2 = base + 2 * T1 * 32;
    void* s2 = base + (2 * T1 + T2) * 32;
    void* y = base + (2 * T1 + 2 * T2) * 32;
    void* ev = base + (2 * T1 + 2 * T2 + 1) * 32;
    unsigned g1 = (unsigned)((T1 + 127) / 128), g2 = (unsigned)((T2 + 127) / 128);
    k_poly_chunk_vals<F><<<g1, 128, 0, s>>>(f, n, u, 1, v1);
    if (T1 <= 8192) {
      k_poly_suffix<F><<<1, 512, 0, s>>>(v1, T1, u, s1, ev);
    } else {
      k_fe_pow<F><<<1, 32, 0, s>>>(u, POLY_CHUNK, y);
      k_poly_chunk_vals<F><<<g2, 128, 0, s>>>(v1, T1, y, 1, v2);
      k_poly_suffix<F><<<1, 512, 0, s>>>(v2, T2, y, s2, ev);
      k_poly_div_apply<F><<<g2, 128, 0, s>>>(v1, T1, y, s2, T1, s1);
    }
    k_poly_div_apply<F><<<g1, 128, 0, s>>>(f, n, u, s1, n - 1, out);
  }
  static void spmv_classify(cudaStream_t s, const void* vals, size_t nnz, int8_t* codes) {
    k_spmv_classify<F><<<(unsigned)((nnz + 255) / 256), 256, 0, s>>>(vals, nnz, codes);
  }
  static void spmv(cudaStream_t s, const uint32_t* indptr, const uint32_t* cols, const int8_t* codes,
                   const void* vals, size_t rows, const void* z1, const void* z2, void* o1, void* o2) {
    if (z2)
      k_spmv<F, 2><<<stream_grid(rows, 256), 256, 0, s>>>(indptr, cols, codes, vals, rows, z1, z2, o1, o2);
    else
      k_spmv<F, 1><<<stream_grid(rows, 256), 256, 0, s>>>(indptr, cols, codes, vals, rows, z1, z1, o1, o1);
  }
  static void spmv_t(cudaStream_t s, const uint32_t* tptr, const uint32_t* trow, const uint32_t* tperm,
                     const int8_t* codes, const void* vals, size_t cols, size_t out_len, const void* rx,
                     void* out) {
    k_spmv_t<F><<<stream_grid(out_len, 256), 256, 0, s>>>(tptr, trow, tperm, codes, vals, cols, out_len, rx, out);
  }
  static void sc_round(cudaStream_t s, int kind, void* state, const void* res, const void* tau,
                       const void* tau_inv, const void* pending, uint32_t pending_len, int absorb_label,
                       int squeeze_label, void* out_poly, void* out_r) {
    k_sc_round<F><<<1, 32, 0, s>>>(kind, (sc_state*)state, res, tau, tau_inv, (const uint8_t*)pending,
                                   pending_len, (uint8_t)absorb_label, (uint8_t)squeeze_label, out_poly, out_r);
  }
  static void fe_inv_each(cudaStream_t s, const void* in, size_t n, void* out) {
    if (n) k_fe_inv_each<F><<<(unsigned)((n + 63) / 64), 64, 0, s>>>(in, n, out);
  }
  static void sc_round_batched(cudaStream_t s, const void* desc, void* state, const void* sums, const void* pending,
                               uint32_t pending_len, int absorb_label, int squeeze_label, void* out_poly, void* out_r) {
    k_sc_round_batched<F><<<1, 32, 0, s>>>(*(const scb_desc*)desc, (scb_state*)state, sums, (const uint8_t*)pending,
                                           pending_len, (uint8_t)absorb_label, (uint8_t)squeeze_label, out_poly, out_r);
  }
  static void eq_prefix_tables(cudaStream_t s, const void* taus, int hi, int K, void* out) {
    k_eq_prefix_tables<F><<<1, 1024, 0, s>>>(taus, hi, K, out);
  }
  static int sc_reduce_multi_partials(cudaStream_t s, const multi_args& a, void* scratch) {
    size_t need = (a.h + 255) / 256;
    unsigned gx = (unsigned)(need < (size_t)SC_MULTI_BLOCKS ? (need ? need : 1) : SC_MULTI_BLOCKS);
    static const bool occ3 = [] {
      const char* e = getenv("NOVA_B200_SC_MULTI_OCC");
      return e && e[0] == '3';
    }();
    if (occ3) k_form_reduce_multi<F, 3><<<dim3(gx, (unsigned)a.n), 256, 0, s>>>(a, scratch);
    else k_form_reduce_multi<F, 2><<<dim3(gx, (unsigned)a.n), 256, 0, s>>>(a, scratch);
    return (int)gx;
  }
  static void sc_round_batched_fused(cudaStream_t s, const void* desc, void* state, const void* partials, int nblocks,
                                     int nsums, const void* pending, uint32_t pending_len, int absorb_label,
                                     int squeeze_label, void* out_poly, void* out_r) {
    k_sc_round_batched_fused<F><<<1, 32 * nsums, 0, s>>>(*(const scb_desc*)desc, (scb_state*)state, partials, nblocks,
                                                       (const uint8_t*)pending, pending_len, (uint8_t)absorb_label,
                                                       (uint8_t)squeeze_label, out_poly, out_r);
  }
  static void poly_eval_small_multi(cudaStream_t s, const poly_multi_args& a, const void* us, int nu, void* evals) {
    if (nu == 1) k_poly_eval_small_multi<F, 1><<<a.k, 256, 0, s>>>(a, us, evals);
    else if (nu == 2) k_poly_eval_small_multi<F, 2><<<a.k, 256, 0, s>>>(a, us, evals);
    else k_poly_eval_small_multi<F, 3><<<a.k, 256, 0, s>>>(a, us, evals);
  }
  static void gather_heads(cudaStream_t s, void* const* zs, int k, void* out) {
    bind_multi_args a{};
    for (int i = 0; i < k; i++) a.z[i] = zs[i];
    k_gather_heads<F><<<1, BIND_MULTI_MAX, 0, s>>>(a, k, out);
  }
  static void sc_reduce_multi(cudaStream_t s, const multi_args& a, void* scratch, void* out) {
    size_t need = (a.h + 255) / 256;
    unsigned gx = (unsigned)(need < (size_t)SC_MULTI_BLOCKS ? (need ? need : 1) : SC_MULTI_BLOCKS);
    k_form_reduce_multi<F><<<dim3(gx, (unsigned)a.n), 256, 0, s>>>(a, scratch);
    k_form_final_multi<F><<<dim3(1, (unsigned)a.n), 256, 0, s>>>(scratch, (int)gx, out);
  }
  static void scb_tail(cudaStream_t s, const scb_tail_args& a, void* state, void* sums, const void* pending,
                       uint32_t pending_len, int absorb_label, int squeeze_label, void* polys, void* rs) {
    k_scb_tail<F><<<1, SCB_TAIL_THREADS, 0, s>>>(a, (scb_state*)state, sums, (const uint8_t*)pending, pending_len,
                                                (uint8_t)absorb_label, (uint8_t)squeeze_label, polys, rs);
  }
  static void on_curve(cudaStream_t s, const void* pts, size_t n, int b_small, uint32_t* first_bad) {
    if (n) k_on_curve<F><<<stream_grid(n, 256), 256, 0, s>>>(pts, n, b_small, first_bad);
  }
  static void powers_canonical(cudaStream_t s, const void* u, size_t n, void* out) {
    if (n) k_powers_canonical<F><<<(unsigned)((n + 127) / 128), 128, 0, s>>>(u, n, out);
  }
  static void scalar_bases(cudaStream_t s, void* bases, size_t n, const void* gen, const void* scalars) {
    if (n) k_scalar_bases<F><<<(unsigned)((n + 127) / 128), 128, 0, s>>>(bases, n, gen, scalars);
  }
  static void poseidon_ro(cudaStream_t s, int t, int r_f, int r_p, const void* rc, const void* mds, const void* elems,
                          uint32_t n, const void* tag, int num_bits, int start_with_one, void* out) {
    poseidon_desc d{t, r_f, r_p};
    k_poseidon_ro<F><<<1, 32 * t, 0, s>>>(d, rc, mds, elems, n, tag, num_bits, start_with_one, out);
  }
  static void to_mont(cudaStream_t s, const void* in, size_t n, void* out) {
    if (n) k_to_mont<F><<<(unsigned)((n + 255) / 256), 256, 0, s>>>(in, n, out);
  }
  static void exchange_identity(cudaStream_t s, const msm_plan& p, void* out_jac) {
#if !defined(NOVA_MSM_ARITH29)
    k_red_final_q<F><<<1, 384, 0, s>>>(nullptr, 0, 4, 4, out_jac, p.peer);
#endif
  }
  static constexpr field_ops table() {
    return field_ops{F::ID,  digits,       expand_key, accumulate, fixup,   reduce,
                     sum_points, jacobian_sum, index_bases, cross_term, axpy,       vec_add, bind_top, bind_top_multi, vec_mul, logup_hash,
                     fold_halves, ipa_scalars, ipa_weights, fill_one,
                     sc_reduce, eq_small, eq_outer, batch_invert, rlc, kzg_fold, poly_eval, poly_div, spmv_classify, spmv, spmv_t,
                     sc_round, fe_inv_each, digits_range, sc_round_batched, on_curve,
                     powers_canonical, scalar_bases, poseidon_ro, to_mont, exchange_identity,
                     sc_round_batched_fused, sc_reduce_multi_partials, gather_heads, poly_eval_small_multi,
                     eq_prefix_tables, sc_reduce_multi, scb_tail};
  }
};

}
```

Before: 260.2 million.

## Replace atomic counting-scatter bucket sort with multi-pass LSD radix sort using decoupled lookback

Swaps the per-bucket count, three-kernel scan and atomic scatter for a multi-pass LSD radix sort of the bucket entries. Each pass ranks items inside a tile with warp ballots, finds global offsets through decoupled lookback over epoch-tagged words, and writes coalesced output through shared memory. The digit kernels now build small per-pass histograms in a capped grid, and bucket starts and heavy buckets come from a binary search over the sorted entries. The aim is to remove global atomic contention and scattered writes, at the cost of several extra passes over the entries, a ping-pong buffer and a lookback array.

```diff
diff --git a/nova_b200/csrc/capi.cu b/nova_b200/csrc/capi.cu
--- a/nova_b200/csrc/capi.cu
+++ b/nova_b200/csrc/capi.cu
@@ -100,8 +100,10 @@
   size_t cap_n = 0;
   void* scalars = nullptr;
   int32_t* digits = nullptr;
-  uint32_t *counts = nullptr, *start = nullptr, *cursor = nullptr, *blocksums = nullptr;
-  uint64_t* entries = nullptr;
+  uint32_t *sortctl = nullptr, *start = nullptr;
+  uint64_t *entries = nullptr, *entries_tmp = nullptr;
+  unsigned long long* look = nullptr;
+  uint32_t sort_epoch = 0;
   void *buckets = nullptr, *parts = nullptr, *rparts = nullptr, *sumscratch = nullptr;
   uint32_t* pkeys = nullptr;
   uint32_t* heavy = nullptr;
@@ -116,7 +118,7 @@
   cudaEvent_t busy = nullptr;
   void release() {
     if (busy) cudaEventDestroy(busy);
-    void* ptrs[] = {scalars, digits, counts, start, cursor, blocksums, entries, buckets,
+    void* ptrs[] = {scalars, digits, sortctl, start, entries, entries_tmp, look, buckets,
                     parts, rparts, sumscratch, pkeys, heavy, hparts, d_out, idx32};
     for (void* p : ptrs)
       if (p) cudaFree(p);
@@ -169,7 +171,7 @@
 };
 
 enum { ST_DIGITS = 0, ST_SORT, ST_ACCUMULATE, ST_FIXUP, ST_REDUCE, ST_COUNT };
-const int STAGE_KERNELS[ST_COUNT] = {1, 4, 1, 3, 2};
+const int STAGE_KERNELS[ST_COUNT] = {1, 1, 1, 3, 2};
 struct profile_state {
   std::mutex mu;
   bool enabled = false;
@@ -267,9 +269,11 @@
     w.out_slots = out_slots;
   }
   if (n <= w.cap_n) return B200_OK;
+  if (n * (size_t)ck.W > 0x7FFFFFFFu)
+    return fail(B200_E_RANGE, "%zu scalars x %d windows exceed 2^31 bucket entries", n, ck.W);
   CU(cudaDeviceSynchronize());
-  void** szbufs[] = {&w.scalars, (void**)&w.digits, (void**)&w.entries, &w.parts, (void**)&w.pkeys,
-                     (void**)&w.heavy, &w.hparts};
+  void** szbufs[] = {&w.scalars, (void**)&w.digits, (void**)&w.entries, (void**)&w.entries_tmp, (void**)&w.look,
+                     &w.parts, (void**)&w.pkeys, (void**)&w.heavy, &w.hparts};
   for (void** p : szbufs)
     if (*p) {
       cudaFree(*p);
@@ -284,13 +288,16 @@
   CU(cudaMalloc(&w.scalars, n * 32));
   CU(cudaMalloc((void**)&w.digits, entries * sizeof(int32_t)));
   CU(cudaMalloc((void**)&w.entries, entries * sizeof(uint64_t)));
+  CU(cudaMalloc((void**)&w.entries_tmp, entries * sizeof(uint64_t)));
+  const size_t look_bytes = (entries + SORT_TILE - 1) / SORT_TILE * SORT_BINS * sizeof(unsigned long long);
+  CU(cudaMalloc((void**)&w.look, look_bytes));
+  CU(cudaMemset(w.look, 0, look_bytes));
+  w.sort_epoch = 0;
   CU(cudaMalloc(&w.parts, 2 * nseg * XYZZ_BYTES));
   CU(cudaMalloc((void**)&w.pkeys, 2 * nseg * sizeof(uint32_t)));
-  if (!w.counts) {
-    CU(cudaMalloc((void**)&w.counts, K * 4));
+  if (!w.sortctl) {
+    CU(cudaMalloc((void**)&w.sortctl, SORT_CTL_WORDS * 4));
     CU(cudaMalloc((void**)&w.start, (K + 1) * 4));
-    CU(cudaMalloc((void**)&w.cursor, K * 4));
-    CU(cudaMalloc((void**)&w.blocksums, 4096 * 4));
     CU(cudaMalloc(&w.buckets, K * XYZZ_BYTES));
     CU(cudaMalloc(&w.rparts, ((size_t)ck.G * (ck.B / ck.m + 4096)) * XYZZ_BYTES));
     CU(cudaMalloc(&w.sumscratch, (size_t)SUM_THREADS * XYZZ_BYTES));
@@ -321,15 +328,17 @@
   p.heavy_cap = ws.heavy_cap;
   p.hparts = ws.hparts;
   p.digits = ws.digits;
-  p.counts = ws.counts;
+  p.sortctl = ws.sortctl;
+  p.sp = make_sort_plan((uint64_t)ck.G * ck.B);
+  p.sort_tag = 0;
+  p.look = ws.look;
   p.start = ws.start;
-  p.cursor = ws.cursor;
   p.entries = ws.entries;
+  p.entries_tmp = ws.entries_tmp;
   p.buckets = ws.buckets;
   p.parts = ws.parts;
   p.pkeys = ws.pkeys;
   p.rparts = ws.rparts;
-  p.blocksums = ws.blocksums;
   return p;
 }
 
@@ -357,9 +366,15 @@
   msm_plan p = make_plan(ck, ws, base_offset, n);
   if (peer) p.peer = *peer;
   if (blinded) p.blind_i = n - 1;
-  size_t K = (size_t)ck.G * ck.B;
-  if (!digits_done) CU(cudaMemsetAsync(p.counts, 0, K * 4, s));
+  if (!digits_done) CU(cudaMemsetAsync(p.sortctl, 0, SORT_CTL_WORDS * 4, s));
+  else CU(cudaMemsetAsync(p.sortctl + SORT_PASSES_MAX * SORT_BINS, 0, SORT_PASSES_MAX * 4, s));
   CU(cudaMemsetAsync(p.heavy, 0, 4, s));
+  if (ws.sort_epoch > 0x7FFFFFFFu - SORT_PASSES_MAX) {
+    CU(cudaMemsetAsync(ws.look, 0, (ws.cap_n * (size_t)ck.W + SORT_TILE - 1) / SORT_TILE * SORT_BINS * 8, s));
+    ws.sort_epoch = 0;
+  }
+  p.sort_tag = ws.sort_epoch + 1;
+  ws.sort_epoch += (uint32_t)p.sp.passes;
   std::lock_guard<std::mutex> plk(g_prof.mu);
   const bool prof = g_prof.enabled && profile_ok;
   const int pset = g_prof.next;
@@ -382,8 +397,7 @@
   else
     sops->digits(s, d_scalars, p);
   STAGE_MARK(ST_SORT);
-  msm_scan(s, p);
-  msm_scatter(s, p);
+  const int sort_launches = msm_sort(s, p);
   STAGE_MARK(ST_ACCUMULATE);
   bops->accumulate(s, ck.tables, p);
   STAGE_MARK(ST_FIXUP);
@@ -394,6 +408,7 @@
 #undef STAGE_MARK
   if (prof) g_prof.pending[pset] = true;
   for (int i = 0; i < ST_COUNT; i++) g_prof.launches += STAGE_KERNELS[i];
+  g_prof.launches += sort_launches - STAGE_KERNELS[ST_SORT];
   g_prof.launches += (ck.c - 1 + 3) / 4 - 1;
   CU(cudaGetLastError());
   return ws_release(ws, s);
@@ -872,7 +887,7 @@
     CU(cudaEventCreateWithFlags(&ev, cudaEventDisableTiming));
     CU(cudaEventRecord(ev, s));
     CU(cudaStreamWaitEvent(side, ev, 0));
-    CU(cudaMemsetAsync(p.counts, 0, (size_t)ck.G * ck.B * 4, side));
+    CU(cudaMemsetAsync(p.sortctl, 0, SORT_CTL_WORDS * 4, side));
     const size_t per = (n + h2d_chunks - 1) / h2d_chunks;
     auto piece = [&](const void* src, size_t lo, size_t hi) -> int {
       CU(cudaMemcpyAsync((char*)W.scalars + 32 * lo, src, 32 * (hi - lo), cudaMemcpyHostToDevice, s));
diff --git a/nova_b200/csrc/capi_stream.inc b/nova_b200/csrc/capi_stream.inc
--- a/nova_b200/csrc/capi_stream.inc
+++ b/nova_b200/csrc/capi_stream.inc
@@ -70,8 +70,7 @@
   if (rc) return rc;
   CU(cudaStreamCreateWithFlags(&w->side, cudaStreamNonBlocking));
   CU(cudaEventCreateWithFlags(&w->ready, cudaEventDisableTiming));
-  size_t K = (size_t)w->target->G * w->target->B;
-  CU(cudaMemsetAsync(w->ws.counts, 0, K * 4, w->side));
+  CU(cudaMemsetAsync(w->ws.sortctl, 0, SORT_CTL_WORDS * 4, w->side));
   CU(cudaMemsetAsync((char*)w->ws.scalars + n * 32, 0, 32, w->side));
   std::lock_guard<std::mutex> lk(g_wstreams_mu);
   *stream_handle = g_next_wstream++;
@@ -143,8 +142,7 @@
   std::lock_guard<std::mutex> lk(w->mu);
   CU(cudaEventRecord(w->ready, g_dev.stream));
   CU(cudaStreamWaitEvent(w->side, w->ready, 0));
-  size_t K = (size_t)w->target->G * w->target->B;
-  CU(cudaMemsetAsync(w->ws.counts, 0, K * 4, w->side));
+  CU(cudaMemsetAsync(w->ws.sortctl, 0, SORT_CTL_WORDS * 4, w->side));
   CU(cudaMemsetAsync((char*)w->ws.scalars + w->n * 32, 0, 32, w->side));
   w->filled = 0;
   w->finished = false;
diff --git a/nova_b200/csrc/msm_common.cu b/nova_b200/csrc/msm_common.cu
--- a/nova_b200/csrc/msm_common.cu
+++ b/nova_b200/csrc/msm_common.cu
@@ -3,192 +3,45 @@
 
 namespace nova {
 
-constexpr int SCAN_BLOCK = 1024;
-constexpr int SCAN_ITEMS = 4;
-
-__global__ void __launch_bounds__(SCAN_BLOCK) k_scan_block(const uint32_t* __restrict__ in,
-                                                           uint32_t* __restrict__ out,
-                                                           uint32_t* __restrict__ blocksums,
-                                                           uint32_t K) {
-  __shared__ uint32_t warp_tot[32];
-  uint32_t base = blockIdx.x * (SCAN_BLOCK * SCAN_ITEMS) + threadIdx.x * SCAN_ITEMS;
-  uint32_t v[SCAN_ITEMS], tot = 0;
-#pragma unroll
-  for (int k = 0; k < SCAN_ITEMS; k++) {
-    v[k] = (base + k < K) ? in[base + k] : 0;
-    tot += v[k];
-  }
-  uint32_t inc = tot;
-  int lane = threadIdx.x & 31, wid = threadIdx.x >> 5;
-#pragma unroll
-  for (int d = 1; d < 32; d <<= 1) {
-    uint32_t o = __shfl_up_sync(0xffffffffu, inc, d);
-    if (lane >= d) inc += o;
-  }
-  if (lane == 31) warp_tot[wid] = inc;
-  __syncthreads();
-  if (wid == 0) {
-    uint32_t w = warp_tot[lane];
-    uint32_t winc = w;
-#pragma unroll
-    for (int d = 1; d < 32; d <<= 1) {
-      uint32_t o = __shfl_up_sync(0xffffffffu, winc, d);
-      if (lane >= d) winc += o;
-    }
-    warp_tot[lane] = winc - w;
-    if (lane == 31) blocksums[blockIdx.x] = winc;
-  }
-  __syncthreads();
-  uint32_t excl = inc - tot + warp_tot[wid];
-#pragma unroll
-  for (int k = 0; k < SCAN_ITEMS; k++) {
-    if (base + k < K) out[base + k] = excl;
-    excl += v[k];
-  }
+void msm_digits_small(cudaStream_t s, const void* scalars, int elem_bytes, const msm_plan& p) {
+  size_t blocks = (p.n + 255) / 256;
+  unsigned grid = (unsigned)(blocks < SORT_HIST_BLOCKS ? blocks : SORT_HIST_BLOCKS);
+  k_digits_small<<<grid, 256, 0, s>>>(scalars, elem_bytes, p.n, p.c, p.W, p.G, p.B, p.digits, p.sortctl, p.sp);
 }
 
-__global__ void __launch_bounds__(SCAN_BLOCK) k_scan_sums(uint32_t* blocksums, uint32_t nblocks) {
-  __shared__ uint32_t warp_tot[32];
-  uint32_t base = threadIdx.x * SCAN_ITEMS;
-  uint32_t v[SCAN_ITEMS], tot = 0;
-#pragma unroll
-  for (int k = 0; k < SCAN_ITEMS; k++) {
-    v[k] = (base + k < nblocks) ? blocksums[base + k] : 0;
-    tot += v[k];
-  }
-  uint32_t inc = tot;
-  int lane = threadIdx.x & 31, wid = threadIdx.x >> 5;
-#pragma unroll
-  for (int d = 1; d < 32; d <<= 1) {
-    uint32_t o = __shfl_up_sync(0xffffffffu, inc, d);
-    if (lane >= d) inc += o;
-  }
-  if (lane == 31) warp_tot[wid] = inc;
-  __syncthreads();
-  if (wid == 0) {
-    uint32_t w = warp_tot[lane], winc = w;
-#pragma unroll
-    for (int d = 1; d < 32; d <<= 1) {
-      uint32_t o = __shfl_up_sync(0xffffffffu, winc, d);
-      if (lane >= d) winc += o;
-    }
-    warp_tot[lane] = winc - w;
-  }
-  __syncthreads();
-  uint32_t excl = inc - tot + warp_tot[wid];
-#pragma unroll
-  for (int k = 0; k < SCAN_ITEMS; k++) {
-    if (base + k < nblocks) blocksums[base + k] = excl;
-    excl += v[k];
-  }
+sort_args make_sort_args(const msm_plan& p) {
+  sort_args a;
+  a.n = (uint32_t)p.n;
+  a.count = (uint32_t)(p.n * (size_t)p.W);
+  a.W = p.W;
+  a.G = p.G;
+  a.B = p.B;
+  a.n_ck = (uint32_t)p.n_ck;
+  a.base_offset = (uint32_t)p.base_offset;
+  a.blind_i = p.blind_i == SIZE_MAX ? NO_KEY : (uint32_t)p.blind_i;
+  a.h_index = (uint32_t)p.h_index;
+  a.sp = p.sp;
+  return a;
 }
 
-__global__ void __launch_bounds__(256) k_scan_add(uint32_t* __restrict__ start,
-                                                  uint32_t* __restrict__ cursor,
-                                                  const uint32_t* __restrict__ counts,
-                                                  const uint32_t* __restrict__ blocksums,
-                                                  uint32_t K, uint32_t* __restrict__ heavy,
-                                                  uint32_t heavy_min, uint32_t heavy_cap) {
-  uint32_t i = blockIdx.x * blockDim.x + threadIdx.x;
-  if (i >= K) return;
-  uint32_t s = start[i] + blocksums[i / (SCAN_BLOCK * SCAN_ITEMS)];
-  start[i] = s;
-  cursor[i] = s;
-  uint32_t cnt = counts[i];
-  if (i == K - 1) start[K] = s + cnt;
-  if (cnt > heavy_min) {
-    uint32_t slot = atomicAdd(&heavy[0], 1u);
-    if (slot < heavy_cap) heavy[1 + slot] = i;
+int msm_sort(cudaStream_t s, const msm_plan& p) {
+  const sort_args a = make_sort_args(p);
+  const unsigned tiles = (unsigned)((a.count + SORT_TILE - 1) / SORT_TILE);
+  const int P = p.sp.passes;
+  const uint64_t* in = nullptr;
+  for (int pass = 0; pass < P; pass++) {
+    uint64_t* out = ((P - 1 - pass) & 1) ? p.entries_tmp : p.entries;
+    if (pass == 0)
+      k_sort_pass<true><<<tiles, SORT_THREADS, 0, s>>>(p.digits, nullptr, out, a, 0, p.sortctl, p.look, p.sort_tag);
+    else
+      k_sort_pass<false><<<tiles, SORT_THREADS, 0, s>>>(nullptr, in, out, a, pass, p.sortctl, p.look,
+                                                        p.sort_tag + (uint32_t)pass);
+    in = out;
   }
-}
-
-__global__ void __launch_bounds__(256) k_digits_small(const void* __restrict__ scalars,
-                                                      int elem_bytes, size_t n, int c, int W, int G,
-                                                      uint32_t B, int32_t* __restrict__ digits,
-                                                      uint32_t* __restrict__ counts) {
-  size_t i = (size_t)blockIdx.x * blockDim.x + threadIdx.x;
-  const bool live = i < n;
-  uint64_t v64 = 0;
-  if (live) switch (elem_bytes) {
-    case 1: v64 = ((const uint8_t*)scalars)[i]; break;
-    case 2: v64 = ((const uint16_t*)scalars)[i]; break;
-    case 4: v64 = ((const uint32_t*)scalars)[i]; break;
-    default: v64 = ((const uint64_t*)scalars)[i]; break;
-  }
-  const uint32_t half = 1u << (c - 1);
-  const uint64_t mask = (1ull << c) - 1;
-  uint32_t carry = 0;
-  for (int w = 0; w < W; w++) {
-    int bit = w * c;
-    uint32_t v = bit < 64 ? (uint32_t)((v64 >> bit) & mask) : 0u;
-    v += carry;
-    int32_t dgt;
-    if (v > half) {
-      dgt = (int32_t)v - (int32_t)(1u << c);
-      carry = 1;
-    } else {
-      dgt = (int32_t)v;
-      carry = 0;
-    }
-    if (live) digits[(size_t)w * n + i] = dgt;
-    uint32_t key = NO_KEY;
-    if (dgt != 0) {
-      uint32_t mag = dgt < 0 ? (uint32_t)(-dgt) : (uint32_t)dgt;
-      key = (uint32_t)(w % G) * B + (mag - 1);
-    }
-    count_key(counts, key);
-  }
-}
-
-__global__ void __launch_bounds__(256) k_scatter(const int32_t* __restrict__ digits, size_t n,
-                                                 int W, int G, uint32_t B, size_t n_ck,
-                                                 size_t base_offset, size_t blind_i, size_t h_index,
-                                                 uint32_t* __restrict__ cursor,
-                                                 uint64_t* __restrict__ entries) {
-  size_t i = (size_t)blockIdx.x * blockDim.x + threadIdx.x;
-  int w = blockIdx.y;
-  int32_t dgt = i < n ? digits[(size_t)w * n + i] : 0;
-  uint32_t sign = dgt < 0 ? 1u : 0u;
-  uint32_t mag = sign ? (uint32_t)(-dgt) : (uint32_t)dgt;
-  uint32_t key = dgt != 0 ? (uint32_t)(w % G) * B + (mag - 1) : NO_KEY;
-  uint32_t pos;
-  if (!warp_has_repeats(key)) {
-    if (key == NO_KEY) return;
-    pos = atomicAdd(&cursor[key], 1u);
-  } else {
-    unsigned peers = __match_any_sync(0xFFFFFFFFu, key);
-    if (key == NO_KEY) return;
-    unsigned lane = threadIdx.x & 31u, leader = (unsigned)(__ffs(peers) - 1);
-    uint32_t base = 0;
-    if (lane == leader) base = atomicAdd(&cursor[key], (uint32_t)__popc(peers));
-    base = __shfl_sync(peers, base, leader);
-    pos = base + (uint32_t)__popc(peers & ((1u << lane) - 1u));
-  }
-  size_t bi = (i == blind_i) ? h_index : base_offset + i;
-  uint32_t idx = (uint32_t)((size_t)(w / G) * n_ck + bi);
-  entries[pos] = ((uint64_t)key << 32) | ((uint64_t)sign << 31) | idx;
-}
-
-void msm_scan(cudaStream_t s, const msm_plan& p) {
-  uint32_t K = (uint32_t)p.G * p.B;
-  uint32_t per_block = SCAN_BLOCK * SCAN_ITEMS;
-  uint32_t nblocks = (K + per_block - 1) / per_block;
-  k_scan_block<<<nblocks, SCAN_BLOCK, 0, s>>>(p.counts, p.start, p.blocksums, K);
-  k_scan_sums<<<1, SCAN_BLOCK, 0, s>>>(p.blocksums, nblocks);
-  k_scan_add<<<(K + 255) / 256, 256, 0, s>>>(p.start, p.cursor, p.counts, p.blocksums, K, p.heavy,
-                                             p.heavy_min, p.heavy_cap);
-}
-
-void msm_digits_small(cudaStream_t s, const void* scalars, int elem_bytes, const msm_plan& p) {
-  k_digits_small<<<(unsigned)((p.n + 255) / 256), 256, 0, s>>>(scalars, elem_bytes, p.n, p.c, p.W,
-                                                               p.G, p.B, p.digits, p.counts);
-}
-
-void msm_scatter(cudaStream_t s, const msm_plan& p) {
-  dim3 grid((unsigned)((p.n + 255) / 256), (unsigned)p.W);
-  k_scatter<<<grid, 256, 0, s>>>(p.digits, p.n, p.W, p.G, p.B, p.n_ck, p.base_offset, p.blind_i,
-                                 p.h_index, p.cursor,
-                                 p.entries);
+  const uint32_t K = (uint32_t)p.G * p.B;
+  k_sort_starts<<<(K + 1 + SORT_THREADS - 1) / SORT_THREADS, SORT_THREADS, 0, s>>>(
+      p.entries, p.sortctl, p.sp, K, p.start, p.heavy, p.heavy_min, p.heavy_cap);
+  return P + 1;
 }
 
 }
diff --git a/nova_b200/csrc/msm_kernels.cuh b/nova_b200/csrc/msm_kernels.cuh
--- a/nova_b200/csrc/msm_kernels.cuh
+++ b/nova_b200/csrc/msm_kernels.cuh
@@ -2,6 +2,7 @@
 #include <cuda_runtime.h>
 #include "curve29.cuh"
 #include "coop.cuh"
+#include "msm_sort.cuh"
 
 namespace nova {
 
@@ -30,15 +31,17 @@
   int L;
   int m;
   int32_t* digits;
-  uint32_t* counts;
+  uint32_t* sortctl;
+  sort_plan sp;
+  uint32_t sort_tag;
+  unsigned long long* look;
   uint32_t* start;
-  uint32_t* cursor;
   uint64_t* entries;
+  uint64_t* entries_tmp;
   void* buckets;
   void* parts;
   uint32_t* pkeys;
   void* rparts;
-  uint32_t* blocksums;
   uint32_t* heavy;
   uint32_t heavy_min;
   uint32_t heavy_cap;
@@ -46,72 +49,62 @@
   msm_peer peer;
 };
 
-constexpr uint32_t NO_KEY = 0xFFFFFFFFu;
-__device__ __forceinline__ bool warp_has_repeats(uint32_t key) {
-  uint32_t next = __shfl_down_sync(0xFFFFFFFFu, key, 1);
-  return __any_sync(0xFFFFFFFFu, key != NO_KEY && key == next && (threadIdx.x & 31u) != 31u);
-}
-__device__ __forceinline__ void count_key(uint32_t* counts, uint32_t key) {
-  if (!warp_has_repeats(key)) {
-    if (key != NO_KEY) atomicAdd(&counts[key], 1u);
-    return;
-  }
-  unsigned peers = __match_any_sync(0xFFFFFFFFu, key);
-  if (key != NO_KEY && (threadIdx.x & 31u) == (unsigned)(__ffs(peers) - 1))
-    atomicAdd(&counts[key], (uint32_t)__popc(peers));
-}
-
 template <class S>
 __global__ void __launch_bounds__(256) k_digits(const void* __restrict__ scalars, size_t i0, size_t i1,
                                                 size_t n, int c, int W, int G, uint32_t B,
                                                 int32_t* __restrict__ digits,
-                                                uint32_t* __restrict__ counts) {
-  size_t i = i0 + (size_t)blockIdx.x * blockDim.x + threadIdx.x;
-  const bool live = i < i1;
-  fe_t s = live ? fe_from_mont<S>(fe_load(scalars, i)) : fe_zero<S>();
-  uint32_t p[8], t[8];
-  load_p<S>(p);
-  bool neg = false;
-  if (!fe_is_zero(s)) {
-    sub8(t, p, s.l);
-    uint32_t d[8];
-    uint32_t lt = sub8(d, t, s.l);
-    if (lt) {
-      neg = true;
+                                                uint32_t* __restrict__ hist, const sort_plan sp) {
+  __shared__ uint32_t s_hist[SORT_PASSES_MAX * SORT_BINS];
+  sort_hist_clear(s_hist);
+  for (size_t blk = i0 + (size_t)blockIdx.x * blockDim.x; blk < i1; blk += (size_t)gridDim.x * blockDim.x) {
+    size_t i = blk + threadIdx.x;
+    const bool live = i < i1;
+    fe_t s = live ? fe_from_mont<S>(fe_load(scalars, i)) : fe_zero<S>();
+    uint32_t p[8], t[8];
+    load_p<S>(p);
+    bool neg = false;
+    if (!fe_is_zero(s)) {
+      sub8(t, p, s.l);
+      uint32_t d[8];
+      uint32_t lt = sub8(d, t, s.l);
+      if (lt) {
+        neg = true;
 #pragma unroll
-      for (int k = 0; k < 8; k++) s.l[k] = t[k];
-    }
-  }
-  const uint32_t half = 1u << (c - 1);
-  const uint32_t mask = (1u << c) - 1;
-  uint32_t carry = 0;
-  for (int w = 0; w < W; w++) {
-    int bit = w * c;
-    int limb = bit >> 5, sh = bit & 31;
-    uint32_t v = 0;
-    if (limb < 8) {
-      uint64_t two = s.l[limb];
-      if (limb + 1 < 8) two |= (uint64_t)s.l[limb + 1] << 32;
-      v = (uint32_t)(two >> sh) & mask;
-    }
-    v += carry;
-    int32_t dgt;
-    if (v > half) {
-      dgt = (int32_t)v - (int32_t)(1u << c);
-      carry = 1;
-    } else {
-      dgt = (int32_t)v;
-      carry = 0;
-    }
-    if (neg) dgt = -dgt;
-    if (live) digits[(size_t)w * n + i] = dgt;
-    uint32_t key = NO_KEY;
-    if (dgt != 0) {
-      uint32_t mag = dgt < 0 ? (uint32_t)(-dgt) : (uint32_t)dgt;
-      key = (uint32_t)(w % G) * B + (mag - 1);
-    }
-    count_key(counts, key);
-  }
+        for (int k = 0; k < 8; k++) s.l[k] = t[k];
+      }
+    }
+    const uint32_t half = 1u << (c - 1);
+    const uint32_t mask = (1u << c) - 1;
+    uint32_t carry = 0;
+    for (int w = 0; w < W; w++) {
+      int bit = w * c;
+      int limb = bit >> 5, sh = bit & 31;
+      uint32_t v = 0;
+      if (limb < 8) {
+        uint64_t two = s.l[limb];
+        if (limb + 1 < 8) two |= (uint64_t)s.l[limb + 1] << 32;
+        v = (uint32_t)(two >> sh) & mask;
+      }
+      v += carry;
+      int32_t dgt;
+      if (v > half) {
+        dgt = (int32_t)v - (int32_t)(1u << c);
+        carry = 1;
+      } else {
+        dgt = (int32_t)v;
+        carry = 0;
+      }
+      if (neg) dgt = -dgt;
+      if (live) digits[(size_t)w * n + i] = dgt;
+      uint32_t key = NO_KEY;
+      if (dgt != 0) {
+        uint32_t mag = dgt < 0 ? (uint32_t)(-dgt) : (uint32_t)dgt;
+        key = (uint32_t)(w % G) * B + (mag - 1);
+      }
+      sort_hist_count(s_hist, key, sp);
+    }
+  }
+  sort_hist_flush(s_hist, hist, sp);
 }
 
 template <class F>
diff --git a/nova_b200/csrc/msm_sort.cuh b/nova_b200/csrc/msm_sort.cuh
--- /dev/null
+++ b/nova_b200/csrc/msm_sort.cuh
@@ -0,0 +1,310 @@
+#pragma once
+#if !defined(NOVA_SIMT_HOST)
+#include <cuda_runtime.h>
+#endif
+#include <cstddef>
+#include <cstdint>
+#include "field.cuh"
+
+namespace nova {
+
+constexpr uint32_t NO_KEY = 0xFFFFFFFFu;
+
+constexpr int SORT_THREADS = 256;
+constexpr int SORT_WARPS = SORT_THREADS / 32;
+constexpr int SORT_ITEMS = 16;
+constexpr int SORT_TILE = SORT_THREADS * SORT_ITEMS;
+constexpr int SORT_RADIX_MAX = 8;
+constexpr int SORT_BINS = 1 << SORT_RADIX_MAX;
+constexpr int SORT_PASSES_MAX = 4;
+constexpr int SORT_CTL_WORDS = SORT_PASSES_MAX * SORT_BINS + SORT_PASSES_MAX;
+constexpr unsigned SORT_HIST_BLOCKS = 1024;
+constexpr int SORT_LOOK_WINDOW = 4;
+constexpr int SORT_MIN_BLOCKS = 3;
+static_assert(SORT_BINS == SORT_THREADS, "the per-bin steps run one bin per thread");
+
+struct sort_plan {
+  int passes;
+  int bits;
+};
+
+inline sort_plan make_sort_plan(uint64_t K) {
+  int kb = 1;
+  while (kb < 32 && ((uint64_t)1 << kb) < K) kb++;
+  sort_plan sp;
+  sp.passes = (kb + SORT_RADIX_MAX - 1) / SORT_RADIX_MAX;
+  sp.bits = (kb + sp.passes - 1) / sp.passes;
+  return sp;
+}
+
+struct sort_args {
+  uint32_t n;
+  uint32_t count;
+  int W, G;
+  uint32_t B;
+  uint32_t n_ck;
+  uint32_t base_offset;
+  uint32_t blind_i;
+  uint32_t h_index;
+  sort_plan sp;
+};
+
+NOVA_D void sort_hist_clear(uint32_t* sh ) {
+  for (int i = threadIdx.x; i < SORT_PASSES_MAX * SORT_BINS; i += blockDim.x) sh[i] = 0;
+  __syncthreads();
+}
+
+NOVA_D void sort_hist_count(uint32_t* sh, uint32_t key, const sort_plan sp) {
+  const bool live = key != NO_KEY;
+  const unsigned live_mask = __ballot_sync(0xFFFFFFFFu, live);
+  if (live_mask == 0) return;
+  const unsigned lane = threadIdx.x & 31u, leader = (unsigned)(__ffs(live_mask) - 1);
+  const uint32_t lead_key = __shfl_sync(0xFFFFFFFFu, key, (int)leader);
+  const bool same = __ballot_sync(0xFFFFFFFFu, live && key != lead_key) == 0;
+  const uint32_t mask = (1u << sp.bits) - 1;
+  for (int p = 0; p < sp.passes; p++) {
+    const uint32_t bin = (key >> (p * sp.bits)) & mask;
+    if (same) {
+      if (lane == leader) atomicAdd(&sh[p * SORT_BINS + bin], (uint32_t)__popc(live_mask));
+    } else if (live) {
+      atomicAdd(&sh[p * SORT_BINS + bin], 1u);
+    }
+  }
+}
+
+NOVA_D void sort_hist_flush(const uint32_t* sh, uint32_t* hist, const sort_plan sp) {
+  __syncthreads();
+  for (int i = threadIdx.x; i < sp.passes * SORT_BINS; i += blockDim.x) {
+    const uint32_t v = sh[i];
+    if (v) atomicAdd(&hist[i], v);
+  }
+}
+
+static __global__ void __launch_bounds__(256) k_digits_small(const void* __restrict__ scalars, int elem_bytes,
+                                                             size_t n, int c, int W, int G, uint32_t B,
+                                                             int32_t* __restrict__ digits, uint32_t* __restrict__ hist,
+                                                             const sort_plan sp) {
+  __shared__ uint32_t s_hist[SORT_PASSES_MAX * SORT_BINS];
+  sort_hist_clear(s_hist);
+  for (size_t blk = (size_t)blockIdx.x * blockDim.x; blk < n; blk += (size_t)gridDim.x * blockDim.x) {
+    const size_t i = blk + threadIdx.x;
+    const bool live = i < n;
+    uint64_t v64 = 0;
+    if (live) switch (elem_bytes) {
+      case 1: v64 = ((const uint8_t*)scalars)[i]; break;
+      case 2: v64 = ((const uint16_t*)scalars)[i]; break;
+      case 4: v64 = ((const uint32_t*)scalars)[i]; break;
+      default: v64 = ((const uint64_t*)scalars)[i]; break;
+    }
+    const uint32_t half = 1u << (c - 1);
+    const uint64_t mask = (1ull << c) - 1;
+    uint32_t carry = 0;
+    for (int w = 0; w < W; w++) {
+      int bit = w * c;
+      uint32_t v = bit < 64 ? (uint32_t)((v64 >> bit) & mask) : 0u;
+      v += carry;
+      int32_t dgt;
+      if (v > half) {
+        dgt = (int32_t)v - (int32_t)(1u << c);
+        carry = 1;
+      } else {
+        dgt = (int32_t)v;
+        carry = 0;
+      }
+      if (live) digits[(size_t)w * n + i] = dgt;
+      uint32_t key = NO_KEY;
+      if (dgt != 0) {
+        uint32_t mag = dgt < 0 ? (uint32_t)(-dgt) : (uint32_t)dgt;
+        key = (uint32_t)(w % G) * B + (mag - 1);
+      }
+      sort_hist_count(s_hist, key, sp);
+    }
+  }
+  sort_hist_flush(s_hist, hist, sp);
+}
+
+NOVA_D uint32_t sort_block_scan(uint32_t v, uint32_t* s_tmp, uint32_t* total) {
+  const int lane = threadIdx.x & 31, warp = threadIdx.x >> 5;
+  uint32_t inc = v;
+#pragma unroll
+  for (int d = 1; d < 32; d <<= 1) {
+    const uint32_t o = __shfl_up_sync(0xFFFFFFFFu, inc, d);
+    if (lane >= d) inc += o;
+  }
+  if (lane == 31) s_tmp[warp] = inc;
+  __syncthreads();
+  uint32_t before = 0, all = 0;
+#pragma unroll
+  for (int w = 0; w < SORT_WARPS; w++) {
+    const uint32_t t = s_tmp[w];
+    before += w < warp ? t : 0u;
+    all += t;
+  }
+  __syncthreads();
+  *total = all;
+  return before + inc - v;
+}
+
+constexpr unsigned long long LOOK_INCLUSIVE = 1ull << 32;
+NOVA_D unsigned long long look_word(uint32_t tag, bool inclusive, uint32_t v) {
+  return ((unsigned long long)tag << 33) | (inclusive ? LOOK_INCLUSIVE : 0ull) | v;
+}
+
+template <bool FIRST>
+__global__ void __launch_bounds__(SORT_THREADS, SORT_MIN_BLOCKS) k_sort_pass(const int32_t* __restrict__ digits,
+                                                            const uint64_t* __restrict__ in,
+                                                            uint64_t* __restrict__ out, const sort_args a, int pass,
+                                                            uint32_t* __restrict__ ctl,
+                                                            unsigned long long* __restrict__ look, uint32_t tag) {
+  __shared__ uint64_t s_items[SORT_TILE];
+  __shared__ uint32_t s_warp[SORT_WARPS][SORT_BINS];
+  __shared__ uint32_t s_glob[SORT_BINS];
+  __shared__ uint32_t s_tmp[SORT_WARPS];
+  __shared__ uint32_t s_tile;
+  const int tid = threadIdx.x, lane = tid & 31, warp = tid >> 5;
+  const unsigned lt_mask = (1u << lane) - 1u;
+  const int shift = pass * a.sp.bits;
+  const uint32_t mask = (1u << a.sp.bits) - 1u;
+
+  if (tid == 0) s_tile = atomicAdd(&ctl[SORT_PASSES_MAX * SORT_BINS + pass], 1u);
+#pragma unroll
+  for (int w = 0; w < SORT_WARPS; w++) s_warp[w][tid] = 0;
+  uint32_t M;
+  const uint32_t bin_base = sort_block_scan(ctl[pass * SORT_BINS + tid], s_tmp, &M);
+  const uint32_t tile = s_tile;
+  const uint32_t count = FIRST ? a.count : M;
+  if ((uint64_t)tile * SORT_TILE >= count) return;
+  const uint32_t wbase = tile * SORT_TILE + warp * 32 * SORT_ITEMS + lane;
+
+  uint64_t item[SORT_ITEMS];
+#pragma unroll
+  for (int j = 0; j < SORT_ITEMS; j++) {
+    const uint32_t idx = wbase + 32u * j;
+    if (FIRST) item[j] = idx < count ? (uint64_t)(uint32_t)digits[idx] : 0ull;
+    else item[j] = idx < count ? in[idx] : 0ull;
+  }
+  uint32_t rank[SORT_ITEMS];
+#pragma unroll
+  for (int j = 0; j < SORT_ITEMS; j++) {
+    const uint32_t idx = wbase + 32u * j;
+    bool valid;
+    if (FIRST) {
+      const int32_t dgt = (int32_t)(uint32_t)item[j];
+      valid = idx < count && dgt != 0;
+      if (valid) {
+        const uint32_t w = idx / a.n, i = idx - w * a.n;
+        const uint32_t sign = dgt < 0 ? 1u : 0u;
+        const uint32_t mag = sign ? (uint32_t)(-dgt) : (uint32_t)dgt;
+        const uint32_t key = (w % (uint32_t)a.G) * a.B + (mag - 1);
+        const uint32_t bi = i == a.blind_i ? a.h_index : a.base_offset + i;
+        const uint32_t tix = (w / (uint32_t)a.G) * a.n_ck + bi;
+        item[j] = ((uint64_t)key << 32) | ((uint64_t)sign << 31) | tix;
+      }
+    } else {
+      valid = idx < count;
+    }
+    const uint32_t bin = (uint32_t)(item[j] >> (32 + shift)) & mask;
+    unsigned peers = __ballot_sync(0xFFFFFFFFu, valid);
+    rank[j] = NO_KEY;
+    if (peers) {
+      for (int b = 0; b < a.sp.bits; b++) {
+        const unsigned m = __ballot_sync(0xFFFFFFFFu, (bin >> b) & 1u);
+        peers &= ((bin >> b) & 1u) ? m : ~m;
+      }
+      const uint32_t before = valid ? s_warp[warp][bin] : 0u;
+      __syncwarp();
+      if (valid) {
+        rank[j] = before + (uint32_t)__popc(peers & lt_mask);
+        if ((peers & lt_mask) == 0) s_warp[warp][bin] = before + (uint32_t)__popc(peers);
+      }
+      __syncwarp();
+    }
+  }
+  __syncthreads();
+
+  uint32_t run = 0;
+#pragma unroll
+  for (int w = 0; w < SORT_WARPS; w++) {
+    const uint32_t c = s_warp[w][tid];
+    s_warp[w][tid] = run;
+    run += c;
+  }
+  volatile unsigned long long* vlook = look;
+  const size_t slot = (size_t)tile * SORT_BINS + tid;
+  vlook[slot] = look_word(tag, tile == 0, run);
+  uint32_t tile_total;
+  const uint32_t tile_off = sort_block_scan(run, s_tmp, &tile_total);
+  uint32_t excl = 0;
+  for (uint32_t t = tile; t > 0;) {
+    unsigned long long v[SORT_LOOK_WINDOW];
+#pragma unroll
+    for (int q = 0; q < SORT_LOOK_WINDOW; q++)
+      v[q] = (uint32_t)q < t ? vlook[(size_t)(t - 1 - q) * SORT_BINS + tid] : 0ull;
+    bool go = true;
+#pragma unroll
+    for (int q = 0; q < SORT_LOOK_WINDOW; q++) {
+      go = go && t > 0 && (uint32_t)(v[q] >> 33) == tag;
+      if (go) {
+        excl += (uint32_t)v[q];
+        t = (v[q] & LOOK_INCLUSIVE) ? 0u : t - 1;
+      }
+    }
+  }
+  if (tile != 0) vlook[slot] = look_word(tag, true, excl + run);
+  s_glob[tid] = bin_base + excl - tile_off;
+#pragma unroll
+  for (int w = 0; w < SORT_WARPS; w++) s_warp[w][tid] += tile_off;
+  __syncthreads();
+
+#pragma unroll
+  for (int j = 0; j < SORT_ITEMS; j++) {
+    if (rank[j] != NO_KEY) {
+      const uint32_t bin = (uint32_t)(item[j] >> (32 + shift)) & mask;
+      s_items[s_warp[warp][bin] + rank[j]] = item[j];
+    }
+  }
+  __syncthreads();
+  for (uint32_t k = tid; k < tile_total; k += SORT_THREADS) {
+    const uint64_t e = s_items[k];
+    const uint32_t bin = (uint32_t)(e >> (32 + shift)) & mask;
+    out[s_glob[bin] + k] = e;
+  }
+}
+
+static __global__ void __launch_bounds__(SORT_THREADS) k_sort_starts(const uint64_t* __restrict__ entries,
+                                                              const uint32_t* __restrict__ ctl, const sort_plan sp,
+                                                              uint32_t K, uint32_t* __restrict__ start,
+                                                              uint32_t* __restrict__ heavy, uint32_t heavy_min,
+                                                              uint32_t heavy_cap) {
+  __shared__ uint32_t s_base[SORT_BINS + 1];
+  __shared__ uint32_t s_start[SORT_THREADS + 1];
+  __shared__ uint32_t s_tmp[SORT_WARPS];
+  const int tid = threadIdx.x;
+  const int last = sp.passes - 1, shift = last * sp.bits;
+  uint32_t M;
+  s_base[tid] = sort_block_scan(ctl[last * SORT_BINS + tid], s_tmp, &M);
+  if (tid == 0) s_base[SORT_BINS] = M;
+  __syncthreads();
+  auto lower_bound = [&](uint32_t k) -> uint32_t {
+    if (k >= K) return M;
+    const uint32_t top = k >> shift;
+    uint32_t lo = s_base[top], hi = s_base[top + 1];
+    while (lo < hi) {
+      const uint32_t mid = lo + (hi - lo) / 2;
+      if ((uint32_t)(entries[mid] >> 32) < k) lo = mid + 1;
+      else hi = mid;
+    }
+    return lo;
+  };
+  const uint32_t k = blockIdx.x * SORT_THREADS + tid;
+  s_start[tid] = lower_bound(k);
+  if (tid == SORT_THREADS - 1) s_start[SORT_THREADS] = lower_bound(k + 1);
+  __syncthreads();
+  if (k <= K) start[k] = s_start[tid];
+  if (k < K && s_start[tid + 1] - s_start[tid] > heavy_min) {
+    const uint32_t slot = atomicAdd(&heavy[0], 1u);
+    if (slot < heavy_cap) heavy[1 + slot] = k;
+  }
+}
+
+}
diff --git a/nova_b200/csrc/ops.cuh b/nova_b200/csrc/ops.cuh
--- a/nova_b200/csrc/ops.cuh
+++ b/nova_b200/csrc/ops.cuh
@@ -111,8 +111,7 @@
   }
 }
 
-void msm_scan(cudaStream_t, const msm_plan&);
-void msm_scatter(cudaStream_t, const msm_plan&);
+int msm_sort(cudaStream_t, const msm_plan&);
 void msm_digits_small(cudaStream_t, const void* scalars, int elem_bytes, const msm_plan&);
 
 }
diff --git a/nova_b200/csrc/ops_impl.cuh b/nova_b200/csrc/ops_impl.cuh
--- a/nova_b200/csrc/ops_impl.cuh
+++ b/nova_b200/csrc/ops_impl.cuh
@@ -40,8 +40,9 @@
   static void digits_range(cudaStream_t s, const void* scalars, size_t i0, size_t i1, const msm_plan& p) {
     if (i1 <= i0) return;
     int block = 256;
-    int grid = (int)((i1 - i0 + block - 1) / block);
-    k_digits<F><<<grid, block, 0, s>>>(scalars, i0, i1, p.n, p.c, p.W, p.G, p.B, p.digits, p.counts);
+    size_t blocks = (i1 - i0 + block - 1) / block;
+    int grid = (int)(blocks < SORT_HIST_BLOCKS ? blocks : SORT_HIST_BLOCKS);
+    k_digits<F><<<grid, block, 0, s>>>(scalars, i0, i1, p.n, p.c, p.W, p.G, p.B, p.digits, p.sortctl, p.sp);
   }
   static void expand_key(cudaStream_t s, void* tables, size_t n_ck, int ntables, int shift) {
     int block = 128;
```

New measurement: 286.4 million (median of 6 runs). 10.1% higher.
